# Ensembl/WiggleTools

Measured on AMD Instinct MI355X. Metric: genomic bp/s (whole node) for 'mean' over N BigWig tracks, higher is better.
Workload: dtype f64

## Files before the change

### wiggletools_amd/csrc/build.py

```python
import os
import subprocess
import sys

HERE = os.path.dirname(os.path.abspath(__file__))
SO = os.path.join(HERE, "libwiggletools_amd.so")
KERNEL_SRCS = ["wt_reduce_stream.hip", "wt_reduce_moments.hip", "wt_reduce_order.hip", "wt_patch_kernels.hip", "wt_delta_kernels.hip", "wt_walk.hip"]
SRCS = KERNEL_SRCS + ["wt_engine.hip", "wt_pipe.hip", "wt_compress.hip", "wt_moments.hip", "wt_map.hip", "wt_cover.hip", "wt_region.hip", "wt_synth.hip", "wt_bwdev.hip", "wt_defaults.cpp", "wt_iter_abi.cpp", "wt_bigwig.cpp", "wt_bwwrite.cpp"]
LIBS = ["-lz"]
FLAGS = ["--offload-arch=gfx950", "-O3", "-std=c++17", "-fPIC", "-shared", "-ffp-contract=off",
         "-Wall", "-Wno-unused-function", "-Wno-pass-failed"]


def build_source_variant(srcs, name, extra_flags):
    from concurrent.futures import ThreadPoolExecutor
    srcs = [srcs] if isinstance(srcs, str) else list(srcs)
    hipcc = os.environ.get("HIPCC", "/opt/rocm/bin/hipcc")
    objdir = os.path.join(HERE, ".obj")
    cflags = [f for f in FLAGS if f != "-shared"]

    def compile_one(src):
        obj = os.path.join(objdir, "%s_%s.o" % (src, name))
        subprocess.check_call([hipcc] + cflags + list(extra_flags) + ["-c", os.path.join(HERE, src), "-o", obj])
        return obj

    with ThreadPoolExecutor(len(srcs)) as ex:
        objs = list(ex.map(compile_one, srcs))
    others = [os.path.join(objdir, s + ".o") for s in SRCS if s not in srcs]
    out = os.path.join(HERE, "libwiggletools_amd_%s.so" % name)
    subprocess.check_call([hipcc, "--offload-arch=gfx950", "-shared", "-fPIC"] + objs + others + LIBS + ["-o", out])
    return out


def build(force=False, verbose=False):
    import time
    from concurrent.futures import ThreadPoolExecutor
    srcs = [os.path.join(HERE, s) for s in SRCS]
    hipcc = os.environ.get("HIPCC", "/opt/rocm/bin/hipcc")
    objdir = os.path.join(HERE, ".obj")
    os.makedirs(objdir, exist_ok=True)
    cflags = [f for f in FLAGS if f != "-shared"]

    def newer_than_deps(target, obj):
        try:
            words = open(obj + ".d").read().replace("\\\n", " ").split()
            t = os.path.getmtime(target)
        except OSError:
            return False
        files = [os.path.join(HERE, w) for w in words[1:] if not w.endswith(":")]
        return bool(files) and all(os.path.exists(f) and os.path.getmtime(f) <= t for f in files)

    objs = [os.path.join(objdir, os.path.basename(s) + ".o") for s in srcs]
    if not force and all(newer_than_deps(SO, o) for o in objs):
        if verbose:
            print("wiggletools_amd: libwiggletools_amd.so is newer than the sources / headers of its %d objects: REUSED (force=True recompiles)" % len(objs))
        return SO
    if verbose:
        print("wiggletools_amd: COMPILING %d sources for gfx950 with hipcc" % len(srcs))

    def compile_one(src):
        obj = os.path.join(objdir, os.path.basename(src) + ".o")
        if not force and newer_than_deps(obj, obj):
            if verbose:
                print("wiggletools_amd: %s unchanged: object REUSED" % os.path.basename(src))
            return obj
        cmd = [hipcc] + cflags + ["-MMD", "-MF", os.path.relpath(obj, HERE) + ".d", "-c", os.path.basename(src), "-o", os.path.relpath(obj, HERE)]
        if verbose:
            print(" ".join(cmd))
        t0 = time.time()
        subprocess.check_call(cmd, cwd=HERE)
        if verbose:
            print("wiggletools_amd: %s compiled in %.0f s" % (os.path.basename(src), time.time() - t0))
        return obj

    with ThreadPoolExecutor(len(srcs)) as ex:
        objs = list(ex.map(compile_one, srcs))
    cmd = [hipcc, "--offload-arch=gfx950", "-shared", "-fPIC"] + objs + LIBS + ["-o", SO]
    if verbose:
        print(" ".join(cmd))
    subprocess.check_call(cmd)
    return SO


if __name__ == "__main__":
    print(build(force="--force" in sys.argv, verbose=True))
```

### wiggletools_amd/csrc/wt_core.h

```cpp
#ifndef WT_CORE_H_
#define WT_CORE_H_

#include <stdint.h>
#include <math.h>
#include <type_traits>

#ifdef WT_EMU
#define WT_DEV inline
#define WT_RESTRICT
#else
#include <hip/hip_runtime.h>
#define WT_DEV __device__ __forceinline__
#define WT_RESTRICT __restrict__
#endif

enum {
    WT_OP_SUM = 0, WT_OP_PRODUCT = 1, WT_OP_MEAN = 2, WT_OP_VAR = 3, WT_OP_STDDEV = 4,
    WT_OP_ENTROPY = 5, WT_OP_CV = 6, WT_OP_MIN = 7, WT_OP_MAX = 8, WT_OP_MEDIAN = 9,
    WT_OP_TTEST = 10, WT_OP_MWU = 11,
    WT_OP_MULTIPLEX = 12
};
#define WT_STRICT_SET0 1u
#define WT_STRICT_SET1 2u

// ... 1263 lines not shown
        auto sweep = [&](auto body) {
            int i = 0;
            for (; i + WT_MWU_RB <= N; i += WT_MWU_RB) {
                KeyT k[WT_MWU_RB];
#pragma unroll
                for (int u = 0; u < WT_MWU_RB; u++) k[u] = col[(size_t) (i + u) * colstride];
#pragma unroll
                for (int u = 0; u < WT_MWU_RB; u++) body(k[u]);
            }
            for (; i < N; i++) body(col[(size_t) i * colstride]);
        };
        sweep([&](KeyT key) { all_and &= key; all_or |= key; });
        const KeyT disputed = all_and ^ all_or;
        KeyT Kk = 0;
        for (int b = KB - B; b >= 0; b -= B) {
            const KeyT group = (KeyT) NT << b;
            if (!(disputed & group)) { Kk |= all_and & group; continue; }
            KeyT trial[NT];
            int below[NT];
#pragma unroll
            for (int q = 0; q < NT; q++) { trial[q] = Kk | ((KeyT) (q + 1) << b); below[q] = 0; }
            sweep([&](KeyT key) {
#pragma unroll
                for (int q = 0; q < NT; q++) below[q] += (key < trial[q]);
            });
#pragma unroll
            for (int q = 0; q < NT; q++)
                if (below[q] <= kth) Kk = trial[q];
        }
        const double m = (sizeof(ScrT) == 4) ? (double) wt_unkey32((uint32_t) Kk) : wt_unkey64((uint64_t) Kk);
        res[0] = A.nan[0] ? wt_nan() : m;
        return;
    }
    if (OP == WT_OP_MWU) return;
    if (OP == WT_OP_MULTIPLEX) {
#pragma unroll
        for (int k = 0; k < K; k++) res[k] = A.a[k];
        return;
    }
}

WT_DEV int32_t wt_next_breakpoint(const WtParams &P, const WtCtx &c, int p) {
    const int w = p >> 6;
    const uint64_t here = c.U[w] & ~wt_mask_incl(p & 63);
    const int w2 = here ? w : (int) c.nextw[w];
    if (w2 < 0) return c.sh->next_bp;
    const uint64_t bits = here ? here : c.U[w2];
    return c.sh->w0 + w2 * 64 + wt_ctz64(bits);
}

WT_DEV void wt_phase_emask(const WtParams &P, WtCtx &c, bool two, int tid, int nt) {
    const int nw32 = P.n_words * 2;
    const uint64_t *any0 = (const uint64_t *) c.cover;
    const uint64_t *all0 = (const uint64_t *) (c.cover + nw32);
    const uint64_t *any1 = (const uint64_t *) (c.cover + 2 * nw32);
    const uint64_t *all1 = (const uint64_t *) (c.cover + 3 * nw32);
    for (int w = tid; w < P.n_words; w += nt) {
        uint64_t emit = (P.flags & WT_STRICT_SET0) ? all0[w] : any0[w];
        if (two) emit &= (P.flags & WT_STRICT_SET1) ? all1[w] : any1[w];
        const long long room = (long long) c.sh->emit_hi - ((long long) c.sh->w0 + (long long) w * 64);
        if (room < 64) emit &= (room <= 0) ? 0ull : ((1ull << room) - 1ull);
        c.E[w] = c.U[w] & emit;
    }
    if (tid == nt - 1) {
        int last = -1;
        for (int w = P.n_words - 1; w >= 0; w--) {
            c.nextw[w] = (int16_t) last;
            if (c.U[w]) last = w;
        }
    }
}

WT_DEV void wt_phase_escan(const WtParams &P, WtCtx &c, int tid, int nt) {
    for (int w = tid; w <= P.n_words; w += nt) {
        unsigned s = 0;
        for (int x = 0; x < w; x++) s += (unsigned) wt_popc64(c.E[x]);
        c.epfx[w] = s;
    }
}

template <int K>
WT_DEV unsigned wt_lane_emit_bits(const WtParams &P, const WtCtx &c, int tid) {
    const int p0 = tid * K;
    if (p0 >= P.W) return 0u;
    return (unsigned) ((c.E[p0 >> 6] >> (p0 & 63)) & ((1ull << K) - 1ull));
}

template <int OP, class ValT, class ScrT, int K, int NR>
WT_DEV void wt_phase_eval_chunk(const WtParams &P, WtCtx &c, WtAcc<K, NR> &A, int pass, int t_lo, int t_hi, bool all,
                                int tid, int nt) {
    const int p0 = tid * K;
    if (p0 >= P.W) return;
    const unsigned emit_bits = all ? ((1u << K) - 1u) : wt_lane_emit_bits<K>(P, c, tid);
    if (!emit_bits) return;
    long long run0 = 0;
    if (OP == WT_OP_MULTIPLEX) {
        const int w = p0 >> 6, b0 = p0 & 63;
        const uint64_t below0 = b0 ? wt_mask_incl(b0 - 1) : 0ull;
        run0 = c.sh->goffset + c.epfx[w] + wt_popc64(c.E[w] & below0);
    }
    wt_eval_chunk<OP, ValT, ScrT, K>(P, c, p0, A, pass, t_lo, t_hi, c.scratch, tid, P.W, emit_bits, run0);
}

template <int OP, class ValT, class ScrT, int K, int NR>
WT_DEV void wt_phase_eval_finish(const WtParams &P, WtCtx &c, WtAcc<K, NR> &A, WtLane<K> &L, int tid, int nt) {
    const unsigned emit_bits = wt_lane_emit_bits<K>(P, c, tid);
    if (!emit_bits) return;
    wt_eval_finish<OP, ValT, ScrT, K>(P, A, L.res, c.scratch, c.attr, tid, P.W, emit_bits);
}

template <class ScrT>
WT_DEV void wt_phase_mwu_rank(const WtParams &P, WtCtx &c, int tid, int nt) {
    const int p = tid % P.W, part = tid / P.W, nparts = nt / P.W;
    if (!((c.E[p >> 6] >> (p & 63)) & 1ull)) return;
    wt_mwu_rank<ScrT>(P, c.scratch, c.attr, p, P.W, part, nparts);
}
template <int K, int NR>
WT_DEV void wt_phase_mwu_tail(const WtParams &P, WtCtx &c, const WtAcc<K, NR> &A, WtLane<K> &L, int tid, int nt) {
    if (tid >= P.W || !((c.E[tid >> 6] >> (tid & 63)) & 1ull)) return;
    L.res[0] = A.nan[0] ? wt_nan() : wt_mwu_tail(P, c.attr, tid, P.W);
}

WT_DEV void wt_lookback_finish(const WtParams &P, WtCtx &c, long long k, unsigned long long excl,
                               unsigned long long mine) {
    WtShared *sh = c.sh;
    wt_status_store(&P.status[k], WT_FLAG_PFX | (excl + mine));
    sh->goffset = (long long) excl;
    const int ch = sh->chrom;
    if (k == P.c_first_win[ch]) P.chrom_run_off[ch] = (long long) excl;
    if (k == P.n_windows - 1) {
        P.chrom_run_off[P.n_chrom] = (long long) (excl + mine);
        P.counters[WT_CTR_RUNS] = excl + mine;
    }
    if ((long long) (excl + mine) > P.capacity) wt_glb_or64(&P.counters[WT_CTR_ERROR], WT_ERR_CAPACITY);
}

WT_DEV void wt_phase_lookback(const WtParams &P, WtCtx &c, long long k, unsigned long long mine);
WT_DEV void wt_phase_lookback(const WtParams &P, WtCtx &c, long long k) {
    wt_phase_lookback(P, c, k, (unsigned long long) c.epfx[P.n_words]);
}
WT_DEV void wt_phase_lookback(const WtParams &P, WtCtx &c, long long k, unsigned long long mine) {
    c.sh->n_emit = (int32_t) mine;
    unsigned long long excl = 0;
    if (k > 0) {
        wt_status_store(&P.status[k], WT_FLAG_AGG | mine);
        long long j = k - 1;
        for (;;) {
            unsigned long long v = wt_status_load(&P.status[j]);
            unsigned spins = 0;
            while (v == 0) {
                wt_backoff();
                v = wt_status_load(&P.status[j]);
                if (++spins > (1u << 24)) {
                    wt_glb_or64(&P.counters[WT_CTR_ERROR], WT_ERR_LOOKBACK);
                    v = WT_FLAG_PFX;
                }
            }
            excl += v & WT_VAL_MASK;
            if (v & WT_FLAG_PFX) break;
            j--;
        }
    }
    wt_lookback_finish(P, c, k, excl, mine);
}

#ifndef WT_EMU
WT_DEV void wt_lookback_publish(const WtParams &P, WtCtx &c, long long k, unsigned long long mine) {
    c.sh->n_emit = (int32_t) mine;
    if (k > 0) wt_status_store(&P.status[k], WT_FLAG_AGG | mine);
}
WT_DEV void wt_lookback_publish(const WtParams &P, WtCtx &c, long long k) {
    wt_lookback_publish(P, c, k, (unsigned long long) c.epfx[P.n_words]);
}

WT_DEV void wt_lookback_complete(const WtParams &P, WtCtx &c, long long k, int lane, unsigned long long mine);
WT_DEV void wt_lookback_complete(const WtParams &P, WtCtx &c, long long k, int lane) {
    wt_lookback_complete(P, c, k, lane, (unsigned long long) c.epfx[P.n_words]);
}
#ifndef WT_LOOKBACK_DEPTH
#define WT_LOOKBACK_DEPTH 1
#endif
WT_DEV void wt_lookback_complete(const WtParams &P, WtCtx &c, long long k, int lane, unsigned long long mine) {
    unsigned long long excl = 0;
    long long base = k - 1;
    unsigned long long ahead[WT_LOOKBACK_DEPTH];
    int have = 0;
    while (base >= 0) {
        const long long j = base - lane;
        if (have == 0) {
#pragma unroll
            for (int r = 0; r < WT_LOOKBACK_DEPTH; r++) {
                const long long jr = j - 64ll * r;
                ahead[r] = (jr >= 0) ? wt_status_load(&P.status[jr]) : WT_FLAG_PFX;
            }
            have = WT_LOOKBACK_DEPTH;
        }
        unsigned long long v = ahead[0];
#pragma unroll
        for (int r = 1; r < WT_LOOKBACK_DEPTH; r++) v = (WT_LOOKBACK_DEPTH - have == r) ? ahead[r] : v;
        have--;
        unsigned long long pfx;
        unsigned spins = 0;
        for (;;) {
            const unsigned long long ready = __ballot(v != 0);
            pfx = __ballot((v & WT_FLAG_PFX) != 0);
            const unsigned long long need = pfx ? (((pfx & (0ull - pfx)) << 1) - 1ull) : ~0ull;
            if ((ready & need) == need) break;
            if (++spins > (1u << 22)) {
                if (lane == 0) wt_glb_or64(&P.counters[WT_CTR_ERROR], WT_ERR_LOOKBACK);
                pfx = 1ull;
                break;
            }
            if (v == 0) { wt_backoff(); v = wt_status_load(&P.status[j]); }
        }
        const int p = pfx ? (int) wt_ctz64(pfx) : 63;
        unsigned long long part = (lane <= p) ? (v & WT_VAL_MASK) : 0ull;
        excl += wt_wave_sum_u64(part);
        if (pfx) break;
        base -= 64;
    }
    if (lane == 0) wt_lookback_finish(P, c, k, excl, mine);
}
#endif

template <int OP, class ValT, int K>
WT_DEV void wt_phase_write(const WtParams &P, WtCtx &c, const WtLane<K> &L, int tid, int nt) {
    const int p0 = tid * K;
    unsigned emit_bits = 0;
    if (p0 < P.W) emit_bits = (unsigned) ((c.E[p0 >> 6] >> (p0 & 63)) & ((1ull << K) - 1ull));
    unsigned long long bp = 0;
    if (emit_bits) {
        const long long goff = c.sh->goffset;
        const int32_t w0 = c.sh->w0;
        const int w = p0 >> 6, b0 = p0 & 63;
        const uint64_t below0 = b0 ? wt_mask_incl(b0 - 1) : 0ull;
        long long idx = goff + c.epfx[w] + wt_popc64(c.E[w] & below0);
#pragma unroll
        for (int k = 0; k < K; k++) {
            if (!((emit_bits >> k) & 1u)) continue;
            const long long o = idx++;
            const int p = p0 + k;
            const int32_t fin = wt_next_breakpoint(P, c, p);
            bp += (unsigned long long) (fin - (w0 + p));
            if (o >= P.capacity) continue;
            P.o_start[o] = w0 + p;
            P.o_finish[o] = fin;
            P.o_value[o] = L.res[k];
        }
        wt_lds_add64(&c.sh->bp_sum, bp);
    }
}

WT_DEV void wt_window_stats(const WtParams &P, WtCtx &c) {
    if (c.sh->bp_sum) wt_glb_add64(&P.counters[WT_CTR_BP], c.sh->bp_sum);
    if (c.sh->n_intervals) wt_glb_add64(&P.counters[WT_CTR_INTERVALS], c.sh->n_intervals);
}

WT_DEV long long wt_index_find_segment(const WtParams &P, long long g) {
    long long lo = 0, hi = (long long) P.n_chrom * P.n_tracks;
    while (hi - lo > 1) {
        const long long mid = (lo + hi) >> 1;
        if (P.seg_off[mid] <= g) lo = mid; else hi = mid;
    }
    return lo;
}

struct WtIndexCursor {
    long long seg, s0, s1;
    long long nw, rowbase;
    int32_t cb;
    int i;
};

WT_DEV void wt_index_cursor_set(const WtParams &P, WtIndexCursor &c, long long seg) {
    const int N = P.n_tracks;
    c.seg = seg;
    c.s0 = P.seg_off[seg];
    c.s1 = P.seg_off[seg + 1];
    const int ch = (int) (seg / N);
    c.i = (int) (seg - (long long) ch * N);
    c.cb = P.cbase[ch];
    c.nw = P.c_nwin[ch];
    c.rowbase = P.c_first_win[ch] + ch;
}

WT_DEV void wt_index_apply(const WtParams &P, WtIndexCursor &c, long long g, int32_t f, int32_t pf) {
    while (g >= c.s1) wt_index_cursor_set(P, c, c.seg + 1);
    if (g > c.s0 && g + 1 < c.s1 && pf >= c.cb &&
        ((uint32_t) (pf - c.cb) >> P.logW) == ((uint32_t) (f - c.cb) >> P.logW)) return;
    const long long jr = g - c.s0;
    const int32_t cb = c.cb;
    long long m_lo = 0;
    if (jr > 0 && pf >= cb) m_lo = (long long) ((uint32_t) (pf - cb) >> P.logW) + 1;
    long long m_hi = (f >= cb) ? (long long) ((uint32_t) (f - cb) >> P.logW) : -1;
    const bool last = (g + 1 == c.s1);
    if (m_lo > m_hi && !last) return;
    const int N = P.n_tracks;
    if (m_hi > c.nw) m_hi = c.nw;
    for (long long m = m_lo; m <= m_hi; m++) P.widx[(size_t) (c.rowbase + m) * N + c.i] = (uint32_t) jr;
    if (last)
        for (long long m = m_hi + 1; m <= c.nw; m++) P.widx[(size_t) (c.rowbase + m) * N + c.i] = (uint32_t) (jr + 1);
}

WT_DEV long long wt_lane_lower_bound(const int32_t *fin, long long lo, long long hi, long long g, long long b) {
    if (lo >= hi) return lo;
    if ((long long) fin[g] >= b) {
        hi = g;
        for (long long d = 1;; d <<= 1) {
            const long long q = hi - d;
            if (q < lo) break;
            if ((long long) fin[q] < b) { lo = q + 1; break; }
            hi = q;
        }
    } else {
        lo = g + 1;
        for (long long d = 1;; d <<= 1) {
            const long long q = lo + d - 1;
            if (q >= hi) break;
            if ((long long) fin[q] >= b) { hi = q; break; }
            lo = q + 1;
        }
    }
    while (lo < hi) {
        const long long mid = (lo + hi) >> 1;
        if ((long long) fin[mid] < b) lo = mid + 1; else hi = mid;
    }
    return lo;
}

#include "wt_delta.h"
#include "wt_walk.h"
#include "wt_mwalk.h"

#endif
```

### wiggletools_amd/csrc/wt_devscope.h

```cpp
#ifndef WT_DEVSCOPE_H_
#define WT_DEVSCOPE_H_
#include <hip/hip_runtime.h>

#include <vector>

struct WtDevScope {
    std::vector<void *> ptrs;
    WtDevScope() = default;
    WtDevScope(const WtDevScope &) = delete;
    WtDevScope &operator=(const WtDevScope &) = delete;
    template <class T>
    hipError_t alloc(T **p, size_t bytes) {
        void *q = nullptr;
        const hipError_t e = hipMalloc(&q, bytes ? bytes : 1);
        if (e == hipSuccess) { ptrs.push_back(q); *p = (T *) q; }
        return e;
    }
    ~WtDevScope() {
        for (void *q : ptrs) (void) hipFree(q);
    }
};

#endif
```

### wiggletools_amd/csrc/wt_engine.hip

```cpp
#include <hip/hip_runtime.h>

#include <cstdio>
#include <thread>
#include <atomic>
#include <cstring>
#include <map>
#include <mutex>
#include <string>
#include <vector>

#include "wt_host.h"
#include "wt_trackset.h"
#include "wt_core.h"
#include "wt_plan.h"
#include "wt_kernels.h"
#include "wt_devscope.h"

#ifndef WT_INDEX_UNROLL
#define WT_INDEX_UNROLL 2
#endif
#define WT_INDEX_CHUNK (256 * 4 * WT_INDEX_UNROLL)
__global__ void __launch_bounds__(256) wt_index_kernel(const WtParams P, long long total, long long span) {
    const long long dev_total = P.seg_off[(long long) P.n_chrom * P.n_tracks];
    if (total > dev_total) total = dev_total;
    const long long begin0 = (long long) blockIdx.x * span;
    long long end0 = begin0 + span;
    if (end0 > total) end0 = total;
    if (begin0 >= end0) return;
    WtIndexCursor cur;
    wt_index_cursor_set(P, cur, wt_index_find_segment(P, begin0));
    struct __attribute__((packed, aligned(4))) V4 { int32_t x[4]; };
    V4 f[WT_INDEX_UNROLL], nf[WT_INDEX_UNROLL];
    int32_t pf[WT_INDEX_UNROLL], npf[WT_INDEX_UNROLL];
    const long long n_full = (end0 - begin0) / WT_INDEX_CHUNK;
    auto fetch = [&](long long base, V4 (&v)[WT_INDEX_UNROLL], int32_t (&p)[WT_INDEX_UNROLL]) {
#pragma unroll
        for (int u = 0; u < WT_INDEX_UNROLL; u++) {
            const long long g = base + 4ll * (threadIdx.x + 256 * u);
            v[u] = *(const V4 *) (P.finish + g);
            p[u] = P.finish[g > 0 ? g - 1 : 0];
        }
    };
    if (n_full > 0) {
        const long long last_full = begin0 + (n_full - 1) * WT_INDEX_CHUNK;
        fetch(begin0, f, pf);
        for (long long begin = begin0; begin <= last_full; begin += WT_INDEX_CHUNK) {
            const long long nb = begin + WT_INDEX_CHUNK;
            fetch(nb <= last_full ? nb : last_full, nf, npf);
#pragma unroll
            for (int u = 0; u < WT_INDEX_UNROLL; u++) {
                const long long g = begin + 4ll * (threadIdx.x + 256 * u);
                int32_t prev = pf[u];
#pragma unroll
                for (int q = 0; q < 4; q++) {
                    wt_index_apply(P, cur, g + q, f[u].x[q], prev);
                    prev = f[u].x[q];
                }
            }
#pragma unroll
            for (int u = 0; u < WT_INDEX_UNROLL; u++) { f[u] = nf[u]; pf[u] = npf[u]; }
        }
    }
    const long long begin = begin0 + n_full * WT_INDEX_CHUNK;
    if (begin < end0) {
#pragma unroll
        for (int u = 0; u < WT_INDEX_UNROLL; u++) {
            const long long g = begin + 4ll * (threadIdx.x + 256 * u);
            int32_t prev = (g < end0 && g > 0) ? P.finish[g - 1] : 0;
#pragma unroll
            for (int q = 0; q < 4; q++) {
                if (g + q < end0) {
                    const int32_t fq = P.finish[g + q];
                    wt_index_apply(P, cur, g + q, fq, prev);
                    prev = fq;
                }
            }
        }
    }
}

#define WT_ISEARCH_ROWS 64
#define WT_ISEARCH_TRACKS 16

__device__ __forceinline__ int wt_index_row_chrom(const WtParams &P, long long row) {
    int lo = 0;
    for (int hi = P.n_chrom; hi - lo > 1;) {
        const int mid = (lo + hi) >> 1;
        if (P.c_first_win[mid] + mid <= row) lo = mid; else hi = mid;
    }
    return lo;
}

__global__ void __launch_bounds__(256) wt_index_coarse_kernel(const WtParams P, long long n_strips, uint32_t *coarse) {
    const long long t = (long long) blockIdx.x * 256 + threadIdx.x;
    const int N = P.n_tracks;
    if (t >= n_strips * N) return;
    const long long strip = t / N;
    const int i = (int) (t - strip * N);
    const long long row = strip * WT_ISEARCH_ROWS;
    const int ch = wt_index_row_chrom(P, row);
    const long long m = row - (P.c_first_win[ch] + ch);
    const long long seg = (long long) ch * N + i;
    const long long s0 = P.seg_off[seg], n = P.seg_off[seg + 1] - s0;
    const long long b = (long long) P.cbase[ch] + (m << P.logW);
    coarse[t] = (uint32_t) wt_lane_lower_bound(P.finish + s0, 0, n, n >> 1, b);
}

__global__ void __launch_bounds__(WT_ISEARCH_ROWS * WT_ISEARCH_TRACKS) wt_index_search_kernel(const WtParams P, long long n_rows, long long n_strips,
                                                                                              const uint32_t *coarse) {
    __shared__ uint32_t out[WT_ISEARCH_ROWS][WT_ISEARCH_TRACKS + 1];
    const int tid = threadIdx.x, lane = tid & 63, wave = tid >> 6;
    const int N = P.n_tracks;
    const long long strip = blockIdx.x;
    const long long r0 = strip * WT_ISEARCH_ROWS;
    const int i = (int) blockIdx.y * WT_ISEARCH_TRACKS + wave;
    if (i < N) {
        long long row = r0 + lane;
        if (row > n_rows - 1) row = n_rows - 1;
        const int ch = wt_index_row_chrom(P, row);
        const long long m = row - (P.c_first_win[ch] + ch);
        const long long seg = (long long) ch * N + i;
        const long long s0 = P.seg_off[seg], n = P.seg_off[seg + 1] - s0;
        const long long b = (long long) P.cbase[ch] + (m << P.logW);
        const int32_t *fin = P.finish + s0;
        const int ch_first = __shfl(ch, 0);
        const bool have_next = strip + 1 < n_strips;
        const int ch_next = have_next ? wt_index_row_chrom(P, r0 + WT_ISEARCH_ROWS) : -1;
        const bool real_a = ch == ch_first, real_b = ch == ch_next;
        const long long A = real_a ? (long long) coarse[strip * N + i] : 0;
        const long long B = real_b ? (long long) coarse[(strip + 1) * N + i] : n;
        long long g = (real_a && real_b) ? A + (((B - A) * lane) >> 6) : (A + B) >> 1;
        if (g > B - 1) g = B - 1;
        out[lane][wave] = (uint32_t) wt_lane_lower_bound(fin, A, B, g, b);
    }
    __syncthreads();
    const int orow = tid / WT_ISEARCH_TRACKS, ocol = tid % WT_ISEARCH_TRACKS;
    const long long row = r0 + orow;
    const int track = (int) blockIdx.y * WT_ISEARCH_TRACKS + ocol;
    if (row < n_rows && track < N) P.widx[(size_t) row * N + track] = out[orow][ocol];
}

__global__ void __launch_bounds__(256) wt_index_compare_kernel(const uint32_t *a, const uint32_t *b, long long n, unsigned long long *diff) {
    const long long t = (long long) blockIdx.x * 256 + threadIdx.x;
    if (t < n && a[t] != b[t]) atomicAdd(diff, 1ull);
}

__global__ void __launch_bounds__(256) wt_extents_kernel(const int64_t *seg_off, const int32_t *start,
                                                          const int32_t *finish, long long n_seg,
                                                          int32_t *first_start, int32_t *last_finish) {
    const long long s = (long long) blockIdx.x * blockDim.x + threadIdx.x;
    if (s >= n_seg) return;
    const long long lo = seg_off[s], hi = seg_off[s + 1];
    first_start[s] = hi > lo ? start[lo] : 0;
    last_finish[s] = hi > lo ? finish[hi - 1] : 0;
}

__global__ void __launch_bounds__(256) wt_validate_kernel(const int32_t *start, const int32_t *finish, const int64_t *seg_off,
                                                           long long n_seg, long long total, unsigned long long *out) {
    const long long g = (long long) blockIdx.x * blockDim.x + threadIdx.x;
    if (g >= total) return;
    bool bad = finish[g] <= start[g];
    if (!bad && g > 0 && start[g] < finish[g - 1]) {
        long long lo = 0, hi = n_seg;
        while (hi - lo > 1) {
            const long long mid = (lo + hi) >> 1;
            if (seg_off[mid] <= g) lo = mid; else hi = mid;
        }
        bad = seg_off[lo] != g;
    }
    if (bad) {
        atomicAdd(&out[0], 1ull);
        atomicMin(&out[1], (unsigned long long) g);
    }
}

static thread_local std::string g_last_error;

int wt_fail(int code, const std::string &msg) {
    g_last_error = msg;
    return code;
}

template <class T>
static hipError_t wt_grow(T **p, int64_t *cap, int64_t need) {
    if (*cap >= need && *p) return hipSuccess;
    int64_t c = *cap * 2;
    if (c < need) c = need;
    if (c < 1) c = 1;
    (void) hipFree(*p);
    *p = nullptr; *cap = 0;
    const hipError_t e = hipMalloc((void **) p, sizeof(T) * (size_t) c);
    if (e == hipSuccess) *cap = c;
    return e;
}

static void wt_free_windows(WtWindows &w) {
    (void) hipFree(w.d_tabs);
    (void) hipFree(w.d_widx); (void) hipFree(w.d_cidx); (void) hipFree(w.d_status); (void) hipFree(w.d_bad_list); (void) hipFree(w.d_bad_goff);
    if (w.h_tab) (void) hipHostFree(w.h_tab);
    w = WtWindows();
}

extern "C" {

const char *wtamd_last_error(void) { return g_last_error.c_str(); }
const char *wtamd_version(void) { return "wiggletools_amd 0.1 (gfx950)"; }

int wtamd_device_count(void) {
    int n = 0;
    if (hipGetDeviceCount(&n) != hipSuccess) return 0;
    return n;
}

__global__ void wt_warm_kernel(int *p) { if (p && threadIdx.x == 4096) *p = 0; }

static std::mutex g_warm_mu;
static std::thread *g_warm_thread = nullptr;
static bool g_warm_started = false;

extern "C++" void wt_warmup_join() {
    std::thread *t = nullptr;
    { std::lock_guard<std::mutex> lk(g_warm_mu); t = g_warm_thread; g_warm_thread = nullptr; }
    if (t) { t->join(); delete t; }
}

static std::atomic<int> g_device_chosen{-1};

void wtamd_warmup_async(void) {
    std::lock_guard<std::mutex> lk(g_warm_mu);
    if (g_warm_started || getenv("WTAMD_NO_WARMUP")) return;
    int n = 0, cur = -1;
    if (hipGetDeviceCount(&n) != hipSuccess || n <= 0) { (void) hipGetLastError(); return; }
    int ordinal = g_device_chosen.load();
    if (ordinal < 0 && hipGetDevice(&cur) == hipSuccess && (n == 1 || cur > 0)) ordinal = cur;
    if (ordinal < 0 || ordinal >= n) return;
    g_warm_started = true;
    g_warm_thread = new std::thread([ordinal] {
        if (hipSetDevice(ordinal) != hipSuccess) { (void) hipGetLastError(); return; }
        hipStream_t st[3] = {nullptr, nullptr, nullptr};
        for (auto &s : st)
            if (hipStreamCreateWithFlags(&s, hipStreamNonBlocking) != hipSuccess) s = nullptr;
        for (auto &s : st)
            if (s) hipLaunchKernelGGL(wt_warm_kernel, dim3(1), dim3(64), 0, s, (int *) nullptr);
        for (auto &s : st)
            if (s) { (void) hipStreamSynchronize(s); (void) hipStreamDestroy(s); }
        (void) hipGetLastError();
    });
    atexit(wt_warmup_join);
}

int wtamd_set_device(int ordinal) {
    wt_warmup_join();
    WT_HIP(hipSetDevice(ordinal));
    g_device_chosen.store(ordinal);
    return WTAMD_OK;
}

int wtamd_current_device(void) {
    int d = 0;
    if (hipGetDevice(&d) != hipSuccess) { (void) hipGetLastError(); return -1; }
    return d;
}

extern "C++" int wt_trackset_common(const wtamd_tracks *t, wtamd_trackset *ts) {
    if (!t || t->n_chrom < 0 || t->n_tracks <= 0 || !t->seg_off || !t->defaults)
        return wt_fail(WTAMD_ERR_ARG, "wtamd_trackset_create: bad tracks descriptor");
    if (wtamd_device_count() <= 0) return wt_fail(WTAMD_ERR_NODEVICE, "no HIP device visible");
    ts->n_chrom = t->n_chrom;
    ts->n_tracks = t->n_tracks;
    ts->value_f64 = t->value_is_f64 != 0;
    const int64_t n_seg = (int64_t) t->n_chrom * t->n_tracks;
    ts->seg_off.assign(t->seg_off, t->seg_off + n_seg + 1);
    for (int64_t s = 0; s < n_seg; s++)
        if (ts->seg_off[s + 1] < ts->seg_off[s]) return wt_fail(WTAMD_ERR_ARG, "seg_off not monotone");
    ts->n_intervals = ts->seg_off[n_seg] - ts->seg_off[0];
    if (ts->seg_off[0] != 0) return wt_fail(WTAMD_ERR_ARG, "seg_off[0] must be 0");
    ts->defaults.assign(t->defaults, t->defaults + t->n_tracks);
    if (t->range_lo && t->range_hi) {
        ts->range_lo.assign(t->range_lo, t->range_lo + t->n_chrom);
        ts->range_hi.assign(t->range_hi, t->range_hi + t->n_chrom);
    }
    ts->scratch_f32 = !ts->value_f64 && wt_defaults_fit_f32(ts->defaults.data(), ts->n_tracks);
    WT_HIP(hipGetDevice(&ts->device));
    hipDeviceProp_t prop;
    WT_HIP(hipGetDeviceProperties(&prop, ts->device));
    ts->num_cu = prop.multiProcessorCount;
    WT_HIP(hipMalloc(&ts->d_seg_off, sizeof(int64_t) * (n_seg + 1)));
    WT_HIP(hipMemcpy(ts->d_seg_off, ts->seg_off.data(), sizeof(int64_t) * (n_seg + 1), hipMemcpyHostToDevice));
    WT_HIP(hipMalloc(&ts->d_defaults, sizeof(double) * t->n_tracks));
    WT_HIP(hipMemcpy(ts->d_defaults, ts->defaults.data(), sizeof(double) * t->n_tracks, hipMemcpyHostToDevice));
    WT_HIP(hipMalloc(&ts->d_counters, sizeof(unsigned long long) * WT_CTR_N));
    WT_HIP(hipHostMalloc(&ts->h_counters, sizeof(unsigned long long) * WT_CTR_N));
    WT_HIP(hipHostMalloc(&ts->h_debug, sizeof(unsigned long long) * 16));
    memset(ts->h_debug, 0, sizeof(unsigned long long) * 16);
    WT_HIP(hipMalloc(&ts->d_chrom_run_off, sizeof(int64_t) * (t->n_chrom + 1)));
    WT_HIP(hipEventCreate(&ts->ev_i0));
    WT_HIP(hipEventCreate(&ts->ev_i1));
    WT_HIP(hipEventCreate(&ts->ev_r0));
    WT_HIP(hipEventCreate(&ts->ev_r1));
    return WTAMD_OK;
}

extern "C++" int wt_check_extents(wtamd_trackset *ts) {
    for (size_t q = 0; q < ts->last_finish.size(); q++)
        if (ts->seg_off[q + 1] > ts->seg_off[q] && ts->last_finish[q] > WTAMD_MAX_COORD) {
            const int64_t bad = ts->last_finish[q];
            return wt_fail(WTAMD_ERR_ARG, "run finish " + std::to_string(bad) + " above the supported maximum " +
                           std::to_string((long long) WTAMD_MAX_COORD) + " (2^31 - 65537)");
        }
    return WTAMD_OK;
}

static int wt_refresh_extents_device(wtamd_trackset *ts) {
    const int64_t n_seg = (int64_t) ts->n_chrom * ts->n_tracks;
    ts->first_start.assign(n_seg, 0);
    ts->last_finish.assign(n_seg, 0);
    if (n_seg > 0 && ts->n_intervals > 0) {
        int32_t *d_fs = nullptr, *d_lf = nullptr;
        WtDevScope scope;
        WT_HIP(scope.alloc(&d_fs, sizeof(int32_t) * n_seg));
        WT_HIP(scope.alloc(&d_lf, sizeof(int32_t) * n_seg));
        hipLaunchKernelGGL(wt_extents_kernel, dim3((unsigned) ((n_seg + 255) / 256)), dim3(256), 0, 0,
                           ts->d_seg_off, ts->d_start, ts->d_finish, (long long) n_seg, d_fs, d_lf);
        WT_HIP(hipGetLastError());
        WT_HIP(hipMemcpy(ts->first_start.data(), d_fs, sizeof(int32_t) * n_seg, hipMemcpyDeviceToHost));
        WT_HIP(hipMemcpy(ts->last_finish.data(), d_lf, sizeof(int32_t) * n_seg, hipMemcpyDeviceToHost));
    }
    return WTAMD_OK;
}

static int wt_create_host_impl(const wtamd_tracks *t, wtamd_trackset *ts) {
    int rc = wt_trackset_common(t, ts);
    if (rc != WTAMD_OK) return rc;
    ts->owns = true;
    const int64_t n = ts->n_intervals;
    const size_t vsz = ts->value_f64 ? 8 : 4;
    const int64_t n_alloc = n > 0 ? n : 1;
    WT_HIP(hipMalloc(&ts->d_start, sizeof(int32_t) * n_alloc));
    WT_HIP(hipMalloc(&ts->d_finish, sizeof(int32_t) * n_alloc));
    WT_HIP(hipMalloc(&ts->d_value, vsz * n_alloc));
    if (n > 0) {
        if (!t->start || !t->finish || !t->value) return wt_fail(WTAMD_ERR_ARG, "NULL arrays");
        WT_HIP(hipMemcpy(ts->d_start, t->start, sizeof(int32_t) * n, hipMemcpyHostToDevice));
        WT_HIP(hipMemcpy(ts->d_finish, t->finish, sizeof(int32_t) * n, hipMemcpyHostToDevice));
        WT_HIP(hipMemcpy(ts->d_value, t->value, vsz * n, hipMemcpyHostToDevice));
    }
    const int64_t n_seg = (int64_t) ts->n_chrom * ts->n_tracks;
    ts->first_start.assign(n_seg, 0);
    ts->last_finish.assign(n_seg, 0);
    for (int64_t s = 0; s < n_seg; s++)
        if (ts->seg_off[s + 1] > ts->seg_off[s]) {
            ts->first_start[s] = t->start[ts->seg_off[s]];
            ts->last_finish[s] = t->finish[ts->seg_off[s + 1] - 1];
        }
    return wt_check_extents(ts);
}

int wtamd_trackset_create_host(const wtamd_tracks *t, wtamd_trackset **out) {
    if (!out) return wt_fail(WTAMD_ERR_ARG, "out == NULL");
    wtamd_trackset *ts = new wtamd_trackset();
    const int rc = wt_create_host_impl(t, ts);
    if (rc != WTAMD_OK) { wtamd_trackset_destroy(ts); return rc; }
    *out = ts;
    return WTAMD_OK;
}

static int wt_create_device_impl(const wtamd_tracks *t, wtamd_trackset *ts) {
    int rc = wt_trackset_common(t, ts);
    if (rc != WTAMD_OK) return rc;
    ts->owns = false;
    ts->d_start = const_cast<int32_t *>(t->start);
    ts->d_finish = const_cast<int32_t *>(t->finish);
    ts->d_value = const_cast<void *>(t->value);
    rc = wt_refresh_extents_device(ts);
    if (rc != WTAMD_OK) return rc;
    return wt_check_extents(ts);
}

int wtamd_trackset_create_device(const wtamd_tracks *t, wtamd_trackset **out) {
    if (!out) return wt_fail(WTAMD_ERR_ARG, "out == NULL");
    wtamd_trackset *ts = new wtamd_trackset();
    const int rc = wt_create_device_impl(t, ts);
    if (rc != WTAMD_OK) { wtamd_trackset_destroy(ts); return rc; }
    *out = ts;
    return WTAMD_OK;
}

void wtamd_trackset_destroy(wtamd_trackset *ts) {
    if (!ts) return;
    if (ts->owns) { (void) hipFree(ts->d_start); (void) hipFree(ts->d_finish); (void) hipFree(ts->d_value); }
    (void) hipFree(ts->d_seg_off); (void) hipFree(ts->d_defaults); (void) hipFree(ts->d_counters); (void) hipFree(ts->d_chrom_run_off); (void) hipFree(ts->d_gscratch); (void) hipFree(ts->d_mwu_table);
    for (double *q : ts->mwu_retired) (void) hipFree(q);
    if (ts->h_counters) (void) hipHostFree(ts->h_counters);
    if (ts->h_debug) (void) hipHostFree(ts->h_debug);
    for (auto &kv : ts->windows) wt_free_windows(kv.second);
    if (ts->ev_i0) (void) hipEventDestroy(ts->ev_i0);
    if (ts->ev_i1) (void) hipEventDestroy(ts->ev_i1);
    if (ts->ev_r0) (void) hipEventDestroy(ts->ev_r0);
    if (ts->ev_r1) (void) hipEventDestroy(ts->ev_r1);
    delete ts;
}

static int64_t wt_span(const wtamd_trackset *ts) {
    int64_t span = 0;
    for (int c = 0; c < ts->n_chrom; c++) {
        int64_t lo = INT64_MAX, hi = INT64_MIN;
        for (int i = 0; i < ts->n_tracks; i++) {
            const int64_t s = (int64_t) c * ts->n_tracks + i;
            if (ts->seg_off[s + 1] > ts->seg_off[s]) {
                lo = std::min<int64_t>(lo, ts->first_start[s]);
                hi = std::max<int64_t>(hi, ts->last_finish[s]);
            }
        }
        if (lo <= hi) span += hi - lo;
    }
    return span;
}

int64_t wtamd_trackset_max_runs(const wtamd_trackset *ts) {
    if (!ts) return 0;
    return std::min<int64_t>(2 * ts->n_intervals, wt_span(ts));
}

static int wt_get_windows(wtamd_trackset *ts, int W, WtWindows **out, hipStream_t s = nullptr) {
    WtWindows &w = ts->windows[W];
    *out = &w;
    if (w.tab_valid) return WTAMD_OK;
    wt_make_windows(ts->n_chrom, ts->n_tracks, ts->seg_off.data(), ts->first_start.data(), ts->last_finish.data(), W, w.tab,
                    ts->range_lo.empty() ? nullptr : ts->range_lo.data(),
                    ts->range_hi.empty() ? nullptr : ts->range_hi.data());
    w.indexed = false;
    const int64_t nc = ts->n_chrom > 0 ? ts->n_chrom : 1;
    const int64_t nwin = w.tab.n_windows > 0 ? w.tab.n_windows : 1;
    const int64_t nwidx = (w.tab.n_rows > 0 ? w.tab.n_rows : 1) * (int64_t) ts->n_tracks;
    auto up8 = [](int64_t x) { return (x + 7) & ~(int64_t) 7; };
    if (w.cap_chrom < nc || w.cap_win < nwin || !w.d_tabs) {
        const int64_t cc = w.cap_chrom < nc ? std::max<int64_t>(nc, 2 * w.cap_chrom) : w.cap_chrom;
        const int64_t cw = w.cap_win < nwin ? std::max<int64_t>(nwin, 2 * w.cap_win) : w.cap_win;
        const int64_t o_cnwin = up8(4 * cc), o_chi = o_cnwin + up8(4 * cc), o_cfirst = o_chi + up8(4 * cc), o_win = o_cfirst + 8 * (cc + 1);
        const int64_t total = o_win + up8(4 * cw);
        (void) hipFree(w.d_tabs);
        w.d_tabs = nullptr; w.cap_tabs = 0;
        w.d_cbase = w.d_cnwin = w.d_chi = w.d_win_chrom = nullptr; w.d_cfirst = nullptr;
        if (w.cap_win < cw) { (void) hipFree(w.d_status); w.d_status = nullptr; }
        w.cap_chrom = 0; w.cap_win = 0;
        WT_HIP(hipMalloc((void **) &w.d_tabs, (size_t) total));
        if (!w.d_status) WT_HIP(hipMalloc((void **) &w.d_status, sizeof(unsigned long long) * (size_t) cw));
        w.cap_tabs = total;
        w.d_cbase = (int32_t *) w.d_tabs; w.d_cnwin = (int32_t *) (w.d_tabs + o_cnwin); w.d_chi = (int32_t *) (w.d_tabs + o_chi);
        w.d_cfirst = (int64_t *) (w.d_tabs + o_cfirst); w.d_win_chrom = (int32_t *) (w.d_tabs + o_win);
        w.cap_chrom = cc; w.cap_win = cw;
    }
    WT_HIP(wt_grow(&w.d_widx, &w.cap_widx, nwidx));
    WT_HIP(wt_grow(&w.d_cidx, &w.cap_cidx, ((w.tab.n_rows > 0 ? w.tab.n_rows : 1) + WT_ISEARCH_ROWS - 1) / WT_ISEARCH_ROWS * (int64_t) ts->n_tracks));
    if (ts->n_chrom > 0) {
        if (ts->pipe_mode) {
            if (ts->n_chrom != 1) return wt_fail(WTAMD_ERR_INTERNAL, "pipeline slots hold one chromosome");
            if (!w.h_tab) WT_HIP(hipHostMalloc((void **) &w.h_tab, 64, hipHostMallocDefault));
            int32_t *h32 = (int32_t *) w.h_tab;
            h32[0] = w.tab.cbase[0]; h32[1] = w.tab.c_nwin[0]; h32[2] = w.tab.c_hi[0];
            w.h_tab[2] = w.tab.c_first_win[0]; w.h_tab[3] = w.tab.c_first_win[1];
            WT_HIP(hipMemcpyAsync(w.d_cbase, h32 + 0, sizeof(int32_t), hipMemcpyHostToDevice, s));
            WT_HIP(hipMemcpyAsync(w.d_cnwin, h32 + 1, sizeof(int32_t), hipMemcpyHostToDevice, s));
            WT_HIP(hipMemcpyAsync(w.d_chi, h32 + 2, sizeof(int32_t), hipMemcpyHostToDevice, s));
            WT_HIP(hipMemcpyAsync(w.d_cfirst, w.h_tab + 2, 2 * sizeof(int64_t), hipMemcpyHostToDevice, s));
            WT_HIP(hipMemsetAsync(w.d_win_chrom, 0, sizeof(int32_t) * (size_t) nwin, s));
        } else {
            const int64_t used = ((char *) w.d_win_chrom - w.d_tabs) + (int64_t) sizeof(int32_t) * std::max<int64_t>(w.tab.n_windows, 0);
            std::vector<char> pack((size_t) used, 0);
            memcpy(pack.data() + ((char *) w.d_cbase - w.d_tabs), w.tab.cbase.data(), sizeof(int32_t) * ts->n_chrom);
            memcpy(pack.data() + ((char *) w.d_cnwin - w.d_tabs), w.tab.c_nwin.data(), sizeof(int32_t) * ts->n_chrom);
            memcpy(pack.data() + ((char *) w.d_chi - w.d_tabs), w.tab.c_hi.data(), sizeof(int32_t) * ts->n_chrom);
            memcpy(pack.data() + ((char *) w.d_cfirst - w.d_tabs), w.tab.c_first_win.data(), sizeof(int64_t) * (ts->n_chrom + 1));
            if (w.tab.n_windows > 0) memcpy(pack.data() + ((char *) w.d_win_chrom - w.d_tabs), w.tab.win_chrom.data(), sizeof(int32_t) * w.tab.n_windows);
            WT_HIP(hipMemcpy(w.d_tabs, pack.data(), (size_t) used, hipMemcpyHostToDevice));
        }
    }
    w.tab_valid = true;
    return WTAMD_OK;
}

static void wt_fill_params(const wtamd_trackset *ts, const WtWindows *w, const WtPlan &plan, WtParams &P) {
    memset(&P, 0, sizeof(P));
    P.start = ts->d_start; P.finish = ts->d_finish; P.value = ts->d_value;
    P.seg_off = ts->d_seg_off; P.defaults = ts->d_defaults;
    P.n_chrom = ts->n_chrom; P.n_tracks = ts->n_tracks; P.n_total = ts->n_intervals;
    P.cbase = w->d_cbase; P.c_nwin = w->d_cnwin; P.c_hi = w->d_chi; P.c_first_win = w->d_cfirst;
    P.n_windows = w->tab.n_windows; P.win_chrom = w->d_win_chrom; P.widx = w->d_widx;
    P.status = w->d_status; P.counters = ts->d_counters; P.debug = ts->h_debug;
    wt_plan_to_params(plan, P);
}

static int wt_build_index(wtamd_trackset *ts, WtWindows *w, const WtPlan &plan, hipStream_t s) {
    WtParams P;
    wt_fill_params(ts, w, plan, P);
    WT_HIP(hipEventRecord(ts->ev_i0, s));
    static const int mode = [] {
        const char *e = getenv("WTAMD_INDEX"), *c = getenv("WTAMD_INDEX_CHECK");
        if (c && atoi(c) > 0) return 2;
        return (e && !strcmp(e, "scan")) ? 1 : 0;
    }();
    const size_t n_widx = (size_t) w->tab.n_rows * ts->n_tracks;
    auto scan = [&](uint32_t *dst) -> int {
        WtParams Q = P;
        Q.widx = dst;
        WT_HIP(hipMemsetAsync(dst, 0, sizeof(uint32_t) * n_widx, s));
        if (ts->n_intervals > 0) {
            const long long total = ts->n_intervals;
            long long blocks = (total + WT_INDEX_CHUNK - 1) / WT_INDEX_CHUNK;
            const long long cap = (long long) ts->num_cu * 8;
            if (blocks > cap) blocks = cap;
            long long span = (total + blocks - 1) / blocks;
            span = (span + WT_INDEX_CHUNK - 1) / WT_INDEX_CHUNK * WT_INDEX_CHUNK;
            blocks = (total + span - 1) / span;
            hipLaunchKernelGGL(wt_index_kernel, dim3((unsigned) blocks), dim3(256), 0, s, Q, total, span);
            WT_HIP(hipGetLastError());
        }
        return WTAMD_OK;
    };
    auto search = [&](uint32_t *dst) -> int {
        WtParams Q = P;
        Q.widx = dst;
        const long long n_rows = w->tab.n_rows;
        if (n_rows > 0 && ts->n_tracks > 0) {
            const long long n_strips = (n_rows + WT_ISEARCH_ROWS - 1) / WT_ISEARCH_ROWS;
            if (w->cap_cidx < n_strips * ts->n_tracks) return wt_fail(WTAMD_ERR_INTERNAL, "coarse window index not allocated");
            hipLaunchKernelGGL(wt_index_coarse_kernel, dim3((unsigned) ((n_strips * ts->n_tracks + 255) / 256)), dim3(256), 0, s, Q, n_strips, w->d_cidx);
            WT_HIP(hipGetLastError());
            const dim3 grid((unsigned) n_strips, (unsigned) ((ts->n_tracks + WT_ISEARCH_TRACKS - 1) / WT_ISEARCH_TRACKS));
            hipLaunchKernelGGL(wt_index_search_kernel, grid, dim3(WT_ISEARCH_ROWS * WT_ISEARCH_TRACKS), 0, s, Q, n_rows, n_strips, (const uint32_t *) w->d_cidx);
            WT_HIP(hipGetLastError());
        }
        return WTAMD_OK;
    };
    if (mode == 1) {
        if (int rc = scan(w->d_widx)) return rc;
    } else {
        if (int rc = search(w->d_widx)) return rc;
    }
    if (mode == 2 && n_widx > 0) {
        uint32_t *other = nullptr;
        unsigned long long *d_diff = nullptr, h_diff = 0;
        WT_HIP(hipMalloc(&other, sizeof(uint32_t) * n_widx));
        WT_HIP(hipMalloc(&d_diff, sizeof(unsigned long long)));
        WT_HIP(hipMemsetAsync(d_diff, 0, sizeof(unsigned long long), s));
        if (int rc = scan(other)) return rc;
        hipLaunchKernelGGL(wt_index_compare_kernel, dim3((unsigned) ((n_widx + 255) / 256)), dim3(256), 0, s, w->d_widx, other, (long long) n_widx, d_diff);
        WT_HIP(hipMemcpyAsync(&h_diff, d_diff, sizeof(h_diff), hipMemcpyDeviceToHost, s));
        WT_HIP(hipStreamSynchronize(s));
        (void) hipFree(other); (void) hipFree(d_diff);
        if (h_diff) {
            fprintf(stderr, "wiggletools_amd: WTAMD_INDEX_CHECK: the searched window index differs from the scanned one in %llu of %zu entries\n", h_diff, n_widx);
            return wt_fail(WTAMD_ERR_INTERNAL, "window index check failed");
        }
    }
    WT_HIP(hipEventRecord(ts->ev_i1, s));
    ts->have_index_time = true;
    w->indexed = true;
    return WTAMD_OK;
}

static inline int wt_delta_class(int op) { return op == WT_OP_TTEST ? 1 : ((op == WT_OP_MAX || op == WT_OP_MIN) ? 2 : 0); }
static bool wt_wants_delta(const wtamd_trackset *ts, int op) {
    return !ts->delta_failed_[wt_delta_class(op)] && wt_delta_eligible(op, ts->value_f64, ts->n_tracks, ts->defaults.data());
}

static double wt_events_per_bp(const wtamd_trackset *ts) {
    const int64_t span = wt_span(ts);
    return span > 0 ? 1.25 * (double) ts->n_intervals / (double) span : 0.0;
}

static bool wt_mwu_few_ties(wtamd_trackset *ts, hipStream_t stream) {
    if (ts->mwu_few_ties >= 0) return ts->mwu_few_ties != 0;
    ts->mwu_few_ties = 0;
    if (hipStreamSynchronize(stream) != hipSuccess) { (void) hipGetLastError(); return false; }
    const int64_t n = ts->n_intervals;
    if (n < 1024 || ts->value_f64 || !ts->d_value) return false;
    const int64_t S = std::min<int64_t>(4096, n), stride = n / S;
    std::vector<uint32_t> v((size_t) S);
    if (hipMemcpy2D(v.data(), 4, ts->d_value, (size_t) stride * 4, 4, (size_t) S, hipMemcpyDeviceToHost) != hipSuccess) { (void) hipGetLastError(); return false; }
    std::sort(v.begin(), v.end());
    const int64_t distinct = (int64_t) (std::unique(v.begin(), v.end()) - v.begin());
    ts->mwu_few_ties = distinct * 100 >= S * 97 ? 1 : 0;
    return ts->mwu_few_ties != 0;
}

static bool wt_pick_plan(wtamd_trackset *ts, int op, int n_set0, WtPlan &plan, std::string &err, hipStream_t stream = nullptr) {
    static const int mwalk = getenv("WTAMD_MWALK") ? (atoi(getenv("WTAMD_MWALK")) != 0 ? 1 : 0) : -1;
    const bool walk = !getenv("WTAMD_NO_WALK");
    const bool mwu_walk = op == WT_OP_MWU && mwalk != 0 && !ts->value_f64 && walk && (mwalk == 1 || wt_mwu_few_ties(ts, stream));
    const double events_per_bp = (op == WT_OP_MEDIAN || op == WT_OP_MWU) ? wt_events_per_bp(ts) : 0.0;
    return wt_pick_general_plan(ts->n_tracks, op, ts->value_f64, ts->scratch_f32, n_set0, walk, mwu_walk, events_per_bp, plan, err);
}

static void wt_trackset_forget(wtamd_trackset *ts, bool delta_failed) {
    for (int q = 0; q < 3; q++) { ts->delta_verified_[q] = false; ts->delta_failed_[q] = delta_failed; ts->delta_n_bad_[q] = 0; }
    for (auto &kv : ts->windows) kv.second.indexed = false;
}

extern "C++" int wt_trackset_rebind(wtamd_trackset *ts, int64_t n, const int64_t *seg_off, int32_t range_lo, int32_t range_hi, bool value_f64,
                                    int32_t *d_start, int32_t *d_finish, void *d_value, bool delta_failed) {
    ts->n_intervals = n;
    ts->seg_off.assign(seg_off, seg_off + (int64_t) ts->n_chrom * ts->n_tracks + 1);
    ts->range_lo[0] = range_lo;
    ts->range_hi[0] = range_hi;
    ts->value_f64 = value_f64;
    ts->scratch_f32 = !ts->value_f64 && wt_defaults_fit_f32(ts->defaults.data(), ts->n_tracks);
    ts->d_start = d_start; ts->d_finish = d_finish; ts->d_value = d_value;
    wt_trackset_forget(ts, delta_failed);
    for (auto &kv : ts->windows) kv.second.tab_valid = false;
    return wt_check_extents(ts);
}

int wtamd_trackset_index(wtamd_trackset *ts, int op, void *stream) {
    if (!ts) return wt_fail(WTAMD_ERR_ARG, "ts == NULL");
    wt_trackset_forget(ts, false);
    ts->mwu_few_ties = -1;
    if (!ts->owns && !ts->pipe_mode) {
        int rce = wt_refresh_extents_device(ts);
        if (rce != WTAMD_OK) return rce;
        rce = wt_check_extents(ts);
        if (rce != WTAMD_OK) return rce;
        for (auto &kv : ts->windows) kv.second.tab_valid = false;
    }
    WtPlan plan;
    std::string err;
    if (wt_wants_delta(ts, op)) wt_make_delta_plan_for(plan, ts->n_tracks, op);
    else if (!wt_pick_plan(ts, op, ts->n_tracks / 2, plan, err, (hipStream_t) stream)) return wt_fail(WTAMD_ERR_ARG, err);
    WtWindows *w = nullptr;
    int rc = wt_get_windows(ts, plan.W, &w, (hipStream_t) stream);
    if (rc != WTAMD_OK) return rc;
    return wt_build_index(ts, w, plan, (hipStream_t) stream);
}

extern "C++" int wt_check_desc(const wtamd_trackset *ts, const wtamd_reduce_desc *d) {
    if (!ts || !d) return wt_fail(WTAMD_ERR_ARG, "NULL argument");
    if (d->op < 0 || d->op >= WTAMD_OP_COUNT_) return wt_fail(WTAMD_ERR_ARG, "unknown op");
    if (d->op == WTAMD_OP_TTEST) {
        if (d->n_set0 < 3 || ts->n_tracks - d->n_set0 < 3)
            return wt_fail(WTAMD_ERR_ARG, "The t-test function only works for two sets with enough elements to compute variance");
    } else if (d->op == WTAMD_OP_MWU) {
        if (d->n_set0 < 1 || ts->n_tracks - d->n_set0 < 1)
            return wt_fail(WTAMD_ERR_ARG, "The Mann-Whitney U function only works for two non-empty sets");
    }
    return WTAMD_OK;
}

static int wt_reduce_plan(wtamd_trackset *ts, const WtPlan &plan, int op, uint32_t flags, int n_set0, wtamd_runs *runs,
                          double *d_tile, uint8_t *d_inplay, int64_t *n_runs, hipStream_t s);

extern "C++" int wt_launch_patch(wtamd_trackset *ts, int delta_W, int op, uint32_t flags, int n_set0, wtamd_runs *runs, long long n_bad,
                                 hipStream_t s) {
    WtPlan plan;
    std::string err;
    if (!wt_make_plan(ts->n_tracks, op, ts->scratch_f32, plan, err)) return wt_fail(WTAMD_ERR_INTERNAL, err);
    if (!wt_patch_compatible(plan, delta_W, ts->scratch_f32, ts->value_f64))
        return wt_fail(WTAMD_ERR_INTERNAL, "no general plan compatible with the difference-array windows (general W " + std::to_string(plan.W) + ", difference-array W " +
                       std::to_string(delta_W) + ", slab " + std::to_string((long long) plan.scratch_slab) + ", float staging " + std::to_string((int) ts->scratch_f32) + ", f64 values " +
                       std::to_string((int) ts->value_f64) + ")");
    WtWindows *dw = nullptr, *w = nullptr;
    int rc = wt_get_windows(ts, delta_W, &dw, s);
    if (rc != WTAMD_OK) return rc;
    rc = wt_get_windows(ts, plan.W, &w, s);
    if (rc != WTAMD_OK) return rc;
    WtLaunch L;
    WtParams &P = L.P;
    wt_fill_params(ts, w, plan, P);
    P.op = op; P.flags = flags; P.n_set0 = op == WT_OP_TTEST ? n_set0 : 0;
    P.capacity = runs->capacity;
    P.o_start = runs->start; P.o_finish = runs->finish; P.o_value = runs->value;
    P.chrom_run_off = runs->chrom_run_off ? runs->chrom_run_off : ts->d_chrom_run_off;
    L.T = plan.T; L.lds = plan.lds_bytes; L.stream = s; L.num_cu = ts->num_cu;
    WtPatchArgs Q;
    Q.bad_list = dw->d_bad_list; Q.bad_goff = dw->d_bad_goff;
    Q.n_bad = ts->d_counters + WT_CTR_DELTA_BAD;
    Q.d_win_chrom = dw->d_win_chrom; Q.d_c_first_win = dw->d_cfirst;
    Q.ratio = delta_W / plan.W;
    if (!wt_patch_launch(L, Q, op, plan.ppt, plan.n_chunks > 1, n_bad, !w->indexed))
        return wt_fail(WTAMD_ERR_INTERNAL, "no general plan compatible with the difference-array windows");
    if (L.err != hipSuccess) return wt_fail(WTAMD_ERR_HIP, std::string("patch kernel launch: ") + hipGetErrorString(L.err));
    WT_HIP(hipEventRecord(ts->ev_r1, s));
    ts->stats.patched_windows = (int32_t) n_bad;
    return WTAMD_OK;
}

static int wt_reduce_impl(wtamd_trackset *ts, int op, uint32_t flags, int n_set0, wtamd_runs *runs,
                          double *d_tile, uint8_t *d_inplay, int64_t *n_runs, hipStream_t s) {
    if (!runs || !runs->start || !runs->finish || !runs->value)
        return wt_fail(WTAMD_ERR_ARG, "wtamd_reduce: output arrays missing");
    WtPlan plan;
    std::string err;
    if (!d_tile && wt_wants_delta(ts, op)) {
        wt_make_delta_plan_for(plan, ts->n_tracks, op);
        const int dc = wt_delta_class(op);
        int64_t n_probe = 0;
        const bool probe = !ts->delta_verified_[dc];
        const int rc = wt_reduce_plan(ts, plan, op, flags, n_set0, runs, d_tile, d_inplay,
                                      (probe && !n_runs) ? &n_probe : n_runs, s);
        if (!probe) {
            if (ts->delta_n_bad_[dc] > 0 && (rc == WTAMD_OK || rc == WTAMD_ERR_CAPACITY)) {
                const int rp = wt_launch_patch(ts, plan.W, op, flags, n_set0, runs, ts->delta_n_bad_[dc], s);
                if (rp != WTAMD_OK) return rp;
                if (n_runs) WT_HIP(hipStreamSynchronize(s));
            }
            return rc;
        }
        if (rc != WTAMD_OK && rc != WTAMD_ERR_CAPACITY) return rc;
        const long long n_bad = (long long) ts->h_counters[WT_CTR_DELTA_BAD];
        if (n_bad == 0) { ts->delta_verified_[dc] = true; ts->delta_n_bad_[dc] = 0; return rc; }
        if (wt_few_enough_to_patch(n_bad, ts->stats.n_windows) && !getenv("WTAMD_NO_PATCH")) {
            const int rp = wt_launch_patch(ts, plan.W, op, flags, n_set0, runs, n_bad, s);
            if (rp == WTAMD_OK) {
                WT_HIP(hipStreamSynchronize(s));
                ts->delta_verified_[dc] = true;
                ts->delta_n_bad_[dc] = n_bad;
                return rc;
            }
            if (rp != WTAMD_ERR_INTERNAL) return rp;
        }
        ts->delta_failed_[dc] = true;
    }
    if (!wt_pick_plan(ts, op, n_set0, plan, err, s)) return wt_fail(WTAMD_ERR_ARG, err);
    return wt_reduce_plan(ts, plan, op, flags, n_set0, runs, d_tile, d_inplay, n_runs, s);
}

extern "C++" int wt_reduce_enqueue(wtamd_trackset *ts, const wtamd_reduce_desc &desc, wtamd_runs *runs, double *d_tile, uint8_t *d_inplay,
                                   hipStream_t s, bool *used_delta, int *delta_W) {
    WtPlan plan;
    std::string err;
    *used_delta = !d_tile && wt_wants_delta(ts, desc.op);
    if (*used_delta) {
        wt_make_delta_plan_for(plan, ts->n_tracks, desc.op);
        *delta_W = plan.W;
    } else if (!wt_pick_plan(ts, desc.op, desc.n_set0, plan, err, s)) {
        return wt_fail(WTAMD_ERR_ARG, err);
    }
    return wt_reduce_plan(ts, plan, desc.op, desc.flags, desc.n_set0, runs, d_tile, d_inplay, nullptr, s);
}

static int wt_reduce_plan(wtamd_trackset *ts, const WtPlan &plan, int op, uint32_t flags, int n_set0, wtamd_runs *runs,
                          double *d_tile, uint8_t *d_inplay, int64_t *n_runs, hipStream_t s) {
    if (plan.T > (plan.delta ? ((wt_op_is_var_family(op) || op == WT_OP_TTEST) ? wt_delta_sq_block : wt_delta_block) : wt_reduce_max_block)) return wt_fail(WTAMD_ERR_ARG, "workgroup size above the kernel's launch bound");
    WtWindows *w = nullptr;
    int rc = wt_get_windows(ts, plan.W, &w, s);
    if (rc != WTAMD_OK) return rc;
    if (!w->indexed) {
        rc = wt_build_index(ts, w, plan, s);
        if (rc != WTAMD_OK) return rc;
    }
    WtLaunch L;
    wt_fill_params(ts, w, plan, L.P);
    L.P.op = op; L.P.flags = flags; L.P.n_set0 = n_set0;
    L.P.capacity = runs->capacity;
    L.P.o_start = runs->start; L.P.o_finish = runs->finish; L.P.o_value = runs->value;
    L.P.chrom_run_off = runs->chrom_run_off ? runs->chrom_run_off : ts->d_chrom_run_off;
    L.P.o_tile = d_tile; L.P.o_inplay = d_inplay;
    L.T = plan.T; L.lds = plan.lds_bytes; L.stream = s; L.num_cu = ts->num_cu;
    L.gscratch = &ts->d_gscratch; L.gscratch_bytes = &ts->gscratch_bytes;
    if (op == WT_OP_MWU && !getenv("WTAMD_MWU_DEVICE_ERF")) {
        const int n1 = n_set0, n2 = ts->n_tracks - n_set0;
        if (ts->mwu_n1 != n1 || ts->mwu_n2 != n2) {
            std::vector<double> t;
            const bool have = wt_mwu_make_table(n1, n2, t);
            if (ts->d_mwu_table) { ts->mwu_retired.push_back(ts->d_mwu_table); ts->d_mwu_table = nullptr; }
            if (have) {
                WT_HIP(hipMalloc((void **) &ts->d_mwu_table, sizeof(double) * t.size()));
                WT_HIP(hipMemcpyAsync(ts->d_mwu_table, t.data(), sizeof(double) * t.size(), hipMemcpyHostToDevice, s));
                WT_HIP(hipStreamSynchronize(s));
            }
            ts->mwu_n1 = n1; ts->mwu_n2 = n2; ts->mwu_kmax = have ? (int) t.size() - 1 : 0;
        }
        L.P.mwu_table = ts->d_mwu_table;
        L.P.mwu_kmax = ts->mwu_kmax;
    }
    if (plan.delta) {
        const int64_t nwin = w->tab.n_windows > 0 ? w->tab.n_windows : 1;
        if (w->cap_bad < nwin) {
            int64_t c1 = w->cap_bad, c2 = w->cap_bad;
            WT_HIP(wt_grow(&w->d_bad_list, &c1, nwin));
            WT_HIP(wt_grow(&w->d_bad_goff, &c2, nwin * WT_BAD_SUB));
            w->cap_bad = c1 < c2 / WT_BAD_SUB ? c1 : c2 / WT_BAD_SUB;
        }
        L.P.bad_list = w->d_bad_list;
        L.P.bad_goff = w->d_bad_goff;
        wt_delta_defaults_params(ts->defaults.data(), ts->n_tracks, L.P);
    }

    WT_HIP(hipMemsetAsync(ts->d_counters, 0, sizeof(unsigned long long) * WT_CTR_N, s));
    WT_HIP(hipMemsetAsync(L.P.chrom_run_off, 0, sizeof(int64_t) * (ts->n_chrom + 1), s));
    if (w->tab.n_windows > 0 && ts->n_intervals > 0) {
        WT_HIP(hipMemsetAsync(w->d_status, 0, sizeof(unsigned long long) * w->tab.n_windows, s));
        if (plan.delta) {
            static const int force_u = getenv("WTAMD_DELTA_U") ? atoi(getenv("WTAMD_DELTA_U")) : 0;
            const double tiles_per_wave = (double) ts->n_intervals / (double) w->tab.n_windows / 256.0 / (double) std::max(1, L.T / 64);
            L.small_tiles = force_u == 2 || (force_u != 4 && tiles_per_wave < 8.0);
        }
        WT_HIP(hipEventRecord(ts->ev_r0, s));
        if (plan.delta) {
            wt_delta_launch(L, op);
        } else if (plan.walk_S) {
            L.err = wt_walk_launch(L.P, plan.regcol, L.T, L.lds, L.num_cu, L.gscratch, L.gscratch_bytes, L.stream, &L.grid);
        } else if (!wt_reduce_launch(L, op, ts->value_f64, ts->scratch_f32, plan.ppt, plan.n_chunks > 1 || plan.scratch_slab > 0, plan.regcol)) {
            return wt_fail(WTAMD_ERR_ARG, "op not dispatchable");
        }
        if (L.err != hipSuccess) return wt_fail(WTAMD_ERR_HIP, std::string("kernel launch: ") + hipGetErrorString(L.err));
        WT_HIP(hipEventRecord(ts->ev_r1, s));
        ts->have_reduce_time = true;
    }
    ts->stats.n_windows = w->tab.n_windows;
    ts->stats.window_bp = plan.W;
    ts->stats.lds_bytes = plan.lds_bytes;
    ts->stats.kernel = plan.delta ? 1 : (plan.walk_S ? (plan.walk_mwu ? 3 : 2) : 0);
    ts->stats.patched_windows = 0;
    if (n_runs) {
        WT_HIP(hipMemcpyAsync(ts->h_counters, ts->d_counters, sizeof(unsigned long long) * WT_CTR_N, hipMemcpyDeviceToHost, s));
        const int rcw = wt_bounded_wait([s] { return hipStreamQuery(s); }, "hipStreamQuery", nullptr, 0.002, 200, [ts](double limit_s) {
            char buf[320];
            snprintf(buf, sizeof buf, "kernel did not finish within %.0f s (debug marker %llu, window %lld; per wave %llu %llu %llu %llu %llu %llu %llu %llu)",
                     limit_s, ts->h_debug[0], (long long) ts->h_debug[1], ts->h_debug[2], ts->h_debug[3], ts->h_debug[4],
                     ts->h_debug[5], ts->h_debug[6], ts->h_debug[7], ts->h_debug[8], ts->h_debug[9]);
            return std::string(buf);
        });
        if (rcw != WTAMD_OK) return rcw;
        ts->stats.n_runs = (int64_t) ts->h_counters[WT_CTR_RUNS];
        ts->stats.covered_bp = (int64_t) ts->h_counters[WT_CTR_BP];
        ts->stats.n_intervals = (int64_t) ts->h_counters[WT_CTR_INTERVALS];
        *n_runs = ts->stats.n_runs;
        if (plan.walk_S) {
            static const bool show = getenv("WTAMD_WALK_PROF") != nullptr;
            if (show) {
                static const char *names_w[8] = {"zero+ranges", "count", "offsets", "scatter", "events", "first-median", "moves", "rest"};
                unsigned long long tot = 0;
                for (int q = 0; q < 8; q++) tot += ts->h_counters[WT_CTR_PROF + q];
                fprintf(stderr, "[wt_walk_profile]");
                for (int q = 0; q < 8; q++) fprintf(stderr, " %s %.1f%%", names_w[q], tot ? 100.0 * ts->h_counters[WT_CTR_PROF + q] / tot : 0.0);
                fprintf(stderr, " (total %.3g cycles)\n", (double) tot);
            }
        }
#ifdef WT_PROFILE
        {
            static const char *names_g[8] = {"zero", "load", "count", "emask+escan", "eval", "lookback", "write", "-"};
            static const char *names_d[8] = {"zero", "ranges", "pass1", "pass2", "scan", "escan", "lookback", "write"};
            const char **names = plan.delta ? names_d : names_g;
            unsigned long long tot = 0;
            for (int q = 0; q < 8; q++) tot += ts->h_counters[WT_CTR_PROF + q];
            fprintf(stderr, "[wt_profile] op %d:", op);
            for (int q = 0; q < 8; q++)
                fprintf(stderr, " %s %.1f%%", names[q], tot ? 100.0 * ts->h_counters[WT_CTR_PROF + q] / tot : 0.0);
            fprintf(stderr, " (total %.3g cycles over all workgroups)\n", (double) tot);
            unsigned long long p2[8] = {0};
            if (wt_prof2_take(p2))
                fprintf(stderr, "[wt_profile] register column, cycles summed over waves: gather %.3g  sort/park %.3g  count loop %.3g  erf %.3g  median sort+select %.3g\n",
                        (double) p2[0], (double) p2[1], (double) p2[2], (double) p2[3], (double) p2[4]);
        }
#endif
        if (ts->h_counters[WT_CTR_ERROR] & WT_ERR_LOOKBACK) return wt_fail(WTAMD_ERR_INTERNAL, "look-back timed out");
        if (ts->h_counters[WT_CTR_ERROR] & WT_ERR_CAPACITY) return wt_fail(WTAMD_ERR_CAPACITY, "output capacity too small");
    }
    return WTAMD_OK;
}

int wtamd_reduce(wtamd_trackset *ts, const wtamd_reduce_desc *desc, wtamd_runs *runs, int64_t *n_runs, void *stream) {
    int rc = wt_check_desc(ts, desc);
    if (rc != WTAMD_OK) return rc;
    return wt_reduce_impl(ts, desc->op, desc->flags, desc->n_set0, runs, nullptr, nullptr, n_runs, (hipStream_t) stream);
}

static int wt_reduce_host_impl(wtamd_trackset *ts, int op, uint32_t flags, int n_set0, wtamd_runs *runs,
                               double *h_tile, uint8_t *h_inplay, int64_t *n_runs) {
    if (!runs) return wt_fail(WTAMD_ERR_ARG, "runs == NULL");
    int64_t cap = wtamd_trackset_max_runs(ts);
    if (cap > runs->capacity) cap = runs->capacity;
    const int64_t alloc = cap > 0 ? cap : 1;
    const int N = ts->n_tracks;
    WtDevScope scope;
    wtamd_runs d{};
    d.capacity = cap;
    double *d_tile = nullptr;
    uint8_t *d_inplay = nullptr;
    WT_HIP(scope.alloc(&d.start, sizeof(int32_t) * alloc));
    WT_HIP(scope.alloc(&d.finish, sizeof(int32_t) * alloc));
    WT_HIP(scope.alloc(&d.value, sizeof(double) * alloc));
    WT_HIP(scope.alloc(&d.chrom_run_off, sizeof(int64_t) * (ts->n_chrom + 1)));
    if (op == WT_OP_MULTIPLEX) {
        WT_HIP(scope.alloc(&d_tile, sizeof(double) * alloc * N));
        WT_HIP(scope.alloc(&d_inplay, sizeof(uint8_t) * alloc * N));
    }
    int64_t n = 0;
    int rc = wt_reduce_impl(ts, op, flags, n_set0, &d, d_tile, d_inplay, &n, nullptr);
    if (rc == WTAMD_OK) {
        if (n > 0) {
            WT_HIP(hipMemcpy(runs->start, d.start, sizeof(int32_t) * n, hipMemcpyDeviceToHost));
            WT_HIP(hipMemcpy(runs->finish, d.finish, sizeof(int32_t) * n, hipMemcpyDeviceToHost));
            if (runs->value) WT_HIP(hipMemcpy(runs->value, d.value, sizeof(double) * n, hipMemcpyDeviceToHost));
            if (h_tile) WT_HIP(hipMemcpy(h_tile, d_tile, sizeof(double) * n * N, hipMemcpyDeviceToHost));
            if (h_inplay) WT_HIP(hipMemcpy(h_inplay, d_inplay, sizeof(uint8_t) * n * N, hipMemcpyDeviceToHost));
        }
        if (runs->chrom_run_off)
            WT_HIP(hipMemcpy(runs->chrom_run_off, d.chrom_run_off, sizeof(int64_t) * (ts->n_chrom + 1), hipMemcpyDeviceToHost));
        if (n_runs) *n_runs = n;
    }
    return rc;
}

int wtamd_reduce_host(wtamd_trackset *ts, const wtamd_reduce_desc *desc, wtamd_runs *runs, int64_t *n_runs) {
    int rc = wt_check_desc(ts, desc);
    if (rc != WTAMD_OK) return rc;
    return wt_reduce_host_impl(ts, desc->op, desc->flags, desc->n_set0, runs, nullptr, nullptr, n_runs);
}

int wtamd_multiplex_host(wtamd_trackset *ts, uint32_t flags, wtamd_runs *runs, double *values, uint8_t *inplay,
                         int64_t *n_runs) {
    if (!ts || !values || !inplay) return wt_fail(WTAMD_ERR_ARG, "NULL argument");
    return wt_reduce_host_impl(ts, WT_OP_MULTIPLEX, flags, 0, runs, values, inplay, n_runs);
}

static int wt_runs_auc_span(const wtamd_runs *runs, int64_t n_runs, double *auc, double *span, void *stream) {
    hipStream_t s = (hipStream_t) stream;
    const int blocks = 512;
    double *d_partial = nullptr, h[2] = {0, 0};
    WtDevScope scope;
    WT_HIP(scope.alloc(&d_partial, wt_auc_partial_bytes(blocks) + sizeof(double) * 2));
    const int rc = wt_auc_async(runs->start, runs->finish, runs->value, (long long) n_runs, nullptr, blocks, d_partial, d_partial + 2 * blocks, span != nullptr, s);
    if (rc != WTAMD_OK) return rc;
    WT_HIP(hipMemcpyAsync(h, d_partial + 2 * blocks, sizeof(double) * (span ? 2 : 1), hipMemcpyDeviceToHost, s));
    WT_HIP(hipStreamSynchronize(s));
    *auc = h[0];
    if (span) *span = h[1];
    return WTAMD_OK;
}

int wtamd_runs_auc(const wtamd_runs *runs, int64_t n_runs, double *auc, void *stream) {
    if (!runs || !auc) return wt_fail(WTAMD_ERR_ARG, "NULL argument");
    return wt_runs_auc_span(runs, n_runs, auc, nullptr, stream);
}

int wtamd_runs_mean(const wtamd_runs *runs, int64_t n_runs, double *mean, void *stream) {
    if (!runs || !mean) return wt_fail(WTAMD_ERR_ARG, "NULL argument");
    double sum = 0, span = 0;
    const int rc = wt_runs_auc_span(runs, n_runs, &sum, &span, stream);
    if (rc != WTAMD_OK) return rc;
    *mean = span > 0 ? sum / span : __builtin_nan("");
    return WTAMD_OK;
}

static int wt_pearson_impl(wtamd_trackset *ts, double *result7) {
    if (ts->n_tracks != 2) return wt_fail(WTAMD_ERR_ARG, "wtamd_pearson: the track set must hold exactly two tracks");
    int64_t cap = wtamd_trackset_max_runs(ts);
    const int64_t alloc = cap > 0 ? cap : 1;
    wtamd_runs d{};
    d.capacity = cap;
    double *d_tile = nullptr;
    uint8_t *d_inplay = nullptr;
    char *d_partial = nullptr;
    double *d_out = nullptr;
    const int blocks = 256;
    WtDevScope scope;
    WT_HIP(scope.alloc(&d.start, sizeof(int32_t) * alloc));
    WT_HIP(scope.alloc(&d.finish, sizeof(int32_t) * alloc));
    WT_HIP(scope.alloc(&d.value, sizeof(double) * alloc));
    WT_HIP(scope.alloc(&d.chrom_run_off, sizeof(int64_t) * (ts->n_chrom + 1)));
    WT_HIP(scope.alloc(&d_tile, sizeof(double) * alloc * 2));
    WT_HIP(scope.alloc(&d_inplay, sizeof(uint8_t) * alloc * 2));
    WT_HIP(scope.alloc(&d_partial, wt_pearson_partial_bytes(blocks)));
    WT_HIP(scope.alloc(&d_out, sizeof(double) * 7));
    int64_t n = 0;
    int rc = wt_reduce_impl(ts, WT_OP_MULTIPLEX, 0, 0, &d, d_tile, d_inplay, &n, nullptr);
    if (rc == WTAMD_OK) {
        rc = wt_pearson_async(d.start, d.finish, d_tile, d_inplay, ts->defaults[0], ts->defaults[1], (long long) n, nullptr, blocks, d_partial, d_out, nullptr);
        if (rc != WTAMD_OK || hipMemcpy(result7, d_out, sizeof(double) * 7, hipMemcpyDeviceToHost) != hipSuccess)
            rc = wt_fail(WTAMD_ERR_HIP, "wtamd_pearson: kernel launch / copy failed");
    }
    return rc;
}

int wtamd_pearson(wtamd_trackset *ts, double *result) {
    if (!ts || !result) return wt_fail(WTAMD_ERR_ARG, "NULL argument");
    double r[7];
    const int rc = wt_pearson_impl(ts, r);
    if (rc == WTAMD_OK) *result = r[0];
    return rc;
}

int wtamd_pearson_moments(wtamd_trackset *ts, double *moments) {
    if (!ts || !moments) return wt_fail(WTAMD_ERR_ARG, "NULL argument");
    double r[7];
    const int rc = wt_pearson_impl(ts, r);
    if (rc == WTAMD_OK) memcpy(moments, r + 1, sizeof(double) * 6);
    return rc;
}


int wtamd_trackset_validate(wtamd_trackset *ts, int64_t *n_bad, int64_t *first_bad) {
    if (!ts || !n_bad) return wt_fail(WTAMD_ERR_ARG, "NULL argument");
    *n_bad = 0;
    if (first_bad) *first_bad = -1;
    if (ts->n_intervals <= 0) return WTAMD_OK;
    unsigned long long h[2] = {0ull, ~0ull}, *d = nullptr;
    WtDevScope scope;
    WT_HIP(scope.alloc(&d, sizeof h));
    WT_HIP(hipMemcpy(d, h, sizeof h, hipMemcpyHostToDevice));
    const long long total = ts->n_intervals;
    hipLaunchKernelGGL(wt_validate_kernel, dim3((unsigned) ((total + 255) / 256)), dim3(256), 0, nullptr, ts->d_start,
                       ts->d_finish, ts->d_seg_off, (long long) ts->n_chrom * ts->n_tracks, total, d);
    const hipError_t e = hipMemcpy(h, d, sizeof h, hipMemcpyDeviceToHost);
    if (e != hipSuccess) return wt_fail(WTAMD_ERR_HIP, "wtamd_trackset_validate: kernel / copy failed");
    *n_bad = (int64_t) h[0];
    if (first_bad && h[0]) *first_bad = (int64_t) h[1];
    return WTAMD_OK;
}

int wtamd_get_stats(const wtamd_trackset *ts_c, wtamd_stats *out) {
    if (!ts_c || !out) return wt_fail(WTAMD_ERR_ARG, "NULL argument");
    wtamd_trackset *ts = const_cast<wtamd_trackset *>(ts_c);
    if (ts->have_index_time && hipEventSynchronize(ts->ev_i1) == hipSuccess)
        (void) hipEventElapsedTime(&ts->stats.index_ms, ts->ev_i0, ts->ev_i1);
    if (ts->have_reduce_time && hipEventSynchronize(ts->ev_r1) == hipSuccess)
        (void) hipEventElapsedTime(&ts->stats.reduce_ms, ts->ev_r0, ts->ev_r1);
    *out = ts->stats;
    return WTAMD_OK;
}

}
```

### wiggletools_amd/csrc/wt_host.h

```cpp
#ifndef WT_HOST_H_
#define WT_HOST_H_

#include <hip/hip_runtime.h>

#include <chrono>
#include <cstdint>
#include <cstdio>
#include <cstdlib>
#include <string>
#include <thread>
#include <unistd.h>

#include "../../include/wiggletools_amd.h"

int wt_fail(int code, const std::string &msg);

#define WT_HIP(expr)                                                                           \
    do {                                                                                       \
        hipError_t e_ = (expr);                                                                \
        if (e_ != hipSuccess)                                                                  \
            return wt_fail(WTAMD_ERR_HIP, std::string(#expr) + ": " + hipGetErrorString(e_));  \
    } while (0)

template <class Query, class Fatal>
static inline int wt_bounded_wait(Query query, const char *call, const char *what, double nap_after_s, int nap_us, Fatal fatal) {
    const double limit_s = getenv("WTAMD_TIMEOUT_S") ? atof(getenv("WTAMD_TIMEOUT_S")) : 120.0;
    const auto t0 = std::chrono::steady_clock::now();
    for (;;) {
        const hipError_t q = query();
        if (q == hipSuccess) return WTAMD_OK;
        if (q != hipErrorNotReady) return wt_fail(WTAMD_ERR_HIP, std::string(call) + (what ? std::string(" (") + what + ")" : std::string()) + ": " + hipGetErrorString(q));
        const double el = std::chrono::duration<double>(std::chrono::steady_clock::now() - t0).count();
        if (el > limit_s) {
            fprintf(stderr, "wiggletools_amd: FATAL: %s\n", fatal(limit_s).c_str());
            fflush(stderr);
            _exit(70);
        }
        if (el > nap_after_s) std::this_thread::sleep_for(std::chrono::microseconds(nap_us));
    }
}

long long wt_map_scratch_words(long long capacity);
int wt_map_upload_chains(const wtamd_map_chain *chains, int n_tracks, void **d_out, bool *drops, bool *f32_exact);
int wt_map_chain_async(const void *d_chains, int n_tracks, bool drops, const int64_t *d_seg_in, long long n, const int32_t *start,
                       const int32_t *finish, const void *value, bool value_is_f64, unsigned long long *scratch,
                       int32_t *o_start, int32_t *o_finish, double *o_value, int64_t *d_seg_out, hipStream_t stream, bool out_f32);
long long wt_bw_scratch_bytes(long long n_sec, long long plain_stride);
long long wt_bw_fill_sections(int num_cu);
int wt_bw_decode_async(const void *h_bytes, void *d_bytes, long long n_bytes, const void *d_comp, const void *d_secs, const void *d_tracks, int n_tracks,
                       long long n_sec, long long plain_stride, void *scratch, long long capacity, int32_t *o_start, int32_t *o_finish,
                       float *o_value, int64_t *d_seg_off, unsigned long long *h_status, int copy_blocks, hipStream_t s_copy,
                       hipEvent_t e_copied, hipStream_t s_dec);
long long wt_compress_scratch_words(long long capacity);
int wt_compress_async(const int32_t *start, const int32_t *finish, const double *value, const unsigned long long *d_n,
                      long long capacity, unsigned long long *scratch, int32_t *o_start, int32_t *o_finish, double *o_value,
                      unsigned long long *d_n_out, hipStream_t s);
size_t wt_moments_partial_bytes(int blocks);
int wt_moments_async(const int32_t *start, const int32_t *finish, const double *value, long long cap, const unsigned long long *n_dev,
                     int blocks, void *d_partial, double *d_out6, hipStream_t st);
size_t wt_auc_partial_bytes(int blocks);
int wt_auc_async(const int32_t *start, const int32_t *finish, const double *value, long long n, const unsigned long long *n_dev,
                 int blocks, void *d_partial, double *d_out, bool with_span, hipStream_t st);
size_t wt_pearson_partial_bytes(int blocks);
int wt_pearson_async(const int32_t *start, const int32_t *finish, const double *tile, const uint8_t *inplay, double dx, double dy, long long n,
                     const unsigned long long *n_dev, int blocks, void *d_partial, double *d_out7, hipStream_t st);

#endif
```

### wiggletools_amd/csrc/wt_pipe.hip

```cpp
#include <hip/hip_runtime.h>

#include <algorithm>
#include <chrono>
#include <cstring>
#include <string>
#include <vector>

#include "wt_host.h"
#include "wt_trackset.h"
#include "wt_core.h"
#include "wt_plan.h"
#include "wt_bwdev_core.h"
#include "wt_pipe.h"
#include "wt_pool.h"

__global__ void __launch_bounds__(256) wt_gather_kernel(const WtGatherSeg *segs, int n_segs, long long n_chunks,
                                                         int32_t *d_start, int32_t *d_finish, float *d_value) {
    __shared__ WtGatherSeg tab[WT_GATHER_MAX_SEGS];
    {
        const long long *src = (const long long *) segs;
        long long *dst = (long long *) tab;
        const int words = n_segs * (int) (sizeof(WtGatherSeg) / 8);
        for (int i = threadIdx.x; i < words; i += 256) dst[i] = __builtin_nontemporal_load(src + i);
    }
// ... 604 lines not shown
        p->d_bw_scratches[s.bw_dec] = p->d_bw_scratch; p->bw_scratch_caps[s.bw_dec] = c;
    }
    if (!b.redo) memcpy(s.h_bw, b.bw_tracks, sizeof(wtamd_bw_track) * (size_t) N);
    s.h_bw_status[0] = ~0ull; s.h_bw_status[1] = 0;
    WT_HIP(hipEventRecord(s.e_bw0, p->s_dec));
    const int rc = wt_bw_decode_async(s.h_bw, s.d_bw, total, s.d_bw + s.bw_off_bytes, s.d_bw + s.bw_off_sec, s.d_bw, N, b.bw_secs, b.bw_stride, p->d_bw_scratch,
                                      (long long) s.dcap, s.d_start, s.d_finish, (float *) s.d_value, b.compacted ? s.d_mseg : s.ts->d_seg_off,
                                      s.h_bw_status, p->gather_blocks, p->s_copy, s.e_bwc, p->s_dec);
    if (rc != WTAMD_OK) return rc;
    WT_HIP(hipEventRecord(s.e_bw1, p->s_dec));
    s.bw_secs = b.bw_secs; s.bw_bytes = b.bw_bytes; s.bw_stride = b.bw_stride; s.bw_bound = b.n;
    s.bw_res_bytes = s.bw_res_secs = -1;
    return WTAMD_OK;
}

static int wt_pipe_upload_gather(wtamd_pipe *p, WtSlot &s, const WtBatch &b) {
    const int64_t max_segs = 2 * (int64_t) s.direct.size() + 1;
    if (s.seg_cap < max_segs) {
        if (s.h_segs) wt_host_free(s.h_segs);
        s.h_segs = nullptr; s.seg_cap = 0;
        const int64_t c = 2 * max_segs;
        WT_HIP(wt_host_alloc((void **) &s.h_segs, sizeof(WtGatherSeg) * c));
        s.seg_cap = c;
    }
    int ns = 0;
    long long chunks = 0;
    auto add = [&](const int32_t *ps, const int32_t *pf, const float *pv, int64_t dst, int64_t count) {
        if (count <= 0) return;
        s.h_segs[ns++] = WtGatherSeg{ps, pf, pv, dst, count, chunks};
        chunks += (count + WT_GATHER_CHUNK - 1) / WT_GATHER_CHUNK;
    };
    int64_t pos = 0;
    for (const auto &d : s.direct) {
        add(s.h_start + pos, s.h_finish + pos, s.h_v32 + pos, pos, d.at - pos);
        add(d.start, d.finish, d.value, d.at, d.count);
        pos = d.at + d.count;
    }
    add(s.h_start + pos, s.h_finish + pos, s.h_v32 + pos, pos, b.n - pos);
    long long grid = p->gather_blocks;
    if (grid > chunks) grid = chunks;
    if (grid < 1) grid = 1;
    hipLaunchKernelGGL(wt_gather_kernel, dim3((unsigned) grid), dim3(256), 0, p->s_copy, s.h_segs, ns, chunks,
                       s.d_start, s.d_finish, (float *) s.d_value);
    WT_HIP(hipGetLastError());
    return WTAMD_OK;
}

static int wt_pipe_upload_copies(wtamd_pipe *p, WtSlot &s, const WtBatch &b) {
    auto staged = [&](int64_t a, int64_t e) -> int {
        if (e <= a) return WTAMD_OK;
        WT_HIP(hipMemcpyAsync(s.d_start + a, s.h_start + a, sizeof(int32_t) * (e - a), hipMemcpyHostToDevice, p->s_copy));
        WT_HIP(hipMemcpyAsync(s.d_finish + a, s.h_finish + a, sizeof(int32_t) * (e - a), hipMemcpyHostToDevice, p->s_copy));
        if (b.f64) WT_HIP(hipMemcpyAsync((double *) s.d_value + a, s.h_v64 + a, sizeof(double) * (e - a), hipMemcpyHostToDevice, p->s_copy));
        else WT_HIP(hipMemcpyAsync((float *) s.d_value + a, s.h_v32 + a, sizeof(float) * (e - a), hipMemcpyHostToDevice, p->s_copy));
        return WTAMD_OK;
    };
    int64_t pos = 0;
    for (const auto &d : s.direct) {
        const int rc = staged(pos, d.at);
        if (rc != WTAMD_OK) return rc;
        WT_HIP(hipMemcpyAsync(s.d_start + d.at, d.start, sizeof(int32_t) * d.count, hipMemcpyHostToDevice, p->s_copy));
        WT_HIP(hipMemcpyAsync(s.d_finish + d.at, d.finish, sizeof(int32_t) * d.count, hipMemcpyHostToDevice, p->s_copy));
        WT_HIP(hipMemcpyAsync((float *) s.d_value + d.at, d.value, sizeof(float) * d.count, hipMemcpyHostToDevice, p->s_copy));
        pos = d.at + d.count;
    }
    return staged(pos, b.n);
}

static int wt_pipe_upload(wtamd_pipe *p, WtSlot &s, const WtBatch &b) {
    const int N = p->cfg.n_tracks;
    int rc = WTAMD_OK;
    WT_HIP(hipEventRecord(s.e_h0, p->s_copy));
    s.bw = b.bw;
    if (b.bw) {
        rc = wt_pipe_upload_bw(p, s, b);
    } else {
        WT_HIP(hipMemcpyAsync(b.compacted ? s.d_mseg : s.ts->d_seg_off, s.h_seg, sizeof(int64_t) * ((size_t) N + 1), hipMemcpyHostToDevice, p->s_copy));
        if (b.n > 0 && p->gather && !b.f64 && !s.direct.empty() && s.direct_pinned && 2 * (int64_t) s.direct.size() + 1 <= WT_GATHER_MAX_SEGS)
            rc = wt_pipe_upload_gather(p, s, b);
        else if (b.n > 0)
            rc = wt_pipe_upload_copies(p, s, b);
    }
    if (rc != WTAMD_OK) return rc;
    s.direct.clear();
    WT_HIP(hipEventRecord(s.e_h1, b.bw ? p->s_dec : p->s_copy));
    p->st.h2d_bytes += b.bw ? s.bw_off_bytes + b.bw_bytes : (int64_t) sizeof(int64_t) * (N + 1) + b.n * (b.f64 ? 16 : 12);
    return WTAMD_OK;
}

static int wt_pipe_compute(wtamd_pipe *p, WtSlot &s, const WtBatch &b) {
    wtamd_trackset *ts = s.ts;
    WT_HIP(hipStreamWaitEvent(p->s_comp, s.e_h1, 0));
    WT_HIP(hipEventRecord(s.e_k0, p->s_comp));
    if (b.mapped) {
        const int rc = wt_map_chain_async(p->d_chains, p->cfg.n_tracks, p->map_drops, b.compacted ? s.d_mseg : ts->d_seg_off, (long long) b.n, s.d_start, s.d_finish,
                                          s.d_value, b.f64, s.d_mscratch, s.d_mstart, s.d_mfinish, s.d_mvalue, ts->d_seg_off, p->s_comp, b.map_f32);
        if (rc != WTAMD_OK) return wt_fail(rc, "operator chain launch failed");
    }
    wtamd_runs runs = wt_slot_runs(s);
    s.patched = false;
    const int rc = wt_reduce_enqueue(ts, p->cfg.desc, &runs, p->tile ? s.d_tile : nullptr, p->tile ? s.d_ip : nullptr, p->s_comp, &s.used_delta, &s.delta_W);
    if (rc != WTAMD_OK) return rc;
    s.integrated = p->integrate != 0;
    s.compressed = p->compress && !s.integrated;
    return s.compressed ? wt_pipe_compress(p, s) : WTAMD_OK;
}

static int wt_pipe_submit_impl(wtamd_pipe *p, int value_is_f64, int32_t range_lo, int32_t range_hi,
                               const wtamd_bw_track *bw_tracks, int64_t bw_bytes, int64_t bw_secs, WtSlot *redo) {
    if (!p || (!redo && p->acquired < 0)) return wt_fail(WTAMD_ERR_ARG, "wtamd_pipe_submit: no acquired slot");
    WtSlot &s = redo ? *redo : p->slots[(size_t) p->acquired];
    const bool bw = bw_tracks != nullptr, f64 = value_is_f64 != 0, mapped = p->d_chains != nullptr;
    WtBatch b = {bw, f64, redo != nullptr, 0, range_lo, range_hi, bw_tracks, bw_bytes, bw_secs, redo ? s.bw_stride : 0,
                 mapped, mapped && p->map_f32 && !f64, mapped && p->map_drops};
    static const bool sdma_out = !(getenv("WTAMD_BW_EXPORT") && !strcmp(getenv("WTAMD_BW_EXPORT"), "kernel"));
    int rc = wt_pipe_check(p, s, b);
    if (rc == WTAMD_OK) rc = wt_pipe_reserve(p, s, b);
    if (rc == WTAMD_OK) rc = wt_pipe_rebind(p, s, b);
    if (rc == WTAMD_OK) rc = wt_pipe_upload(p, s, b);
    if (rc == WTAMD_OK) rc = wt_pipe_compute(p, s, b);
    if (rc != WTAMD_OK) return rc;
    s.export_pending = bw && sdma_out && !p->tile && !s.integrated;
    rc = wt_pipe_ship(p, s, s.e_cnt, p->integrate, true);
    if (rc != WTAMD_OK) return rc;

    s.n_int = b.n; s.f64 = f64; s.err = WTAMD_OK;
    if (redo) return WTAMD_OK;
    s.state = 2;
    p->acquired = -1;
    p->head = (p->head + 1) % (int) p->slots.size();
    p->in_flight++;
    p->st.batches++;
    if (!bw) p->st.intervals += b.n;
    if (s.used_delta) p->st.delta_batches++;
    return WTAMD_OK;
}

static int wt_pipe_wait_slot(wtamd_pipe *p, WtSlot &s) {
    int rc = WTAMD_OK;
    if (s.integrated) {
        rc = wt_wait_event(s.e_cnt, "batch kernels");
        if (rc == WTAMD_OK) s.ts->h_counters[WT_CTR_EXPORTED] = s.ts->h_counters[WT_CTR_RUNS];
    } else if (s.export_pending) {
        s.export_pending = false;
        rc = wt_wait_event(s.e_cnt, "batch kernels");
        if (rc == WTAMD_OK) {
            unsigned long long *hc = s.ts->h_counters;
            if (!s.compressed) hc[WT_CTR_EXPORTED] = hc[WT_CTR_RUNS];
            if ((int64_t) hc[WT_CTR_EXPORTED] > s.ocap) hc[WT_CTR_EXPORTED] = (unsigned long long) s.ocap;
            const size_t nr = (size_t) hc[WT_CTR_EXPORTED];
            const bool cz = s.compressed;
            hipError_t e = hipEventRecord(s.e_d0, p->s_out);
            if (e == hipSuccess && nr > 0) {
                e = hipMemcpyAsync(s.h_os, cz ? s.d_cs : s.d_os, sizeof(int32_t) * nr, hipMemcpyDeviceToHost, p->s_out);
                if (e == hipSuccess) e = hipMemcpyAsync(s.h_of, cz ? s.d_cf : s.d_of, sizeof(int32_t) * nr, hipMemcpyDeviceToHost, p->s_out);
                if (e == hipSuccess) e = hipMemcpyAsync(s.h_ov, cz ? s.d_cv : s.d_ov, sizeof(double) * nr, hipMemcpyDeviceToHost, p->s_out);
            }
            if (e == hipSuccess) e = hipEventRecord(s.e_d1, p->s_out);
            if (e != hipSuccess) rc = wt_fail(WTAMD_ERR_HIP, std::string("copy-engine export: ") + hipGetErrorString(e));
        }
    }
    if (rc == WTAMD_OK && !s.integrated) rc = wt_wait_event(s.e_d1, "batch");
    return rc;
}

int wtamd_pipe_collect(wtamd_pipe *p, wtamd_pipe_result *out) {
    WtDevGuard dev_guard_(p ? p->device : -1);
    if (!p || !out) return wt_fail(WTAMD_ERR_ARG, "NULL argument");
    if (p->in_flight <= 0) return wt_fail(WTAMD_ERR_ARG, "wtamd_pipe_collect: nothing in flight");
    if (p->held) return wt_fail(WTAMD_ERR_ARG, "wtamd_pipe_collect: the previous result was not released");
    WtSlot &s = p->slots[(size_t) p->tail];
    if (s.state != 2) return wt_fail(WTAMD_ERR_INTERNAL, "wtamd_pipe_collect: slot order corrupted");
    const auto t_wait0 = std::chrono::steady_clock::now();
    int rc = wt_pipe_wait_slot(p, s);
    if (rc == WTAMD_OK && s.bw && s.h_bw_status[0] == WT_BW_ERR_CAPACITY && s.dcap < s.bw_bound) {
        p->bw_density = 2.0;
        p->bw_redone++;
        rc = wt_pipe_submit_impl(p, 0, s.ts->range_lo[0], s.ts->range_hi[0], (const wtamd_bw_track *) s.h_bw, s.bw_bytes, s.bw_secs, &s);
        if (rc == WTAMD_OK) rc = wt_pipe_wait_slot(p, s);
    }
    s.state = 3;
    p->in_flight--;
    p->held = 1;
    if (rc != WTAMD_OK) return rc;
    p->last_bw_err = 0;
    if (s.bw) {
        const unsigned long long e = s.h_bw_status[0];
        if (e) {
            p->last_bw_err = e == ~0ull ? ~0u : (unsigned) e;
            std::string why = "BigWig sections could not be decoded on the device:";
            if (e == ~0ull) why += " decode kernels did not report";
            else {
                if (e & WT_BW_ERR_INFLATE) why += " corrupt zlib stream;";
                if (e & WT_BW_ERR_SECTION) why += " malformed section;";
                if (e & WT_BW_ERR_EXTENT) why += " items outside their index leaf / out of order (WTAMD_BW_DEVICE=0 selects the host decoder);";
                if (e & WT_BW_ERR_COORD) why += " coordinate above the supported maximum;";
                if (e & WT_BW_ERR_CAPACITY) why += " more intervals than the host's bound;";
            }
            return wt_fail(WTAMD_ERR_INTERNAL, why);
        }
        s.n_int = (int64_t) s.h_bw_status[1];
        if (s.bw_bound > 0 && p->bw_density < 1.0) {
            const double d = (double) s.n_int / (double) s.bw_bound;
            if (d > p->bw_density) p->bw_density = d;
        }
        p->st.intervals += s.n_int;
        p->st.bw_sections += s.bw_secs;
        float msb = 0;
        if (hipEventElapsedTime(&msb, s.e_bw0, s.e_bw1) == hipSuccess) p->st.bw_decode_ms += msb;
    }
    rc = wt_pipe_finish(p, s);
    if (rc != WTAMD_OK) return rc;
    p->st.host_wait_ms += std::chrono::duration<double, std::milli>(std::chrono::steady_clock::now() - t_wait0).count();
    float ms = 0;
    if (hipEventElapsedTime(&ms, s.e_h0, s.e_h1) == hipSuccess) p->st.h2d_ms += ms;
    if (hipEventElapsedTime(&ms, s.e_k0, s.e_cnt) == hipSuccess) p->st.kernel_ms += ms;
    if (!s.integrated && hipEventElapsedTime(&ms, s.e_d0, s.e_d1) == hipSuccess) p->st.d2h_ms += ms;
    p->st.runs += s.n_runs;
    p->st.covered_bp += s.covered;
    p->st.d2h_bytes += s.integrated ? (int64_t) (sizeof(unsigned long long) * WT_CTR_N + 48) : s.n_runs * (16 + (p->tile ? 9 * (int64_t) p->cfg.n_tracks : 0));
    out->n_runs = s.n_runs;
    out->integ_valid = s.integrated ? 1 : 0;
    out->reserved = 0;
    for (int k = 0; k < 6; k++) out->integ[k] = s.integrated ? s.h_integ[k] : 0.0;
    if (s.integrated && !p->tile && s.integ_mode != 2) { out->integ[2] = out->integ[3] = out->integ[4] = out->integ[5] = 0.0; }
    out->start = s.integrated ? nullptr : s.h_os; out->finish = s.integrated ? nullptr : s.h_of; out->value = s.integrated ? nullptr : s.h_ov;
    out->tile = (p->tile && !s.integrated) ? s.h_tile : nullptr;
    out->inplay = (p->tile && !s.integrated) ? s.h_ip : nullptr;
    out->covered_bp = s.covered;
    out->n_intervals = s.n_int;
    return WTAMD_OK;
}

int wtamd_pipe_release(wtamd_pipe *p) {
    if (!p || !p->held) return wt_fail(WTAMD_ERR_ARG, "wtamd_pipe_release: nothing to release");
    p->slots[(size_t) p->tail].state = 0;
    p->held = 0;
    p->tail = (p->tail + 1) % (int) p->slots.size();
    return WTAMD_OK;
}

int wtamd_pipe_in_flight(const wtamd_pipe *p) { return p ? p->in_flight : 0; }

int wtamd_pipe_set_compress(wtamd_pipe *p, int on) {
    if (!p) return wt_fail(WTAMD_ERR_ARG, "NULL argument");
    if (on && p->tile) return wt_fail(WTAMD_ERR_ARG, "wtamd_pipe_set_compress: the Multiplexer tile cannot be compressed");
    p->compress = on != 0;
    return WTAMD_OK;
}

int wtamd_pipe_set_integrate(wtamd_pipe *p, int on) {
    if (!p) return wt_fail(WTAMD_ERR_ARG, "NULL argument");
    if (on && p->tile && p->cfg.n_tracks != 2) return wt_fail(WTAMD_ERR_ARG, "the fused Pearson integrator needs a Multiplexer of exactly two tracks");
    if (on == 2 && p->tile) return wt_fail(WTAMD_ERR_ARG, "wtamd_pipe_set_integrate: mode 2 (run moments) needs a reducer, not a Multiplexer tile");
    p->integrate = on == 2 ? 2 : on != 0;
    return WTAMD_OK;
}

int wtamd_pipe_integrate_modes(const wtamd_pipe *p) {
    if (!p) return 0;
    return p->tile ? 1 : 2;
}

int wtamd_pipe_integrate_held(wtamd_pipe *p, double *integ) {
    WtDevGuard dev_guard_(p ? p->device : -1);
    if (!p || !integ) return wt_fail(WTAMD_ERR_ARG, "NULL argument");
    if (!p->held) return wt_fail(WTAMD_ERR_ARG, "wtamd_pipe_integrate_held: no collected batch");
    WtSlot &s = p->slots[(size_t) p->tail];
    for (int k = 0; k < 6; k++) integ[k] = 0.0;
    const int mode = p->integrate == 2 ? 2 : 1;
    if (!s.integrated || s.integ_mode != mode) {
        int rc = wt_pipe_enqueue_integ(p, s, p->s_comp, mode);
        if (rc != WTAMD_OK) return rc;
        WT_HIP(hipEventRecord(s.e_patch, p->s_comp));
        rc = wt_wait_event(s.e_patch, "integrals of the held batch");
        if (rc != WTAMD_OK) return rc;
    }
    for (int k = 0; k < (p->tile || mode == 2 ? 6 : 2); k++) integ[k] = s.h_integ[k];
    return WTAMD_OK;
}

int wtamd_pipe_set_map(wtamd_pipe *p, const wtamd_map_chain *chains) {
    WtDevGuard dev_guard_(p ? p->device : -1);
    if (!p) return wt_fail(WTAMD_ERR_ARG, "NULL argument");
    if (p->in_flight > 0 || p->acquired >= 0) return wt_fail(WTAMD_ERR_ARG, "wtamd_pipe_set_map: batches in flight");
    if (p->d_chains) { (void) wt_dev_free(p->d_chains); p->d_chains = nullptr; p->map_drops = false; p->map_f32 = false; }
    if (!chains) return WTAMD_OK;
    bool any = false;
    for (int t = 0; t < p->cfg.n_tracks; t++) any = any || chains[t].n_ops != 0;
    if (!any) return WTAMD_OK;
    return wt_map_upload_chains(chains, p->cfg.n_tracks, &p->d_chains, &p->map_drops, &p->map_f32);
}

void *wtamd_host_alloc(size_t bytes) {
    void *q = nullptr;
    if (wt_host_alloc(&q, bytes ? bytes : 1) != hipSuccess) return nullptr;
    return q;
}

void wtamd_host_free(void *q) {
    if (q) wt_host_free(q);
}

void wtamd_pool_trim(void) {
    std::vector<void *> host, dev;
    {
        std::lock_guard<std::mutex> lk(g_pinned_pool.mu);
        for (auto &kv : g_pinned_pool.free_list) { host.push_back(kv.second); g_pinned_pool.size_of.erase(kv.second); }
        g_pinned_pool.free_list.clear();
        g_pinned_pool.pooled = 0;
    }
    {
        std::lock_guard<std::mutex> lk(g_dev_pool.mu);
        for (auto &kv : g_dev_pool.free_list) { dev.push_back(kv.second); g_dev_pool.size_of.erase(kv.second); }
        g_dev_pool.free_list.clear();
        g_dev_pool.pooled = 0;
    }
    for (void *x : host) wt_pin_raw_free(x);
    for (void *x : dev) (void) hipFree(x);
}

void wtamd_pool_stats(int64_t out[6]) {
    if (!out) return;
    {
        std::lock_guard<std::mutex> lk(g_pinned_pool.mu);
        out[0] = (int64_t) g_pinned_pool.misses; out[1] = (int64_t) g_pinned_pool.miss_bytes; out[2] = (int64_t) g_pinned_pool.pooled;
    }
    std::lock_guard<std::mutex> lk(g_dev_pool.mu);
    out[3] = (int64_t) g_dev_pool.misses; out[4] = (int64_t) g_dev_pool.miss_bytes; out[5] = (int64_t) g_dev_pool.pooled;
}

int wtamd_pipe_get_stats(const wtamd_pipe *p, wtamd_pipe_stats *out) {
    if (!p || !out) return wt_fail(WTAMD_ERR_ARG, "NULL argument");
    *out = p->st;
    return WTAMD_OK;
}

}
```

### wiggletools_amd/csrc/wt_plan.h

```cpp
#ifndef WT_PLAN_H_
#define WT_PLAN_H_

#include <algorithm>
#include <cmath>
#include <cstdint>
#include <cstdlib>
#include <cstring>
#include <string>
#include <vector>

#include "wt_core.h"

struct WtPlan {
    int W = 0;
    int T = 0;
    int n_words = 0;
    int spitch = 0, cpitch = 0, count_segs = 8;
    int chunk_tracks = 0, n_chunks = 1;
    int lanes_per_pos = 1;
    int off_acc = 0, off_ev = 0, off_ltv = 0, off_ltc = 0, off_gtv = 0, off_gtc = 0, off_tbase = 0, off_tpfx = 0, off_tfirst = 0, off_dsh = 0, off_tdef = 0;
    int off_qa = 0, off_ltq = 0, off_gtq = 0, delta_q = 0;
    int delta_ns = 1;
    bool delta = false;
    int off_S = 0, off_cnt = 0, off_segtot = 0, off_U = 0, off_cover = 0, off_E = 0, off_epfx = 0, off_nextw = 0, off_gbase = 0, off_scratch = 0, off_shared = 0;
// ... 52 lines not shown
    p.lds_bytes = o;
}

static inline bool wt_op_is_var_family(int op) {
    return op == WT_OP_VAR || op == WT_OP_STDDEV || op == WT_OP_ENTROPY || op == WT_OP_CV;
}

static inline void wt_make_delta_plan(WtPlan &p, int n_tracks, bool squares = false, bool two_sets = false) {
    if (two_sets) squares = true;
    const char *eT = getenv("WTAMD_DELTA_T");
    const int T0 = squares ? WT_DELTA_SQ_T0 : 1024;
    int T = eT ? atoi(eT) : T0;
    (void) n_tracks;
    const int Tmax = squares ? WT_DELTA_SQ_T0 : WT_MAX_DELTA_T;
    if (T < 64 || T > Tmax || ((T & (T - 1)) && !(squares && T > 512 && T % 64 == 0))) T = T0;
    if (squares && !eT) {
        const char *eS = getenv("WTAMD_DELTA_SQ_T");
        if (eS && atoi(eS) >= 512 && atoi(eS) <= Tmax && atoi(eS) % 64 == 0) T = atoi(eS);
    }
    int TS = squares && T > 512 ? 512 : T;
    const int ns = two_sets ? 2 : 1;
    if (two_sets) {
        const char *e2 = getenv("WTAMD_DELTA_TT_W");
        TS = (e2 && atoi(e2) == 1024) ? 128 : 256;
        if (T < 2 * TS) T = 2 * TS;
    }
    p = WtPlan();
    p.delta = true;
    p.delta_ns = ns;
    p.T = T; p.ppt = WT_DELTA_K; p.W = WT_DELTA_K * TS; p.n_words = p.W / 64;
    p.chunk_tracks = 0; p.n_chunks = 1;
    int o = 0;
    p.off_acc = o;    o = wt_align16(o + (ns * p.W + p.W / 32) * 8);
    p.off_ev = o;     o = wt_align16(o + (ns * p.W + p.W / 32) * 4);
    p.off_U = o;      o = wt_align16(o + p.n_words * 8);
    p.off_E = o;      o = wt_align16(o + p.n_words * 8);
    p.off_epfx = o;   o = wt_align16(o + std::max(p.n_words + 1, 48) * 4);
    p.off_nextw = o;  o = wt_align16(o + p.n_words * 2);
    p.off_ltv = o;    o = wt_align16(o + ns * TS * 8);
    p.off_ltc = o;    o = wt_align16(o + std::max(T, ns * TS) * 4);
    p.off_gtv = o;    o = wt_align16(o + ns * (TS / WT_DELTA_GROUP) * 8);
    p.off_gtc = o;    o = wt_align16(o + (std::max(T, ns * TS) / WT_DELTA_GROUP) * 4);
    p.off_tbase = o;  o = wt_align16(o + T * 8);
    p.off_tpfx = o;   o = wt_align16(o + (T + 1) * 4);
    p.off_tfirst = o; o = wt_align16(o + WT_DELTA_TF * 2);
    p.off_tdef = o;   o = wt_align16(o + (squares ? 0 : T * 4));
    p.off_dsh = o;    o = wt_align16(o + (int) sizeof(WtDeltaShared));
    p.delta_q = squares ? 1 : 0;
    if (squares) {
        p.off_qa = o;  o = wt_align16(o + 2 * ns * p.W * 8);
        p.off_ltq = o; o = wt_align16(o + 2 * ns * TS * 8);
        p.off_gtq = o; o = wt_align16(o + 2 * ns * (TS / WT_DELTA_GROUP) * 8);
    }
    p.off_shared = o; o = wt_align16(o + (int) sizeof(WtShared));
    p.lds_bytes = o;
}

static inline bool wt_defaults_fit_f32(const double *d, int n);

static inline void wt_make_delta_plan_for(WtPlan &p, int n_tracks, int op) {
    wt_make_delta_plan(p, n_tracks, wt_op_is_var_family(op), op == WT_OP_TTEST);
}

static inline bool wt_delta_eligible(int op, bool value_f64, int n_tracks, const double *defaults) {
    if (getenv("WTAMD_NO_DELTA")) return false;
    const bool sq = wt_op_is_var_family(op);
    if (op == WT_OP_TTEST) {
        return !getenv("WTAMD_NO_DELTA_TTEST") && !value_f64 && n_tracks >= 8 && n_tracks <= 32767 && wt_defaults_fit_f32(defaults, n_tracks);
    }
    const bool mm = op == WT_OP_MAX || op == WT_OP_MIN;
    if (mm && getenv("WTAMD_NO_DELTA_MINMAX")) return false;
    if (op != WT_OP_SUM && op != WT_OP_MEAN && !sq && !mm) return false;
    if (sq && (n_tracks < 8 || getenv("WTAMD_NO_DELTA_VAR"))) return false;
    const char *eM = getenv("WTAMD_DELTA_MIN_TRACKS");
    const int min_tracks = eM ? atoi(eM) : 4;
    if (value_f64 || n_tracks < min_tracks || n_tracks > 32767) return false;
    for (int i = 0; i < n_tracks; i++) {
        if (defaults[i] == 0.0) continue;
        if (sq || mm || getenv("WTAMD_NO_DELTA_DEFAULTS")) return false;
        const float f = (float) defaults[i];
        if (!((double) f == defaults[i]) || !(f - f == 0.0f)) return false;
    }
    return true;
}

static inline void wt_delta_defaults_params(const double *defaults, int n_tracks, WtParams &P) {
    P.delta_df = 0; P.def_emin = 255; P.def_emax = 0;
    if (P.op == WT_OP_TTEST) return;
    for (int i = 0; i < n_tracks; i++) {
        if (defaults[i] == 0.0) continue;
        const float f = (float) defaults[i];
        uint32_t bits;
        memcpy(&bits, &f, 4);
        int e = (int) ((bits >> 23) & 0xffu);
        if (e == 0) e = 1;
        P.delta_df = 1;
        if (e < P.def_emin) P.def_emin = e;
        if (e > P.def_emax) P.def_emax = e;
    }
}

static inline bool wt_make_walk_plan(WtPlan &p, int n_tracks, int nr, double events_per_bp, int hard_limit = 160 * 1024, int mwu_n_set0 = -1) {
    const char *eT = getenv("WTAMD_WALK_T"), *eS = getenv("WTAMD_WALK_S"), *eP = getenv("WTAMD_WALK_PAIR");
    const bool mwu = mwu_n_set0 >= 0;
    const int n_big = mwu ? std::max(mwu_n_set0, n_tracks - mwu_n_set0) : 0;
    if (mwu && (mwu_n_set0 < 1 || n_tracks - mwu_n_set0 < 1 || n_big > 64)) return false;
    const int pair = mwu ? 1 : (eP ? (atoi(eP) != 0 ? 1 : 0) : WT_WALK_PAIR_DEFAULT);
    const int wantT = eT ? atoi(eT) : 256, wantS = eS ? atoi(eS) : (pair ? 16 : 32);
    struct Cand { int T, S; bool half_cu; };
    for (const Cand cd : {Cand{wantT, wantS, pair != 0}, Cand{128, 16, pair != 0}, Cand{64, 32, pair != 0},
                          Cand{wantT, wantS, false}, Cand{wantT, 16, false}, Cand{256, 16, false}, Cand{128, 16, false}, Cand{64, 16, false}}) {
        const int T = cd.T, S = cd.S;
        if (cd.half_cu && (eT || eS) && (T != wantT || S != wantS)) continue;
        if (T != 64 && T != 128 && T != 256 && !(pair && T == 512)) continue;
        if (S != 4 && S != 8 && S != 16 && S != 32) continue;
        if (n_tracks > T) continue;
        WtPlan q;
        q.T = T; q.W = (T >> pair) * S; q.n_words = q.W / 64; q.ppt = S; q.walk_S = S; q.regcol = nr; q.walk_pair = pair; q.walk_mwu = mwu ? 1 : 0;
        if (q.W < 64) continue;
        q.chunk_tracks = n_tracks; q.n_chunks = 1;
        int o = 0;
        q.off_wcol = o;   o = wt_align16(o + (((mwu ? n_big : (pair ? (n_tracks + 1) / 2 : n_tracks)) + 7) & ~7) * T * 4);
        q.off_wcnt = o;   o = wt_align16(o + q.W * 4);
        q.off_woff = 0;
        q.off_wtot = o;   o = wt_align16(o + T * 4);
        q.off_wbase = o;  o = wt_align16(o + (T + 1) * 4);
        q.off_wgt = o;    o = wt_align16(o + (T / 64 + 1) * 4);
        q.off_wncov = o;  o = wt_align16(o + T * 4);
        q.off_wfe = o;    o = wt_align16(o + T * 4);
        q.off_wdk = o;    o = wt_align16(o + n_tracks * 4);
        q.off_wguess = o; o = wt_align16(o + 8);
        q.off_tbase = o;  o = wt_align16(o + T * 8);
        q.off_ltc = o;    o = wt_align16(o + T * 4);
        q.off_gtc = o;    o = wt_align16(o + (T / WT_DELTA_GROUP + 1) * 4);
        q.off_tpfx = o;   o = wt_align16(o + (T + 1) * 4);
        q.off_tfirst = o; o = wt_align16(o + WT_WALK_TF * 2);
        q.off_shared = o; o = wt_align16(o + (int) sizeof(WtShared));
        q.lds_bytes = o;
        if (q.lds_bytes > hard_limit - 1024) continue;
        if (cd.half_cu && q.lds_bytes > hard_limit / 2 - 512) continue;
        int capp = 16;
        if (events_per_bp > 0) {
            capp = 8;
            while (capp < 64 && capp < 2.5 * events_per_bp) capp <<= 1;
        }
        if (const char *eC = getenv("WTAMD_WALK_CAPP")) { const int c = atoi(eC); if (c >= 1 && c <= 64 && !(c & (c - 1))) capp = c; }
        long long ov = 2048;
        if (const char *eO = getenv("WTAMD_WALK_OV")) { const long long c = atoll(eO); if (c >= 0) ov = c; }
        q.walk_capp = capp;
        q.walk_ov = (int) ov;
        long long bytes = (long long) q.W * capp * 8 + (ov > 8 ? ov : 8) * 12;
        const long long lane_max = 2ll * n_tracks * S * 8;
        if (bytes < lane_max) bytes = lane_max;
        bytes = (bytes + 255) & ~255ll;
        q.walk_off_at = (int) bytes;
        q.scratch_slab = (bytes + (long long) (q.W + 1) * 4 + 255) & ~255ll;
        p = q;
        return true;
    }
    return false;
}

static inline int wt_regcol_slots(int n_tracks, int op, bool scratch_f32, int n_set0) {
    if (!scratch_f32 || getenv("WTAMD_NO_REGCOL")) return 0;
    if (getenv("WTAMD_CHUNK") || getenv("WTAMD_GLOBAL_SCRATCH") || getenv("WTAMD_PPT") || getenv("WTAMD_T") || getenv("WTAMD_MWU_LPP1"))
        return 0;
    int need = 0;
    if (op == WT_OP_MEDIAN) need = n_tracks;
    else if (op == WT_OP_MWU) need = 2 * std::max(n_set0, n_tracks - n_set0);
    else return 0;
    if (op == WT_OP_MWU && (n_set0 < 1 || n_set0 >= n_tracks)) return 0;
    for (int nr : {32, 64, 128})
        if (need <= nr) return nr;
    return 0;
}

static inline bool wt_make_plan(int n_tracks, int op, bool scratch_f32, WtPlan &out, std::string &err,
                                int soft_limit = 80 * 1024, int hard_limit = 160 * 1024, int n_set0 = 0) {
    const char *eP = getenv("WTAMD_PPT");
    if (const int nr = wt_regcol_slots(n_tracks, op, scratch_f32, n_set0)) {
        WtPlan p;
        const int kk = 2;
        wt_carve(n_tracks, op, 256 * kk, 256, 4, p, 0, false, nr, n_set0);
        p.ppt = kk;
        p.lanes_per_pos = 1;
        if (p.n_chunks == 1 && p.lds_bytes <= hard_limit / 2 - 512) { out = p; return true; }
    }
    const char *eT = getenv("WTAMD_T");
    const bool scr = wt_op_needs_scratch(op);
    const int scratch_elem = scr ? (scratch_f32 ? 4 : 8) : 0;
    struct Cand { int ppt, T, lpp; };
    std::vector<Cand> cands;
    if (eP || eT) {
        const int ppt = scr ? 1 : (eP ? atoi(eP) : 4);
        const int T = eT ? atoi(eT) : 256;
        if ((ppt == 1 || ppt == 4) && T >= 64 && T <= 512 && !(T & (T - 1))) cands.push_back({ppt, T, 1});
    }
    if (cands.empty()) {
        if (op == WT_OP_MWU && !getenv("WTAMD_MWU_LPP1")) cands = {{1, 512, 2}, {1, 256, 2}, {1, 128, 2}, {1, 64, 1}};
        else if (scr) cands = {{1, 256, 1}, {1, 128, 1}, {1, 64, 1}};
        else cands = {{4, 512, 1}, {4, 256, 1}, {1, 512, 1}, {1, 256, 1}, {1, 128, 1}, {1, 64, 1}};
    }
    const int limit = hard_limit - 1024;
    const int half = hard_limit / 2 - 512;
    (void) soft_limit;
    const char *eC = getenv("WTAMD_CHUNK");
    auto try_plan = [&](const Cand &cd, int chunk, int lim, bool glob = false) -> bool {
        WtPlan p;
        wt_carve(n_tracks, scr ? op : WT_OP_SUM, cd.ppt * cd.T / cd.lpp, cd.T, scratch_elem, p, chunk, glob);
        p.ppt = cd.ppt;
        p.lanes_per_pos = cd.lpp;
        if (p.lds_bytes > lim) return false;
        out = p;
        return true;
    };
    auto max_chunk = [&](const Cand &cd, int lim, bool glob = false) -> int {
        int lo = 0, hi = n_tracks;
        while (lo < hi) {
            const int mid = (lo + hi + 1) / 2;
            WtPlan p;
            wt_carve(n_tracks, scr ? op : WT_OP_SUM, cd.ppt * cd.T / cd.lpp, cd.T, scratch_elem, p, mid, glob);
            if (p.lds_bytes <= lim) lo = mid; else hi = mid - 1;
        }
        return lo;
    };
    const bool eG = scr && getenv("WTAMD_GLOBAL_SCRATCH");
    if (eC || eG) {
        for (const Cand &cd : cands)
            if (try_plan(cd, eC ? atoi(eC) : 0, limit, eG)) return true;
    } else if (!scr) {
        const Cand &cd = cands[0];
        if (try_plan(cd, 0, half)) return true;
        const int best = max_chunk(cd, half);
        if (best >= 16) {
            const int n_chunks = (n_tracks + best - 1) / best;
            if (try_plan(cd, (n_tracks + n_chunks - 1) / n_chunks, half)) return true;
        }
        for (const Cand &c2 : cands)
            if (try_plan(c2, 0, limit)) return true;
    } else {
        if (op == WT_OP_MWU && cands.size() > 1 && try_plan({1, 256, 1}, 0, half)) return true;
        for (const Cand &cd : cands)
            if (try_plan(cd, 0, limit)) return true;
        for (const Cand &cd : cands) {
            const int best = max_chunk(cd, half, true);
            if (best < 1) continue;
            const int n_chunks = (n_tracks + best - 1) / best;
            if (try_plan(cd, (n_tracks + n_chunks - 1) / n_chunks, half, true)) return true;
        }
    }
    err = "no LDS plan fits " + std::to_string(n_tracks) + " tracks (op " + std::to_string(op) + ")";
    return false;
}

static inline int wt_mwu_wrap_mul(int a, int b) { return (int) ((unsigned) a * (unsigned) b); }
static inline bool wt_mwu_make_table(int n1, int n2, std::vector<double> &t) {
    const double mu = (double) (wt_mwu_wrap_mul(n1, n2) / 2);
    const double sigma = sqrt((double) (wt_mwu_wrap_mul(wt_mwu_wrap_mul(n1, n2), (int) ((unsigned) n1 + (unsigned) n2 + 1u)) / 12));
    t.clear();
    if (sigma != sigma) { t.push_back(sigma); return true; }
    const int cap = 1 << 20;
    for (int k = 0; k < cap; k++) {
        const double U1 = mu + 0.5 * (double) k;
        const double v = k == 0 ? 2 * erf((U1 - mu) / sigma) : 2 * erf((mu - U1) / sigma);
        t.push_back(v);
        if (v == -2.0) return true;
    }
    t.clear();
    return false;
}

static inline void wt_plan_to_params(const WtPlan &p, WtParams &P) {
    P.W = p.W; P.n_words = p.n_words; P.spitch = p.spitch; P.cpitch = p.cpitch; P.count_segs = p.count_segs;
    P.chunk_tracks = p.chunk_tracks; P.n_chunks = p.n_chunks;
    P.g_scratch = nullptr; P.g_scratch_slab = p.scratch_slab; P.g_attr_slab = p.attr_slab;
    P.logW = 0;
    while ((1 << P.logW) < p.W) P.logW++;
    P.off_S = p.off_S; P.off_cnt = p.off_cnt; P.off_segtot = p.off_segtot; P.off_U = p.off_U; P.off_cover = p.off_cover; P.off_E = p.off_E;
    P.off_epfx = p.off_epfx; P.off_nextw = p.off_nextw; P.off_gbase = p.off_gbase; P.off_scratch = p.off_scratch;
    P.off_dflt32 = p.off_dflt32;
    P.off_acc = p.off_acc; P.off_ev = p.off_ev; P.off_ltv = p.off_ltv; P.off_ltc = p.off_ltc;
    P.off_gtv = p.off_gtv; P.off_gtc = p.off_gtc; P.off_tbase = p.off_tbase; P.off_tpfx = p.off_tpfx; P.off_tfirst = p.off_tfirst; P.off_dsh = p.off_dsh; P.off_tdef = p.off_tdef;
    P.delta_df = 0; P.def_emin = 255; P.def_emax = 0;
    P.off_qa = p.off_qa; P.off_ltq = p.off_ltq; P.off_gtq = p.off_gtq; P.delta_q = p.delta_q; P.delta_ns = p.delta_ns;
    P.off_wcol = p.off_wcol; P.off_wcnt = p.off_wcnt; P.off_woff = p.off_woff; P.off_wtot = p.off_wtot; P.off_wbase = p.off_wbase;
    P.off_wgt = p.off_wgt; P.off_wncov = p.off_wncov; P.off_wfe = p.off_wfe; P.off_wdk = p.off_wdk; P.walk_S = p.walk_S;
    P.off_wguess = p.off_wguess; P.walk_capp = p.walk_capp; P.walk_ov = p.walk_ov; P.walk_off_at = p.walk_off_at; P.walk_pair = p.walk_pair;
    P.walk_mwu = p.walk_mwu;
    P.off_shared = p.off_shared; P.lds_bytes = p.lds_bytes;
}

struct WtWindowTables {
    std::vector<int32_t> cbase, c_nwin, c_hi, win_chrom;
    std::vector<int64_t> c_first_win;
    std::vector<int> empty_chrom;
    int64_t n_windows = 0;
    int64_t n_rows = 0;
    int64_t span_bp = 0;
};

static inline void wt_make_windows(int n_chrom, int n_tracks, const int64_t *seg_off,
                                   const int32_t *first_start, const int32_t *last_finish, int W,
                                   WtWindowTables &t, const int32_t *range_lo = nullptr,
                                   const int32_t *range_hi = nullptr) {
    t.cbase.assign(n_chrom, 0);
    t.c_nwin.assign(n_chrom, 1);
    t.c_hi.assign(n_chrom, INT32_MAX);
    t.c_first_win.assign(n_chrom + 1, 0);
    t.win_chrom.clear();
    t.empty_chrom.clear();
    t.span_bp = 0;
    for (int c = 0; c < n_chrom; c++) {
        int64_t lo = INT64_MAX, hi = INT64_MIN;
        for (int i = 0; i < n_tracks; i++) {
            const int64_t s = (int64_t) c * n_tracks + i;
            if (seg_off[s + 1] > seg_off[s]) {
                lo = std::min<int64_t>(lo, first_start[s]);
                hi = std::max<int64_t>(hi, last_finish[s]);
            }
        }
        int64_t nw = 1;
        if (lo <= hi) {
            const int64_t data_hi = hi;
            if (range_lo && range_lo[c] > lo) lo = range_lo[c];
            if (range_hi && range_hi[c] != INT32_MAX && range_hi[c] < hi) hi = range_hi[c];
            if (lo < hi) {
                t.cbase[c] = (int32_t) lo;
                nw = std::max<int64_t>(1, (hi - lo + W - 1) / W);
                t.span_bp += hi - lo;
            } else {
                t.cbase[c] = (int32_t) std::min<int64_t>(data_hi, INT32_MAX - 65536);
                t.empty_chrom.push_back(c);
            }
        }
        t.c_nwin[c] = (int32_t) nw;
        if (range_hi) t.c_hi[c] = range_hi[c];
        t.c_first_win[c + 1] = t.c_first_win[c] + nw;
        for (int64_t m = 0; m < nw; m++) t.win_chrom.push_back(c);
    }
    t.n_windows = t.c_first_win[n_chrom];
    t.n_rows = t.n_windows + n_chrom;
}

template <int OP, int K, class F>
static inline void wt_dispatch_types2(bool value_f64, bool scratch_f32, bool multi, F &f) {
    if (multi) {
        if (value_f64) f.template run<OP, double, double, K, true>();
        else if (!scratch_f32) f.template run<OP, float, double, K, true>();
        else f.template run<OP, float, float, K, true>();
    } else {
        if (value_f64) f.template run<OP, double, double, K, false>();
        else if (!scratch_f32) f.template run<OP, float, double, K, false>();
        else f.template run<OP, float, float, K, false>();
    }
}

template <int OP, class F>
static inline void wt_dispatch_op(bool value_f64, bool scratch_f32, int ppt, bool multi, F &f, int regcol = 0) {
    if constexpr (OP == WT_OP_MEDIAN || OP == WT_OP_MWU) {
        if (regcol && !value_f64 && scratch_f32 && !multi) {
            if (regcol == 32) f.template run<OP, float, float, 2, false, 32>();
            else if (regcol == 64) f.template run<OP, float, float, 2, false, 64>();
            else f.template run<OP, float, float, 2, false, 128>();
            return;
        }
    }
    if (wt_op_needs_scratch(OP) || ppt == 1) wt_dispatch_types2<OP, 1>(value_f64, scratch_f32, multi, f);
    else wt_dispatch_types2<OP, 4>(value_f64, scratch_f32, multi, f);
}

template <int... OPS, class F>
static inline bool wt_dispatch_ops(int op, bool value_f64, bool scratch_f32, int ppt, bool multi, F &f, int regcol = 0) {
    if (op == WT_OP_ENTROPY) op = WT_OP_STDDEV;
    return ((op == OPS ? (wt_dispatch_op<OPS>(value_f64, scratch_f32, ppt, multi, f, regcol), true) : false) || ...);
}

template <class F>
static inline bool wt_dispatch(int op, bool value_f64, bool scratch_f32, int ppt, bool multi, F &f, int regcol = 0) {
    return wt_dispatch_ops<WT_OP_SUM, WT_OP_PRODUCT, WT_OP_MEAN, WT_OP_VAR, WT_OP_STDDEV, WT_OP_CV, WT_OP_MIN, WT_OP_MAX, WT_OP_MEDIAN, WT_OP_TTEST, WT_OP_MWU,
                           WT_OP_MULTIPLEX>(op, value_f64, scratch_f32, ppt, multi, f, regcol);
}

static inline bool wt_defaults_fit_f32(const double *d, int n) {
    for (int i = 0; i < n; i++) {
        if (d[i] != d[i]) continue;
        if ((double) (float) d[i] != d[i]) return false;
    }
    return true;
}

static inline bool wt_pick_general_plan(int n_tracks, int op, bool value_f64, bool scratch_f32, int n_set0, bool median_walk, bool mwu_walk,
                                        double events_per_bp, WtPlan &plan, std::string &err) {
    if (op == WT_OP_MEDIAN && !value_f64 && median_walk)
        if (const int nr = wt_regcol_slots(n_tracks, op, scratch_f32, n_set0))
            if (wt_make_walk_plan(plan, n_tracks, nr, events_per_bp)) return true;
    if (op == WT_OP_MWU && !value_f64 && mwu_walk)
        if (const int nr = wt_regcol_slots(n_tracks, op, scratch_f32, n_set0))
            if (wt_make_walk_plan(plan, n_tracks, nr, events_per_bp, 160 * 1024, n_set0)) return true;
    return wt_make_plan(n_tracks, op, scratch_f32, plan, err, 80 * 1024, 160 * 1024, n_set0);
}

static inline bool wt_patch_compatible(const WtPlan &general, int delta_W, bool scratch_f32, bool value_f64) {
    return !(general.scratch_slab > 0 || general.W > delta_W || delta_W % general.W != 0 || delta_W / general.W > WT_BAD_SUB || !scratch_f32 || value_f64);
}

static inline bool wt_few_enough_to_patch(long long n_bad, long long n_windows) { return n_bad * 4 <= n_windows; }

#endif
```

### wiggletools_amd/csrc/wt_pool.h

```cpp
#ifndef WT_POOL_H_
#define WT_POOL_H_

#include <sys/mman.h>

#include <atomic>
#include <cstring>
#include <map>
#include <mutex>
#include <vector>

#include "wt_host.h"

static bool wt_is_registered(const void *q);
static bool wt_is_pinned(const void *q) {
    if (wt_is_registered(q)) return true;
    hipPointerAttribute_t a;
    if (hipPointerGetAttributes(&a, q) != hipSuccess) { (void) hipGetLastError(); return false; }
    return a.type == hipMemoryTypeHost;
}

struct WtPinnedPool {
    std::mutex mu;
    std::multimap<size_t, void *> free_list;
    std::map<void *, size_t> size_of;
    size_t pooled = 0;
    size_t misses = 0, miss_bytes = 0;
    size_t limit() const {
        const char *e = getenv("WTAMD_PINNED_POOL_MB");
        return (size_t) (e ? atoll(e) : 8192) << 20;
    }
};
static WtPinnedPool g_pinned_pool;

static size_t wt_pool_round(size_t bytes) {
    if (bytes < (1u << 20)) return bytes;
    int lg = 63;
    while (!((bytes >> lg) & 1u)) lg--;
    const size_t step = (size_t) 1 << (lg - 3);
    return (bytes + step - 1) / step * step;
}

struct WtRegistered { void *base; size_t map_len; size_t len; };
static std::mutex g_reg_mu;
static std::map<void *, WtRegistered> g_registered;
static std::atomic<int> g_reg_state{0};
static std::atomic<int> g_reg_failures{0};

static bool wt_is_registered(const void *q) {
    std::lock_guard<std::mutex> lk(g_reg_mu);
    auto it = g_registered.upper_bound((void *) q);
    if (it == g_registered.begin()) return false;
    --it;
    return (const char *) q < (const char *) it->first + it->second.len;
}

static int wt_pin_threads() {
    static const int n = [] {
        int c = (int) std::thread::hardware_concurrency();
        if (FILE *fp = fopen("/sys/fs/cgroup/cpu.max", "r")) {
            char q[64]; long long period = 0;
            if (fscanf(fp, "%63s %lld", q, &period) == 2 && period > 0 && strcmp(q, "max") != 0) {
                const long long k = atoll(q) / period;
                if (k >= 1 && k < c) c = (int) k;
            }
            fclose(fp);
        }
        return c < 1 ? 1 : (c > 16 ? 16 : c);
    }();
    return n;
}

static bool wt_pin_by_register(void **out, size_t bytes) {
    static const bool off = getenv("WTAMD_PIN") && !strcmp(getenv("WTAMD_PIN"), "malloc");
    if (off || g_reg_state.load() < 0 || bytes < ((size_t) 2 << 20)) return false;
    const size_t huge = (size_t) 2 << 20;
    const size_t len = (bytes + huge - 1) / huge * huge;
    void *base = mmap(nullptr, len + huge, PROT_READ | PROT_WRITE, MAP_PRIVATE | MAP_ANONYMOUS, -1, 0);
    if (base == MAP_FAILED) return false;
    char *p = (char *) (((uintptr_t) base + huge - 1) & ~(uintptr_t) (huge - 1));
#ifdef MADV_HUGEPAGE
    (void) madvise(p, len, MADV_HUGEPAGE);
#endif
    int T = wt_pin_threads();
    const size_t per_thread_min = (size_t) 32 << 20;
    if ((size_t) T > len / per_thread_min) T = (int) (len / per_thread_min);
    if (T < 1) T = 1;
    const size_t slice = (len / (size_t) T + huge - 1) / huge * huge;
    auto touch = [p, len, slice](int t) {
        const size_t a = slice * (size_t) t, b = a + slice < len ? a + slice : len;
        for (size_t q = a; q < b; q += 4096) ((volatile char *) p)[q] = 0;
    };
    std::vector<std::thread> th;
    for (int t = 1; t < T; t++) th.emplace_back(touch, t);
    touch(0);
    for (auto &t : th) t.join();
    void *dp = nullptr;
    const bool registered = hipHostRegister(p, len, hipHostRegisterDefault) == hipSuccess;
    if (!registered || hipHostGetDevicePointer(&dp, p, 0) != hipSuccess || dp != (void *) p) {
        (void) hipGetLastError();
        const bool never = registered;
        if (registered) (void) hipHostUnregister(p);
        munmap(base, len + huge);
        if (never || g_reg_failures.fetch_add(1) + 1 >= 3) g_reg_state.store(-1);
        return false;
    }
    g_reg_state.store(1);
    g_reg_failures.store(0);
    { std::lock_guard<std::mutex> lk(g_reg_mu); g_registered[p] = WtRegistered{base, len + huge, len}; }
    *out = p;
    return true;
}

static hipError_t wt_pin_raw_alloc(void **out, size_t bytes) {
    if (wt_pin_by_register(out, bytes)) return hipSuccess;
    return hipHostMalloc(out, bytes, hipHostMallocDefault);
}

static void wt_pin_raw_free(void *q) {
    WtRegistered r{nullptr, 0};
    {
        std::lock_guard<std::mutex> lk(g_reg_mu);
        auto it = g_registered.find(q);
        if (it != g_registered.end()) { r = it->second; g_registered.erase(it); }
    }
    if (r.base) { (void) hipHostUnregister(q); munmap(r.base, r.map_len); }
    else (void) hipHostFree(q);
}

static hipError_t wt_host_alloc(void **out, size_t bytes) {
    if (bytes < 1) bytes = 1;
    bytes = wt_pool_round(bytes);
    if (bytes >= (1u << 20)) {
        std::lock_guard<std::mutex> lk(g_pinned_pool.mu);
        auto it = g_pinned_pool.free_list.lower_bound(bytes);
        if (it != g_pinned_pool.free_list.end() && it->first <= bytes + bytes / 4) {
            *out = it->second;
            g_pinned_pool.pooled -= it->first;
            g_pinned_pool.free_list.erase(it);
            return hipSuccess;
        }
    }
    const auto t_alloc0 = std::chrono::steady_clock::now();
    hipError_t e = wt_pin_raw_alloc(out, bytes);
    if (e != hipSuccess) {
        std::vector<void *> idle;
        {
            std::lock_guard<std::mutex> lk(g_pinned_pool.mu);
            for (auto &kv : g_pinned_pool.free_list) { idle.push_back(kv.second); g_pinned_pool.size_of.erase(kv.second); }
            g_pinned_pool.free_list.clear();
            g_pinned_pool.pooled = 0;
        }
        if (!idle.empty()) {
            (void) hipGetLastError();
            for (void *x : idle) wt_pin_raw_free(x);
            e = wt_pin_raw_alloc(out, bytes);
        }
    }
    if (e == hipSuccess && bytes >= (1u << 20)) {
        std::lock_guard<std::mutex> lk(g_pinned_pool.mu);
        g_pinned_pool.size_of[*out] = bytes;
        g_pinned_pool.misses++;
        g_pinned_pool.miss_bytes += bytes;
        static const bool trace = getenv("WTAMD_TRACE_POOL") != nullptr;
        bool by_register = false;
        if (trace) { std::lock_guard<std::mutex> lk2(g_reg_mu); by_register = g_registered.count(*out) != 0; }
        if (trace) fprintf(stderr, "[pool] page-locked %.1f MB (%s) in %.1f ms\n", bytes / 1048576.0, by_register ? "mmap + hipHostRegister" : "hipHostMalloc",
                           std::chrono::duration<double, std::milli>(std::chrono::steady_clock::now() - t_alloc0).count());
    }
    return e;
}

static void wt_host_free(void *q) {
    if (!q) return;
    {
        std::lock_guard<std::mutex> lk(g_pinned_pool.mu);
        auto it = g_pinned_pool.size_of.find(q);
        if (it != g_pinned_pool.size_of.end()) {
            if (g_pinned_pool.pooled + it->second <= g_pinned_pool.limit()) {
                g_pinned_pool.free_list.emplace(it->second, q);
                g_pinned_pool.pooled += it->second;
                return;
            }
            g_pinned_pool.size_of.erase(it);
        }
    }
    wt_pin_raw_free(q);
}

struct WtDevPool {
    std::mutex mu;
    std::multimap<std::pair<int, size_t>, void *> free_list;
    std::map<void *, std::pair<int, size_t>> size_of;
    size_t pooled = 0, misses = 0, miss_bytes = 0;
    size_t limit() const {
        const char *e = getenv("WTAMD_DEVICE_POOL_MB");
        return (size_t) (e ? atoll(e) : 65536) << 20;
    }
};
static WtDevPool g_dev_pool;

template <class T>
static hipError_t wt_dev_alloc(T **out, size_t bytes, int line = __builtin_LINE()) {
    if (bytes < 1) bytes = 1;
    bytes = wt_pool_round(bytes);
    int dev = 0;
    (void) hipGetDevice(&dev);
    {
        std::lock_guard<std::mutex> lk(g_dev_pool.mu);
        auto it = g_dev_pool.free_list.lower_bound({dev, bytes});
        if (it != g_dev_pool.free_list.end() && it->first.first == dev && it->first.second <= bytes + bytes / 4) {
            *out = (T *) it->second;
            g_dev_pool.pooled -= it->first.second;
            g_dev_pool.free_list.erase(it);
            return hipSuccess;
        }
    }
    void *q = nullptr;
    const auto t_alloc0 = std::chrono::steady_clock::now();
    hipError_t e = hipMalloc(&q, bytes);
    if (e != hipSuccess) {
        std::vector<void *> idle;
        {
            std::lock_guard<std::mutex> lk(g_dev_pool.mu);
            for (auto &kv : g_dev_pool.free_list) { idle.push_back(kv.second); g_dev_pool.size_of.erase(kv.second); }
            g_dev_pool.free_list.clear();
            g_dev_pool.pooled = 0;
        }
        if (!idle.empty()) {
            (void) hipGetLastError();
            for (void *x : idle) (void) hipFree(x);
            e = hipMalloc(&q, bytes);
        }
    }
    *out = (T *) q;
    if (e == hipSuccess) {
        std::lock_guard<std::mutex> lk(g_dev_pool.mu);
        g_dev_pool.size_of[q] = {dev, bytes};
        g_dev_pool.misses++;
        g_dev_pool.miss_bytes += bytes;
        static const bool trace = getenv("WTAMD_TRACE_POOL") != nullptr;
        if (trace && bytes >= (1u << 20)) fprintf(stderr, "[pool] hipMalloc %.1f MB in %.1f ms (device %d, wt_pipe.hip:%d)\n", bytes / 1048576.0,
                                                  std::chrono::duration<double, std::milli>(std::chrono::steady_clock::now() - t_alloc0).count(), dev, line);
    }
    return e;
}

static hipError_t wt_dev_free(void *q) {
    if (!q) return hipSuccess;
    {
        std::lock_guard<std::mutex> lk(g_dev_pool.mu);
        auto it = g_dev_pool.size_of.find(q);
        if (it != g_dev_pool.size_of.end()) {
            if (g_dev_pool.pooled + it->second.second <= g_dev_pool.limit()) {
                g_dev_pool.free_list.emplace(it->second, q);
                g_dev_pool.pooled += it->second.second;
                return hipSuccess;
            }
            g_dev_pool.size_of.erase(it);
        }
    }
    return hipFree(q);
}

#endif
```

### wiggletools_amd/csrc/wt_trackset.h

```cpp
#ifndef WT_TRACKSET_H_
#define WT_TRACKSET_H_

#include <map>
#include <vector>

#include "wt_host.h"
#include "wt_plan.h"

struct WtWindows {
    WtPlan plan_geom;
    WtWindowTables tab;
    int32_t *d_cbase = nullptr, *d_cnwin = nullptr, *d_chi = nullptr, *d_win_chrom = nullptr;
    int64_t *d_cfirst = nullptr;
    uint32_t *d_widx = nullptr;
    uint32_t *d_cidx = nullptr;
    unsigned long long *d_status = nullptr;
    int32_t *d_bad_list = nullptr;
    long long *d_bad_goff = nullptr;
    bool indexed = false;
    int64_t cap_chrom = 0, cap_win = 0, cap_widx = 0, cap_bad = 0, cap_cidx = 0;
    bool tab_valid = false;
    int64_t *h_tab = nullptr;
    char *d_tabs = nullptr;
    int64_t cap_tabs = 0;
};

struct wtamd_trackset {
    int n_chrom = 0, n_tracks = 0;
    bool value_f64 = false;
    bool owns = false;
    int64_t n_intervals = 0;
    std::vector<int64_t> seg_off;
    std::vector<double> defaults;
    std::vector<int32_t> first_start, last_finish;
    std::vector<int32_t> range_lo, range_hi;
    int32_t *d_start = nullptr, *d_finish = nullptr;
    void *d_value = nullptr;
    int64_t *d_seg_off = nullptr;
    double *d_defaults = nullptr;
    unsigned long long *d_counters = nullptr;
    unsigned long long *h_counters = nullptr;
    unsigned long long *h_debug = nullptr;
    int64_t *d_chrom_run_off = nullptr;
    char *d_gscratch = nullptr;
    size_t gscratch_bytes = 0;
    double *d_mwu_table = nullptr;
    int mwu_n1 = -1, mwu_n2 = -1, mwu_kmax = 0;
    int mwu_few_ties = -1;
    std::vector<double *> mwu_retired;
    std::map<int, WtWindows> windows;
    hipEvent_t ev_i0 = nullptr, ev_i1 = nullptr, ev_r0 = nullptr, ev_r1 = nullptr;
    bool have_index_time = false, have_reduce_time = false;
    wtamd_stats stats{};
    int device = 0;
    int num_cu = 256;
    bool scratch_f32 = false;
    bool delta_failed_[3] = {false, false, false};
    bool delta_verified_[3] = {false, false, false};
    long long delta_n_bad_[3] = {0, 0, 0};
    bool pipe_mode = false;
};

void wt_warmup_join();
int wt_trackset_common(const wtamd_tracks *t, wtamd_trackset *ts);
int wt_check_extents(wtamd_trackset *ts);
int wt_check_desc(const wtamd_trackset *ts, const wtamd_reduce_desc *d);

int wt_trackset_rebind(wtamd_trackset *ts, int64_t n, const int64_t *seg_off, int32_t range_lo, int32_t range_hi, bool value_f64,
                       int32_t *d_start, int32_t *d_finish, void *d_value, bool delta_failed);

int wt_reduce_enqueue(wtamd_trackset *ts, const wtamd_reduce_desc &desc, wtamd_runs *runs, double *d_tile, uint8_t *d_inplay,
                      hipStream_t s, bool *used_delta, int *delta_W);

int wt_launch_patch(wtamd_trackset *ts, int delta_W, int op, uint32_t flags, int n_set0, wtamd_runs *runs, long long n_bad,
                    hipStream_t s);

#endif
```

Baseline: 44.68 billion.

## Add pooled device/pinned allocators, interpolation index search, async extents and window tables

Introduces a shared pool module for device and page-locked host allocations. Scoped and trackset allocations, previously raw hipMalloc/hipFree, now go through it and synchronize via a device quiesce before reuse. The index search kernels switch to an interpolation-guided lower bound with a fast path for single-chromosome sets. Extents are now computed on a stream into persistent buffers, and window tables gain async upload events and new clear and win-chrom kernels. The goal is to cut allocation and synchronization overhead and search cost per call, at the price of global device synchronizations on free and more complex buffer lifetimes.

After: 49.00 billion (median of 6 runs). +9.7%, better.

```diff
diff --git a/wiggletools_amd/csrc/build.py b/wiggletools_amd/csrc/build.py
--- a/wiggletools_amd/csrc/build.py
+++ b/wiggletools_amd/csrc/build.py
@@ -5,7 +5,7 @@
 HERE = os.path.dirname(os.path.abspath(__file__))
 SO = os.path.join(HERE, "libwiggletools_amd.so")
 KERNEL_SRCS = ["wt_reduce_stream.hip", "wt_reduce_moments.hip", "wt_reduce_order.hip", "wt_patch_kernels.hip", "wt_delta_kernels.hip", "wt_walk.hip"]
-SRCS = KERNEL_SRCS + ["wt_engine.hip", "wt_pipe.hip", "wt_compress.hip", "wt_moments.hip", "wt_map.hip", "wt_cover.hip", "wt_region.hip", "wt_synth.hip", "wt_bwdev.hip", "wt_defaults.cpp", "wt_iter_abi.cpp", "wt_bigwig.cpp", "wt_bwwrite.cpp"]
+SRCS = KERNEL_SRCS + ["wt_engine.hip", "wt_pool.hip", "wt_pipe.hip", "wt_compress.hip", "wt_moments.hip", "wt_map.hip", "wt_cover.hip", "wt_region.hip", "wt_synth.hip", "wt_bwdev.hip", "wt_defaults.cpp", "wt_iter_abi.cpp", "wt_bigwig.cpp", "wt_bwwrite.cpp"]
 LIBS = ["-lz"]
 FLAGS = ["--offload-arch=gfx950", "-O3", "-std=c++17", "-fPIC", "-shared", "-ffp-contract=off",
          "-Wall", "-Wno-unused-function", "-Wno-pass-failed"]
diff --git a/wiggletools_amd/csrc/wt_core.h b/wiggletools_amd/csrc/wt_core.h
--- a/wiggletools_amd/csrc/wt_core.h
+++ b/wiggletools_amd/csrc/wt_core.h
@@ -1589,31 +1589,7 @@
         for (long long m = m_hi + 1; m <= c.nw; m++) P.widx[(size_t) (c.rowbase + m) * N + c.i] = (uint32_t) (jr + 1);
 }
 
-WT_DEV long long wt_lane_lower_bound(const int32_t *fin, long long lo, long long hi, long long g, long long b) {
-    if (lo >= hi) return lo;
-    if ((long long) fin[g] >= b) {
-        hi = g;
-        for (long long d = 1;; d <<= 1) {
-            const long long q = hi - d;
-            if (q < lo) break;
-            if ((long long) fin[q] < b) { lo = q + 1; break; }
-            hi = q;
-        }
-    } else {
-        lo = g + 1;
-        for (long long d = 1;; d <<= 1) {
-            const long long q = lo + d - 1;
-            if (q >= hi) break;
-            if ((long long) fin[q] >= b) { hi = q; break; }
-            lo = q + 1;
-        }
-    }
-    while (lo < hi) {
-        const long long mid = (lo + hi) >> 1;
-        if ((long long) fin[mid] < b) lo = mid + 1; else hi = mid;
-    }
-    return lo;
-}
+#include "wt_isearch.h"
 
 #include "wt_delta.h"
 #include "wt_walk.h"
diff --git a/wiggletools_amd/csrc/wt_devscope.h b/wiggletools_amd/csrc/wt_devscope.h
--- a/wiggletools_amd/csrc/wt_devscope.h
+++ b/wiggletools_amd/csrc/wt_devscope.h
@@ -3,6 +3,8 @@
 #include <hip/hip_runtime.h>
 
 #include <vector>
+
+#include "wt_pool.h"
 
 struct WtDevScope {
     std::vector<void *> ptrs;
@@ -10,14 +12,16 @@
     WtDevScope(const WtDevScope &) = delete;
     WtDevScope &operator=(const WtDevScope &) = delete;
     template <class T>
-    hipError_t alloc(T **p, size_t bytes) {
+    hipError_t alloc(T **p, size_t bytes, const char *file = __builtin_FILE(), int line = __builtin_LINE()) {
         void *q = nullptr;
-        const hipError_t e = hipMalloc(&q, bytes ? bytes : 1);
+        const hipError_t e = wt_dev_alloc_bytes(&q, bytes ? bytes : 1, file, line);
         if (e == hipSuccess) { ptrs.push_back(q); *p = (T *) q; }
         return e;
     }
     ~WtDevScope() {
-        for (void *q : ptrs) (void) hipFree(q);
+        if (ptrs.empty()) return;
+        (void) wt_pool_quiesce();
+        for (void *q : ptrs) (void) wt_dev_free(q);
     }
 };
 
diff --git a/wiggletools_amd/csrc/wt_engine.hip b/wiggletools_amd/csrc/wt_engine.hip
--- a/wiggletools_amd/csrc/wt_engine.hip
+++ b/wiggletools_amd/csrc/wt_engine.hip
@@ -15,6 +15,7 @@
 #include "wt_plan.h"
 #include "wt_kernels.h"
 #include "wt_devscope.h"
+#include "wt_pool.h"
 
 #ifndef WT_INDEX_UNROLL
 #define WT_INDEX_UNROLL 2
@@ -91,25 +92,45 @@
     return lo;
 }
 
+struct WtIndexRow { int ch; long long b, s0, n; };
+__device__ __forceinline__ WtIndexRow wt_index_row(const WtParams &P, long long row, int i) {
+    WtIndexRow r;
+    r.ch = P.n_chrom == 1 ? 0 : wt_index_row_chrom(P, row);
+    const long long m = row - (P.c_first_win[r.ch] + r.ch);
+    const long long seg = (long long) r.ch * P.n_tracks + i;
+    r.s0 = P.seg_off[seg];
+    r.n = P.seg_off[seg + 1] - r.s0;
+    r.b = (long long) P.cbase[r.ch] + (m << P.logW);
+    return r;
+}
+
 __global__ void __launch_bounds__(256) wt_index_coarse_kernel(const WtParams P, long long n_strips, uint32_t *coarse) {
     const long long t = (long long) blockIdx.x * 256 + threadIdx.x;
     const int N = P.n_tracks;
     if (t >= n_strips * N) return;
     const long long strip = t / N;
     const int i = (int) (t - strip * N);
-    const long long row = strip * WT_ISEARCH_ROWS;
-    const int ch = wt_index_row_chrom(P, row);
-    const long long m = row - (P.c_first_win[ch] + ch);
-    const long long seg = (long long) ch * N + i;
-    const long long s0 = P.seg_off[seg], n = P.seg_off[seg + 1] - s0;
-    const long long b = (long long) P.cbase[ch] + (m << P.logW);
-    coarse[t] = (uint32_t) wt_lane_lower_bound(P.finish + s0, 0, n, n >> 1, b);
+    const WtIndexRow r = wt_index_row(P, strip * WT_ISEARCH_ROWS, i);
+    const int32_t *fin = P.finish + r.s0;
+    long long g = r.n >> 1;
+    float density = 0.0f;
+    if (r.n > 1) {
+        const long long f0 = fin[0], f1 = fin[r.n - 1];
+        if (f1 > f0) {
+            density = (float) (r.n - 1) / (float) (f1 - f0);
+            const float guess = fminf(fmaxf((float) (r.b - f0) * density, 0.0f), (float) (r.n - 1));
+            g = (long long) guess;
+            if (g > r.n - 1) g = r.n - 1;
+        }
+    }
+    coarse[t] = (uint32_t) wt_interp_lower_bound(WtFinArray{fin}, 0, r.n, g, r.b, density);
 }
 
 __global__ void __launch_bounds__(WT_ISEARCH_ROWS * WT_ISEARCH_TRACKS) wt_index_search_kernel(const WtParams P, long long n_rows, long long n_strips,
                                                                                               const uint32_t *coarse) {
     __shared__ uint32_t out[WT_ISEARCH_ROWS][WT_ISEARCH_TRACKS + 1];
-    const int tid = threadIdx.x, lane = tid & 63, wave = tid >> 6;
+    const int tid = threadIdx.x, lane = tid & 63;
+    const int wave = __builtin_amdgcn_readfirstlane(tid >> 6);
     const int N = P.n_tracks;
     const long long strip = blockIdx.x;
     const long long r0 = strip * WT_ISEARCH_ROWS;
@@ -117,21 +138,23 @@
     if (i < N) {
         long long row = r0 + lane;
         if (row > n_rows - 1) row = n_rows - 1;
-        const int ch = wt_index_row_chrom(P, row);
-        const long long m = row - (P.c_first_win[ch] + ch);
-        const long long seg = (long long) ch * N + i;
-        const long long s0 = P.seg_off[seg], n = P.seg_off[seg + 1] - s0;
-        const long long b = (long long) P.cbase[ch] + (m << P.logW);
-        const int32_t *fin = P.finish + s0;
-        const int ch_first = __shfl(ch, 0);
+        const WtIndexRow r = wt_index_row(P, row, i);
+        const int32_t *fin = P.finish + r.s0;
         const bool have_next = strip + 1 < n_strips;
-        const int ch_next = have_next ? wt_index_row_chrom(P, r0 + WT_ISEARCH_ROWS) : -1;
-        const bool real_a = ch == ch_first, real_b = ch == ch_next;
-        const long long A = real_a ? (long long) coarse[strip * N + i] : 0;
-        const long long B = real_b ? (long long) coarse[(strip + 1) * N + i] : n;
+        const long long cA = (long long) coarse[strip * N + i];
+        const long long cB = have_next ? (long long) coarse[(strip + 1) * N + i] : 0;
+        bool real_a = true, real_b = have_next;
+        if (P.n_chrom != 1) {
+            const int ch_first = __shfl(r.ch, 0);
+            const int ch_next = have_next ? wt_index_row_chrom(P, r0 + WT_ISEARCH_ROWS) : -1;
+            real_a = r.ch == ch_first; real_b = r.ch == ch_next;
+        }
+        const long long A = real_a ? cA : 0;
+        const long long B = real_b ? cB : r.n;
         long long g = (real_a && real_b) ? A + (((B - A) * lane) >> 6) : (A + B) >> 1;
         if (g > B - 1) g = B - 1;
-        out[lane][wave] = (uint32_t) wt_lane_lower_bound(fin, A, B, g, b);
+        const float density = (real_a && real_b) ? (float) (B - A) / (float) ((long long) WT_ISEARCH_ROWS << P.logW) : 0.0f;
+        out[lane][wave] = (uint32_t) wt_interp_lower_bound(WtFinArray{fin}, A, B, g, r.b, density);
     }
     __syncthreads();
     const int orow = tid / WT_ISEARCH_TRACKS, ocol = tid % WT_ISEARCH_TRACKS;
@@ -153,6 +176,25 @@
     const long long lo = seg_off[s], hi = seg_off[s + 1];
     first_start[s] = hi > lo ? start[lo] : 0;
     last_finish[s] = hi > lo ? finish[hi - 1] : 0;
+}
+
+__global__ void __launch_bounds__(256) wt_win_chrom_kernel(const int64_t *c_first_win, int n_chrom, long long n_windows, int32_t *win_chrom) {
+    const long long k = (long long) blockIdx.x * 256 + threadIdx.x;
+    if (k >= n_windows) return;
+    int lo = 0;
+    for (int hi = n_chrom; hi - lo > 1;) {
+        const int mid = (lo + hi) >> 1;
+        if (c_first_win[mid] <= k) lo = mid; else hi = mid;
+    }
+    win_chrom[k] = lo;
+}
+
+__global__ void __launch_bounds__(256) wt_clear_kernel(unsigned long long *counters, int n_counters, int64_t *chrom_run_off, int n_cro,
+                                                        unsigned long long *status, long long n_status) {
+    const long long t = (long long) blockIdx.x * 256 + threadIdx.x, stride = (long long) gridDim.x * 256;
+    for (long long q = t; q < n_status; q += stride) status[q] = 0ull;
+    for (long long q = t; q < n_counters; q += stride) counters[q] = 0ull;
+    for (long long q = t; q < n_cro; q += stride) chrom_run_off[q] = 0;
 }
 
 __global__ void __launch_bounds__(256) wt_validate_kernel(const int32_t *start, const int32_t *finish, const int64_t *seg_off,
@@ -182,22 +224,30 @@
 }
 
 template <class T>
-static hipError_t wt_grow(T **p, int64_t *cap, int64_t need) {
+static hipError_t wt_grow(T **p, int64_t *cap, int64_t need, bool *quiet) {
     if (*cap >= need && *p) return hipSuccess;
     int64_t c = *cap * 2;
     if (c < need) c = need;
     if (c < 1) c = 1;
-    (void) hipFree(*p);
+    if (*p) {
+        if (!*quiet) {
+            const hipError_t eq = wt_pool_quiesce();
+            if (eq != hipSuccess) return eq;
+            *quiet = true;
+        }
+        (void) wt_dev_free(*p);
+    }
     *p = nullptr; *cap = 0;
-    const hipError_t e = hipMalloc((void **) p, sizeof(T) * (size_t) c);
+    const hipError_t e = wt_dev_alloc(p, sizeof(T) * (size_t) c);
     if (e == hipSuccess) *cap = c;
     return e;
 }
 
 static void wt_free_windows(WtWindows &w) {
-    (void) hipFree(w.d_tabs);
-    (void) hipFree(w.d_widx); (void) hipFree(w.d_cidx); (void) hipFree(w.d_status); (void) hipFree(w.d_bad_list); (void) hipFree(w.d_bad_goff);
-    if (w.h_tab) (void) hipHostFree(w.h_tab);
+    (void) wt_dev_free(w.d_tabs);
+    (void) wt_dev_free(w.d_widx); (void) wt_dev_free(w.d_cidx); (void) wt_dev_free(w.d_status); (void) wt_dev_free(w.d_bad_list); (void) wt_dev_free(w.d_bad_goff);
+    if (w.h_tab) wt_host_free(w.h_tab);
+    if (w.ev_tab) (void) hipEventDestroy(w.ev_tab);
     w = WtWindows();
 }
 
@@ -285,15 +335,15 @@
     hipDeviceProp_t prop;
     WT_HIP(hipGetDeviceProperties(&prop, ts->device));
     ts->num_cu = prop.multiProcessorCount;
-    WT_HIP(hipMalloc(&ts->d_seg_off, sizeof(int64_t) * (n_seg + 1)));
+    WT_HIP(wt_dev_alloc(&ts->d_seg_off, sizeof(int64_t) * (n_seg + 1)));
     WT_HIP(hipMemcpy(ts->d_seg_off, ts->seg_off.data(), sizeof(int64_t) * (n_seg + 1), hipMemcpyHostToDevice));
-    WT_HIP(hipMalloc(&ts->d_defaults, sizeof(double) * t->n_tracks));
+    WT_HIP(wt_dev_alloc(&ts->d_defaults, sizeof(double) * t->n_tracks));
     WT_HIP(hipMemcpy(ts->d_defaults, ts->defaults.data(), sizeof(double) * t->n_tracks, hipMemcpyHostToDevice));
-    WT_HIP(hipMalloc(&ts->d_counters, sizeof(unsigned long long) * WT_CTR_N));
-    WT_HIP(hipHostMalloc(&ts->h_counters, sizeof(unsigned long long) * WT_CTR_N));
-    WT_HIP(hipHostMalloc(&ts->h_debug, sizeof(unsigned long long) * 16));
+    WT_HIP(wt_dev_alloc(&ts->d_counters, sizeof(unsigned long long) * WT_CTR_N));
+    WT_HIP(wt_host_alloc((void **) &ts->h_counters, sizeof(unsigned long long) * WT_CTR_N));
+    WT_HIP(wt_host_alloc((void **) &ts->h_debug, sizeof(unsigned long long) * 16));
     memset(ts->h_debug, 0, sizeof(unsigned long long) * 16);
-    WT_HIP(hipMalloc(&ts->d_chrom_run_off, sizeof(int64_t) * (t->n_chrom + 1)));
+    WT_HIP(wt_dev_alloc(&ts->d_chrom_run_off, sizeof(int64_t) * (t->n_chrom + 1)));
     WT_HIP(hipEventCreate(&ts->ev_i0));
     WT_HIP(hipEventCreate(&ts->ev_i1));
     WT_HIP(hipEventCreate(&ts->ev_r0));
@@ -311,20 +361,21 @@
     return WTAMD_OK;
 }
 
-static int wt_refresh_extents_device(wtamd_trackset *ts) {
+static int wt_refresh_extents_device(wtamd_trackset *ts, hipStream_t s) {
     const int64_t n_seg = (int64_t) ts->n_chrom * ts->n_tracks;
     ts->first_start.assign(n_seg, 0);
     ts->last_finish.assign(n_seg, 0);
     if (n_seg > 0 && ts->n_intervals > 0) {
-        int32_t *d_fs = nullptr, *d_lf = nullptr;
-        WtDevScope scope;
-        WT_HIP(scope.alloc(&d_fs, sizeof(int32_t) * n_seg));
-        WT_HIP(scope.alloc(&d_lf, sizeof(int32_t) * n_seg));
-        hipLaunchKernelGGL(wt_extents_kernel, dim3((unsigned) ((n_seg + 255) / 256)), dim3(256), 0, 0,
-                           ts->d_seg_off, ts->d_start, ts->d_finish, (long long) n_seg, d_fs, d_lf);
+        const size_t bytes = sizeof(int32_t) * 2 * (size_t) n_seg;
+        if (!ts->d_extents) WT_HIP(wt_dev_alloc(&ts->d_extents, bytes));
+        if (!ts->h_extents) WT_HIP(wt_host_alloc((void **) &ts->h_extents, bytes));
+        hipLaunchKernelGGL(wt_extents_kernel, dim3((unsigned) ((n_seg + 255) / 256)), dim3(256), 0, s,
+                           ts->d_seg_off, ts->d_start, ts->d_finish, (long long) n_seg, ts->d_extents, ts->d_extents + n_seg);
         WT_HIP(hipGetLastError());
-        WT_HIP(hipMemcpy(ts->first_start.data(), d_fs, sizeof(int32_t) * n_seg, hipMemcpyDeviceToHost));
-        WT_HIP(hipMemcpy(ts->last_finish.data(), d_lf, sizeof(int32_t) * n_seg, hipMemcpyDeviceToHost));
+        WT_HIP(hipMemcpyAsync(ts->h_extents, ts->d_extents, bytes, hipMemcpyDeviceToHost, s));
+        WT_HIP(hipStreamSynchronize(s));
+        ts->first_start.assign(ts->h_extents, ts->h_extents + n_seg);
+        ts->last_finish.assign(ts->h_extents + n_seg, ts->h_extents + 2 * n_seg);
     }
     return WTAMD_OK;
 }
@@ -372,7 +423,7 @@
     ts->d_start = const_cast<int32_t *>(t->start);
     ts->d_finish = const_cast<int32_t *>(t->finish);
     ts->d_value = const_cast<void *>(t->value);
-    rc = wt_refresh_extents_device(ts);
+    rc = wt_refresh_extents_device(ts, nullptr);
     if (rc != WTAMD_OK) return rc;
     return wt_check_extents(ts);
 }
@@ -388,11 +439,15 @@
 
 void wtamd_trackset_destroy(wtamd_trackset *ts) {
     if (!ts) return;
+    (void) wt_pool_quiesce();
     if (ts->owns) { (void) hipFree(ts->d_start); (void) hipFree(ts->d_finish); (void) hipFree(ts->d_value); }
-    (void) hipFree(ts->d_seg_off); (void) hipFree(ts->d_defaults); (void) hipFree(ts->d_counters); (void) hipFree(ts->d_chrom_run_off); (void) hipFree(ts->d_gscratch); (void) hipFree(ts->d_mwu_table);
+    (void) wt_dev_free(ts->d_seg_off); (void) wt_dev_free(ts->d_defaults); (void) wt_dev_free(ts->d_counters); (void) wt_dev_free(ts->d_chrom_run_off);
+    (void) wt_dev_free(ts->d_extents);
+    (void) hipFree(ts->d_gscratch); (void) hipFree(ts->d_mwu_table);
     for (double *q : ts->mwu_retired) (void) hipFree(q);
-    if (ts->h_counters) (void) hipHostFree(ts->h_counters);
-    if (ts->h_debug) (void) hipHostFree(ts->h_debug);
+    if (ts->h_counters) wt_host_free(ts->h_counters);
+    if (ts->h_debug) wt_host_free(ts->h_debug);
+    if (ts->h_extents) wt_host_free(ts->h_extents);
     for (auto &kv : ts->windows) wt_free_windows(kv.second);
     if (ts->ev_i0) (void) hipEventDestroy(ts->ev_i0);
     if (ts->ev_i1) (void) hipEventDestroy(ts->ev_i1);
@@ -428,52 +483,62 @@
     if (w.tab_valid) return WTAMD_OK;
     wt_make_windows(ts->n_chrom, ts->n_tracks, ts->seg_off.data(), ts->first_start.data(), ts->last_finish.data(), W, w.tab,
                     ts->range_lo.empty() ? nullptr : ts->range_lo.data(),
-                    ts->range_hi.empty() ? nullptr : ts->range_hi.data());
+                    ts->range_hi.empty() ? nullptr : ts->range_hi.data(), false);
     w.indexed = false;
     const int64_t nc = ts->n_chrom > 0 ? ts->n_chrom : 1;
     const int64_t nwin = w.tab.n_windows > 0 ? w.tab.n_windows : 1;
     const int64_t nwidx = (w.tab.n_rows > 0 ? w.tab.n_rows : 1) * (int64_t) ts->n_tracks;
     auto up8 = [](int64_t x) { return (x + 7) & ~(int64_t) 7; };
+    bool quiet = false;
     if (w.cap_chrom < nc || w.cap_win < nwin || !w.d_tabs) {
         const int64_t cc = w.cap_chrom < nc ? std::max<int64_t>(nc, 2 * w.cap_chrom) : w.cap_chrom;
         const int64_t cw = w.cap_win < nwin ? std::max<int64_t>(nwin, 2 * w.cap_win) : w.cap_win;
         const int64_t o_cnwin = up8(4 * cc), o_chi = o_cnwin + up8(4 * cc), o_cfirst = o_chi + up8(4 * cc), o_win = o_cfirst + 8 * (cc + 1);
         const int64_t total = o_win + up8(4 * cw);
-        (void) hipFree(w.d_tabs);
+        if (w.d_tabs || w.d_status) { WT_HIP(wt_pool_quiesce()); quiet = true; }
+        (void) wt_dev_free(w.d_tabs);
         w.d_tabs = nullptr; w.cap_tabs = 0;
         w.d_cbase = w.d_cnwin = w.d_chi = w.d_win_chrom = nullptr; w.d_cfirst = nullptr;
-        if (w.cap_win < cw) { (void) hipFree(w.d_status); w.d_status = nullptr; }
+        if (w.cap_win < cw) { (void) wt_dev_free(w.d_status); w.d_status = nullptr; }
         w.cap_chrom = 0; w.cap_win = 0;
-        WT_HIP(hipMalloc((void **) &w.d_tabs, (size_t) total));
-        if (!w.d_status) WT_HIP(hipMalloc((void **) &w.d_status, sizeof(unsigned long long) * (size_t) cw));
+        WT_HIP(wt_dev_alloc(&w.d_tabs, (size_t) total));
+        if (!w.d_status) WT_HIP(wt_dev_alloc(&w.d_status, sizeof(unsigned long long) * (size_t) cw));
         w.cap_tabs = total;
         w.d_cbase = (int32_t *) w.d_tabs; w.d_cnwin = (int32_t *) (w.d_tabs + o_cnwin); w.d_chi = (int32_t *) (w.d_tabs + o_chi);
         w.d_cfirst = (int64_t *) (w.d_tabs + o_cfirst); w.d_win_chrom = (int32_t *) (w.d_tabs + o_win);
         w.cap_chrom = cc; w.cap_win = cw;
     }
-    WT_HIP(wt_grow(&w.d_widx, &w.cap_widx, nwidx));
-    WT_HIP(wt_grow(&w.d_cidx, &w.cap_cidx, ((w.tab.n_rows > 0 ? w.tab.n_rows : 1) + WT_ISEARCH_ROWS - 1) / WT_ISEARCH_ROWS * (int64_t) ts->n_tracks));
+    WT_HIP(wt_grow(&w.d_widx, &w.cap_widx, nwidx, &quiet));
+    WT_HIP(wt_grow(&w.d_cidx, &w.cap_cidx, ((w.tab.n_rows > 0 ? w.tab.n_rows : 1) + WT_ISEARCH_ROWS - 1) / WT_ISEARCH_ROWS * (int64_t) ts->n_tracks, &quiet));
     if (ts->n_chrom > 0) {
-        if (ts->pipe_mode) {
-            if (ts->n_chrom != 1) return wt_fail(WTAMD_ERR_INTERNAL, "pipeline slots hold one chromosome");
-            if (!w.h_tab) WT_HIP(hipHostMalloc((void **) &w.h_tab, 64, hipHostMallocDefault));
-            int32_t *h32 = (int32_t *) w.h_tab;
-            h32[0] = w.tab.cbase[0]; h32[1] = w.tab.c_nwin[0]; h32[2] = w.tab.c_hi[0];
-            w.h_tab[2] = w.tab.c_first_win[0]; w.h_tab[3] = w.tab.c_first_win[1];
-            WT_HIP(hipMemcpyAsync(w.d_cbase, h32 + 0, sizeof(int32_t), hipMemcpyHostToDevice, s));
-            WT_HIP(hipMemcpyAsync(w.d_cnwin, h32 + 1, sizeof(int32_t), hipMemcpyHostToDevice, s));
-            WT_HIP(hipMemcpyAsync(w.d_chi, h32 + 2, sizeof(int32_t), hipMemcpyHostToDevice, s));
-            WT_HIP(hipMemcpyAsync(w.d_cfirst, w.h_tab + 2, 2 * sizeof(int64_t), hipMemcpyHostToDevice, s));
-            WT_HIP(hipMemsetAsync(w.d_win_chrom, 0, sizeof(int32_t) * (size_t) nwin, s));
-        } else {
-            const int64_t used = ((char *) w.d_win_chrom - w.d_tabs) + (int64_t) sizeof(int32_t) * std::max<int64_t>(w.tab.n_windows, 0);
-            std::vector<char> pack((size_t) used, 0);
-            memcpy(pack.data() + ((char *) w.d_cbase - w.d_tabs), w.tab.cbase.data(), sizeof(int32_t) * ts->n_chrom);
-            memcpy(pack.data() + ((char *) w.d_cnwin - w.d_tabs), w.tab.c_nwin.data(), sizeof(int32_t) * ts->n_chrom);
-            memcpy(pack.data() + ((char *) w.d_chi - w.d_tabs), w.tab.c_hi.data(), sizeof(int32_t) * ts->n_chrom);
-            memcpy(pack.data() + ((char *) w.d_cfirst - w.d_tabs), w.tab.c_first_win.data(), sizeof(int64_t) * (ts->n_chrom + 1));
-            if (w.tab.n_windows > 0) memcpy(pack.data() + ((char *) w.d_win_chrom - w.d_tabs), w.tab.win_chrom.data(), sizeof(int32_t) * w.tab.n_windows);
-            WT_HIP(hipMemcpy(w.d_tabs, pack.data(), (size_t) used, hipMemcpyHostToDevice));
+        if (ts->pipe_mode && ts->n_chrom != 1) return wt_fail(WTAMD_ERR_INTERNAL, "pipeline slots hold one chromosome");
+        if (!w.ev_tab) WT_HIP(hipEventCreateWithFlags(&w.ev_tab, hipEventDisableTiming));
+        if (w.tab_in_flight) { WT_HIP(hipEventSynchronize(w.ev_tab)); w.tab_in_flight = false; }
+        const int64_t head = (char *) w.d_win_chrom - w.d_tabs;
+        if (w.h_tab_bytes < head) {
+            if (w.h_tab) wt_host_free(w.h_tab);
+            w.h_tab = nullptr; w.h_tab_bytes = 0;
+            WT_HIP(wt_host_alloc((void **) &w.h_tab, (size_t) head));
+            w.h_tab_bytes = head;
+        }
+        const int64_t o_cfirst = (char *) w.d_cfirst - w.d_tabs;
+        const int64_t used = o_cfirst + (int64_t) sizeof(int64_t) * (ts->n_chrom + 1);
+        memset(w.h_tab, 0, (size_t) used);
+        memcpy(w.h_tab + ((char *) w.d_cbase - w.d_tabs), w.tab.cbase.data(), sizeof(int32_t) * ts->n_chrom);
+        memcpy(w.h_tab + ((char *) w.d_cnwin - w.d_tabs), w.tab.c_nwin.data(), sizeof(int32_t) * ts->n_chrom);
+        memcpy(w.h_tab + ((char *) w.d_chi - w.d_tabs), w.tab.c_hi.data(), sizeof(int32_t) * ts->n_chrom);
+        memcpy(w.h_tab + o_cfirst, w.tab.c_first_win.data(), sizeof(int64_t) * (ts->n_chrom + 1));
+        WT_HIP(hipMemcpyAsync(w.d_tabs, w.h_tab, (size_t) used, hipMemcpyHostToDevice, s));
+        WT_HIP(hipEventRecord(w.ev_tab, s));
+        w.tab_in_flight = true;
+        if (w.tab.n_windows > 0) {
+            if (ts->n_chrom == 1) {
+                WT_HIP(hipMemsetAsync(w.d_win_chrom, 0, sizeof(int32_t) * (size_t) w.tab.n_windows, s));
+            } else {
+                hipLaunchKernelGGL(wt_win_chrom_kernel, dim3((unsigned) ((w.tab.n_windows + 255) / 256)), dim3(256), 0, s,
+                                   (const int64_t *) w.d_cfirst, ts->n_chrom, (long long) w.tab.n_windows, w.d_win_chrom);
+                WT_HIP(hipGetLastError());
+            }
         }
     }
     w.tab_valid = true;
@@ -617,7 +682,7 @@
     wt_trackset_forget(ts, false);
     ts->mwu_few_ties = -1;
     if (!ts->owns && !ts->pipe_mode) {
-        int rce = wt_refresh_extents_device(ts);
+        int rce = wt_refresh_extents_device(ts, (hipStream_t) stream);
         if (rce != WTAMD_OK) return rce;
         rce = wt_check_extents(ts);
         if (rce != WTAMD_OK) return rce;
@@ -777,8 +842,9 @@
         const int64_t nwin = w->tab.n_windows > 0 ? w->tab.n_windows : 1;
         if (w->cap_bad < nwin) {
             int64_t c1 = w->cap_bad, c2 = w->cap_bad;
-            WT_HIP(wt_grow(&w->d_bad_list, &c1, nwin));
-            WT_HIP(wt_grow(&w->d_bad_goff, &c2, nwin * WT_BAD_SUB));
+            bool quiet = false;
+            WT_HIP(wt_grow(&w->d_bad_list, &c1, nwin, &quiet));
+            WT_HIP(wt_grow(&w->d_bad_goff, &c2, nwin * WT_BAD_SUB, &quiet));
             w->cap_bad = c1 < c2 / WT_BAD_SUB ? c1 : c2 / WT_BAD_SUB;
         }
         L.P.bad_list = w->d_bad_list;
@@ -786,10 +852,16 @@
         wt_delta_defaults_params(ts->defaults.data(), ts->n_tracks, L.P);
     }
 
-    WT_HIP(hipMemsetAsync(ts->d_counters, 0, sizeof(unsigned long long) * WT_CTR_N, s));
-    WT_HIP(hipMemsetAsync(L.P.chrom_run_off, 0, sizeof(int64_t) * (ts->n_chrom + 1), s));
-    if (w->tab.n_windows > 0 && ts->n_intervals > 0) {
-        WT_HIP(hipMemsetAsync(w->d_status, 0, sizeof(unsigned long long) * w->tab.n_windows, s));
+    const bool launches = w->tab.n_windows > 0 && ts->n_intervals > 0;
+    {
+        const long long n_status = launches ? (long long) w->tab.n_windows : 0;
+        const long long most = std::max<long long>(std::max<long long>(n_status, WT_CTR_N), ts->n_chrom + 1);
+        const unsigned blocks = (unsigned) std::min<long long>((most + 255) / 256, 1024);
+        hipLaunchKernelGGL(wt_clear_kernel, dim3(blocks), dim3(256), 0, s, ts->d_counters, (int) WT_CTR_N, L.P.chrom_run_off, ts->n_chrom + 1,
+                           w->d_status, n_status);
+        WT_HIP(hipGetLastError());
+    }
+    if (launches) {
         if (plan.delta) {
             static const int force_u = getenv("WTAMD_DELTA_U") ? atoi(getenv("WTAMD_DELTA_U")) : 0;
             const double tiles_per_wave = (double) ts->n_intervals / (double) w->tab.n_windows / 256.0 / (double) std::max(1, L.T / 64);
diff --git a/wiggletools_amd/csrc/wt_host.h b/wiggletools_amd/csrc/wt_host.h
--- a/wiggletools_amd/csrc/wt_host.h
+++ b/wiggletools_amd/csrc/wt_host.h
@@ -36,7 +36,10 @@
             fflush(stderr);
             _exit(70);
         }
-        if (el > nap_after_s) std::this_thread::sleep_for(std::chrono::microseconds(nap_us));
+        if (el > nap_after_s) {
+            const double nap = el * (1e6 / 64.0);
+            std::this_thread::sleep_for(std::chrono::nanoseconds((long long) (1e3 * (nap < (double) nap_us ? nap : (double) nap_us))));
+        }
     }
 }
 
diff --git a/wiggletools_amd/csrc/wt_isearch.h b/wiggletools_amd/csrc/wt_isearch.h
--- /dev/null
+++ b/wiggletools_amd/csrc/wt_isearch.h
@@ -0,0 +1,70 @@
+#ifndef WT_ISEARCH_H_
+#define WT_ISEARCH_H_
+
+#include <math.h>
+#include <stdint.h>
+
+#ifndef WT_DEV
+#if defined(__HIPCC__) && !defined(WT_EMU)
+#define WT_DEV __device__ __forceinline__
+#else
+#define WT_DEV inline
+#endif
+#endif
+
+struct WtFinArray {
+    const int32_t *p;
+    WT_DEV long long operator()(long long x) const { return (long long) p[x]; }
+};
+
+template <class Fin>
+WT_DEV long long wt_gallop_lower_bound(Fin fin, long long lo, long long hi, long long g, long long b) {
+    if (lo >= hi) return lo;
+    if (fin(g) >= b) {
+        hi = g;
+        for (long long d = 1;; d <<= 1) {
+            const long long q = hi - d;
+            if (q < lo) break;
+            if (fin(q) < b) { lo = q + 1; break; }
+            hi = q;
+        }
+    } else {
+        lo = g + 1;
+        for (long long d = 1;; d <<= 1) {
+            const long long q = lo + d - 1;
+            if (q >= hi) break;
+            if (fin(q) >= b) { hi = q; break; }
+            lo = q + 1;
+        }
+    }
+    while (lo < hi) {
+        const long long mid = (lo + hi) >> 1;
+        if (fin(mid) < b) lo = mid + 1; else hi = mid;
+    }
+    return lo;
+}
+
+#define WT_ISEARCH_STEPS 2
+template <class Fin>
+WT_DEV long long wt_interp_lower_bound(Fin fin, long long lo, long long hi, long long g, long long b, float density) {
+    if (lo >= hi) return lo;
+    if (density > 0.0f) {
+        for (int step = 0; step < WT_ISEARCH_STEPS; step++) {
+            const long long f = fin(g);
+            if (f >= b) hi = g; else lo = g + 1;
+            if (lo >= hi) return lo;
+            const float span = (float) (hi - lo);
+            const float move = fminf(fmaxf((float) (b - f) * density, -span), span);
+            g += (long long) move;
+            if (g < lo) g = lo;
+            if (g > hi - 1) g = hi - 1;
+        }
+    }
+    return wt_gallop_lower_bound(fin, lo, hi, g, b);
+}
+
+WT_DEV long long wt_lane_lower_bound(const int32_t *fin, long long lo, long long hi, long long g, long long b) {
+    return wt_gallop_lower_bound(WtFinArray{fin}, lo, hi, g, b);
+}
+
+#endif
diff --git a/wiggletools_amd/csrc/wt_pipe.hip b/wiggletools_amd/csrc/wt_pipe.hip
--- a/wiggletools_amd/csrc/wt_pipe.hip
+++ b/wiggletools_amd/csrc/wt_pipe.hip
@@ -930,33 +930,6 @@
     if (q) wt_host_free(q);
 }
 
-void wtamd_pool_trim(void) {
-    std::vector<void *> host, dev;
-    {
-        std::lock_guard<std::mutex> lk(g_pinned_pool.mu);
-        for (auto &kv : g_pinned_pool.free_list) { host.push_back(kv.second); g_pinned_pool.size_of.erase(kv.second); }
-        g_pinned_pool.free_list.clear();
-        g_pinned_pool.pooled = 0;
-    }
-    {
-        std::lock_guard<std::mutex> lk(g_dev_pool.mu);
-        for (auto &kv : g_dev_pool.free_list) { dev.push_back(kv.second); g_dev_pool.size_of.erase(kv.second); }
-        g_dev_pool.free_list.clear();
-        g_dev_pool.pooled = 0;
-    }
-    for (void *x : host) wt_pin_raw_free(x);
-    for (void *x : dev) (void) hipFree(x);
-}
-
-void wtamd_pool_stats(int64_t out[6]) {
-    if (!out) return;
-    {
-        std::lock_guard<std::mutex> lk(g_pinned_pool.mu);
-        out[0] = (int64_t) g_pinned_pool.misses; out[1] = (int64_t) g_pinned_pool.miss_bytes; out[2] = (int64_t) g_pinned_pool.pooled;
-    }
-    std::lock_guard<std::mutex> lk(g_dev_pool.mu);
-    out[3] = (int64_t) g_dev_pool.misses; out[4] = (int64_t) g_dev_pool.miss_bytes; out[5] = (int64_t) g_dev_pool.pooled;
-}
 
 int wtamd_pipe_get_stats(const wtamd_pipe *p, wtamd_pipe_stats *out) {
     if (!p || !out) return wt_fail(WTAMD_ERR_ARG, "NULL argument");
diff --git a/wiggletools_amd/csrc/wt_plan.h b/wiggletools_amd/csrc/wt_plan.h
--- a/wiggletools_amd/csrc/wt_plan.h
+++ b/wiggletools_amd/csrc/wt_plan.h
@@ -378,7 +378,7 @@
 static inline void wt_make_windows(int n_chrom, int n_tracks, const int64_t *seg_off,
                                    const int32_t *first_start, const int32_t *last_finish, int W,
                                    WtWindowTables &t, const int32_t *range_lo = nullptr,
-                                   const int32_t *range_hi = nullptr) {
+                                   const int32_t *range_hi = nullptr, bool with_win_chrom = true) {
     t.cbase.assign(n_chrom, 0);
     t.c_nwin.assign(n_chrom, 1);
     t.c_hi.assign(n_chrom, INT32_MAX);
@@ -412,7 +412,7 @@
         t.c_nwin[c] = (int32_t) nw;
         if (range_hi) t.c_hi[c] = range_hi[c];
         t.c_first_win[c + 1] = t.c_first_win[c] + nw;
-        for (int64_t m = 0; m < nw; m++) t.win_chrom.push_back(c);
+        if (with_win_chrom) t.win_chrom.insert(t.win_chrom.end(), (size_t) nw, c);
     }
     t.n_windows = t.c_first_win[n_chrom];
     t.n_rows = t.n_windows + n_chrom;
diff --git a/wiggletools_amd/csrc/wt_pool.h b/wiggletools_amd/csrc/wt_pool.h
--- a/wiggletools_amd/csrc/wt_pool.h
+++ b/wiggletools_amd/csrc/wt_pool.h
@@ -1,265 +1,25 @@
 #ifndef WT_POOL_H_
 #define WT_POOL_H_
 
-#include <sys/mman.h>
-
-#include <atomic>
-#include <cstring>
-#include <map>
-#include <mutex>
-#include <vector>
-
 #include "wt_host.h"
 
-static bool wt_is_registered(const void *q);
-static bool wt_is_pinned(const void *q) {
-    if (wt_is_registered(q)) return true;
-    hipPointerAttribute_t a;
-    if (hipPointerGetAttributes(&a, q) != hipSuccess) { (void) hipGetLastError(); return false; }
-    return a.type == hipMemoryTypeHost;
-}
+bool wt_is_pinned(const void *q);
 
-struct WtPinnedPool {
-    std::mutex mu;
-    std::multimap<size_t, void *> free_list;
-    std::map<void *, size_t> size_of;
-    size_t pooled = 0;
-    size_t misses = 0, miss_bytes = 0;
-    size_t limit() const {
-        const char *e = getenv("WTAMD_PINNED_POOL_MB");
-        return (size_t) (e ? atoll(e) : 8192) << 20;
-    }
-};
-static WtPinnedPool g_pinned_pool;
+size_t wt_pool_round(size_t bytes);
 
-static size_t wt_pool_round(size_t bytes) {
-    if (bytes < (1u << 20)) return bytes;
-    int lg = 63;
-    while (!((bytes >> lg) & 1u)) lg--;
-    const size_t step = (size_t) 1 << (lg - 3);
-    return (bytes + step - 1) / step * step;
-}
+hipError_t wt_host_alloc(void **out, size_t bytes);
+void wt_host_free(void *q);
 
-struct WtRegistered { void *base; size_t map_len; size_t len; };
-static std::mutex g_reg_mu;
-static std::map<void *, WtRegistered> g_registered;
-static std::atomic<int> g_reg_state{0};
-static std::atomic<int> g_reg_failures{0};
-
-static bool wt_is_registered(const void *q) {
-    std::lock_guard<std::mutex> lk(g_reg_mu);
-    auto it = g_registered.upper_bound((void *) q);
-    if (it == g_registered.begin()) return false;
-    --it;
-    return (const char *) q < (const char *) it->first + it->second.len;
-}
-
-static int wt_pin_threads() {
-    static const int n = [] {
-        int c = (int) std::thread::hardware_concurrency();
-        if (FILE *fp = fopen("/sys/fs/cgroup/cpu.max", "r")) {
-            char q[64]; long long period = 0;
-            if (fscanf(fp, "%63s %lld", q, &period) == 2 && period > 0 && strcmp(q, "max") != 0) {
-                const long long k = atoll(q) / period;
-                if (k >= 1 && k < c) c = (int) k;
-            }
-            fclose(fp);
-        }
-        return c < 1 ? 1 : (c > 16 ? 16 : c);
-    }();
-    return n;
-}
-
-static bool wt_pin_by_register(void **out, size_t bytes) {
-    static const bool off = getenv("WTAMD_PIN") && !strcmp(getenv("WTAMD_PIN"), "malloc");
-    if (off || g_reg_state.load() < 0 || bytes < ((size_t) 2 << 20)) return false;
-    const size_t huge = (size_t) 2 << 20;
-    const size_t len = (bytes + huge - 1) / huge * huge;
-    void *base = mmap(nullptr, len + huge, PROT_READ | PROT_WRITE, MAP_PRIVATE | MAP_ANONYMOUS, -1, 0);
-    if (base == MAP_FAILED) return false;
-    char *p = (char *) (((uintptr_t) base + huge - 1) & ~(uintptr_t) (huge - 1));
-#ifdef MADV_HUGEPAGE
-    (void) madvise(p, len, MADV_HUGEPAGE);
-#endif
-    int T = wt_pin_threads();
-    const size_t per_thread_min = (size_t) 32 << 20;
-    if ((size_t) T > len / per_thread_min) T = (int) (len / per_thread_min);
-    if (T < 1) T = 1;
-    const size_t slice = (len / (size_t) T + huge - 1) / huge * huge;
-    auto touch = [p, len, slice](int t) {
-        const size_t a = slice * (size_t) t, b = a + slice < len ? a + slice : len;
-        for (size_t q = a; q < b; q += 4096) ((volatile char *) p)[q] = 0;
-    };
-    std::vector<std::thread> th;
-    for (int t = 1; t < T; t++) th.emplace_back(touch, t);
-    touch(0);
-    for (auto &t : th) t.join();
-    void *dp = nullptr;
-    const bool registered = hipHostRegister(p, len, hipHostRegisterDefault) == hipSuccess;
-    if (!registered || hipHostGetDevicePointer(&dp, p, 0) != hipSuccess || dp != (void *) p) {
-        (void) hipGetLastError();
-        const bool never = registered;
-        if (registered) (void) hipHostUnregister(p);
-        munmap(base, len + huge);
-        if (never || g_reg_failures.fetch_add(1) + 1 >= 3) g_reg_state.store(-1);
-        return false;
-    }
-    g_reg_state.store(1);
-    g_reg_failures.store(0);
-    { std::lock_guard<std::mutex> lk(g_reg_mu); g_registered[p] = WtRegistered{base, len + huge, len}; }
-    *out = p;
-    return true;
-}
-
-static hipError_t wt_pin_raw_alloc(void **out, size_t bytes) {
-    if (wt_pin_by_register(out, bytes)) return hipSuccess;
-    return hipHostMalloc(out, bytes, hipHostMallocDefault);
-}
-
-static void wt_pin_raw_free(void *q) {
-    WtRegistered r{nullptr, 0};
-    {
-        std::lock_guard<std::mutex> lk(g_reg_mu);
-        auto it = g_registered.find(q);
-        if (it != g_registered.end()) { r = it->second; g_registered.erase(it); }
-    }
-    if (r.base) { (void) hipHostUnregister(q); munmap(r.base, r.map_len); }
-    else (void) hipHostFree(q);
-}
-
-static hipError_t wt_host_alloc(void **out, size_t bytes) {
-    if (bytes < 1) bytes = 1;
-    bytes = wt_pool_round(bytes);
-    if (bytes >= (1u << 20)) {
-        std::lock_guard<std::mutex> lk(g_pinned_pool.mu);
-        auto it = g_pinned_pool.free_list.lower_bound(bytes);
-        if (it != g_pinned_pool.free_list.end() && it->first <= bytes + bytes / 4) {
-            *out = it->second;
-            g_pinned_pool.pooled -= it->first;
-            g_pinned_pool.free_list.erase(it);
-            return hipSuccess;
-        }
-    }
-    const auto t_alloc0 = std::chrono::steady_clock::now();
-    hipError_t e = wt_pin_raw_alloc(out, bytes);
-    if (e != hipSuccess) {
-        std::vector<void *> idle;
-        {
-            std::lock_guard<std::mutex> lk(g_pinned_pool.mu);
-            for (auto &kv : g_pinned_pool.free_list) { idle.push_back(kv.second); g_pinned_pool.size_of.erase(kv.second); }
-            g_pinned_pool.free_list.clear();
-            g_pinned_pool.pooled = 0;
-        }
-        if (!idle.empty()) {
-            (void) hipGetLastError();
-            for (void *x : idle) wt_pin_raw_free(x);
-            e = wt_pin_raw_alloc(out, bytes);
-        }
-    }
-    if (e == hipSuccess && bytes >= (1u << 20)) {
-        std::lock_guard<std::mutex> lk(g_pinned_pool.mu);
-        g_pinned_pool.size_of[*out] = bytes;
-        g_pinned_pool.misses++;
-        g_pinned_pool.miss_bytes += bytes;
-        static const bool trace = getenv("WTAMD_TRACE_POOL") != nullptr;
-        bool by_register = false;
-        if (trace) { std::lock_guard<std::mutex> lk2(g_reg_mu); by_register = g_registered.count(*out) != 0; }
-        if (trace) fprintf(stderr, "[pool] page-locked %.1f MB (%s) in %.1f ms\n", bytes / 1048576.0, by_register ? "mmap + hipHostRegister" : "hipHostMalloc",
-                           std::chrono::duration<double, std::milli>(std::chrono::steady_clock::now() - t_alloc0).count());
-    }
+hipError_t wt_dev_alloc_bytes(void **out, size_t bytes, const char *file, int line);
+template <class T>
+static inline hipError_t wt_dev_alloc(T **out, size_t bytes, const char *file = __builtin_FILE(), int line = __builtin_LINE()) {
+    void *q = nullptr;
+    const hipError_t e = wt_dev_alloc_bytes(&q, bytes, file, line);
+    *out = (T *) q;
     return e;
 }
+hipError_t wt_dev_free(void *q);
 
-static void wt_host_free(void *q) {
-    if (!q) return;
-    {
-        std::lock_guard<std::mutex> lk(g_pinned_pool.mu);
-        auto it = g_pinned_pool.size_of.find(q);
-        if (it != g_pinned_pool.size_of.end()) {
-            if (g_pinned_pool.pooled + it->second <= g_pinned_pool.limit()) {
-                g_pinned_pool.free_list.emplace(it->second, q);
-                g_pinned_pool.pooled += it->second;
-                return;
-            }
-            g_pinned_pool.size_of.erase(it);
-        }
-    }
-    wt_pin_raw_free(q);
-}
-
-struct WtDevPool {
-    std::mutex mu;
-    std::multimap<std::pair<int, size_t>, void *> free_list;
-    std::map<void *, std::pair<int, size_t>> size_of;
-    size_t pooled = 0, misses = 0, miss_bytes = 0;
-    size_t limit() const {
-        const char *e = getenv("WTAMD_DEVICE_POOL_MB");
-        return (size_t) (e ? atoll(e) : 65536) << 20;
-    }
-};
-static WtDevPool g_dev_pool;
-
-template <class T>
-static hipError_t wt_dev_alloc(T **out, size_t bytes, int line = __builtin_LINE()) {
-    if (bytes < 1) bytes = 1;
-    bytes = wt_pool_round(bytes);
-    int dev = 0;
-    (void) hipGetDevice(&dev);
-    {
-        std::lock_guard<std::mutex> lk(g_dev_pool.mu);
-        auto it = g_dev_pool.free_list.lower_bound({dev, bytes});
-        if (it != g_dev_pool.free_list.end() && it->first.first == dev && it->first.second <= bytes + bytes / 4) {
-            *out = (T *) it->second;
-            g_dev_pool.pooled -= it->first.second;
-            g_dev_pool.free_list.erase(it);
-            return hipSuccess;
-        }
-    }
-    void *q = nullptr;
-    const auto t_alloc0 = std::chrono::steady_clock::now();
-    hipError_t e = hipMalloc(&q, bytes);
-    if (e != hipSuccess) {
-        std::vector<void *> idle;
-        {
-            std::lock_guard<std::mutex> lk(g_dev_pool.mu);
-            for (auto &kv : g_dev_pool.free_list) { idle.push_back(kv.second); g_dev_pool.size_of.erase(kv.second); }
-            g_dev_pool.free_list.clear();
-            g_dev_pool.pooled = 0;
-        }
-        if (!idle.empty()) {
-            (void) hipGetLastError();
-            for (void *x : idle) (void) hipFree(x);
-            e = hipMalloc(&q, bytes);
-        }
-    }
-    *out = (T *) q;
-    if (e == hipSuccess) {
-        std::lock_guard<std::mutex> lk(g_dev_pool.mu);
-        g_dev_pool.size_of[q] = {dev, bytes};
-        g_dev_pool.misses++;
-        g_dev_pool.miss_bytes += bytes;
-        static const bool trace = getenv("WTAMD_TRACE_POOL") != nullptr;
-        if (trace && bytes >= (1u << 20)) fprintf(stderr, "[pool] hipMalloc %.1f MB in %.1f ms (device %d, wt_pipe.hip:%d)\n", bytes / 1048576.0,
-                                                  std::chrono::duration<double, std::milli>(std::chrono::steady_clock::now() - t_alloc0).count(), dev, line);
-    }
-    return e;
-}
-
-static hipError_t wt_dev_free(void *q) {
-    if (!q) return hipSuccess;
-    {
-        std::lock_guard<std::mutex> lk(g_dev_pool.mu);
-        auto it = g_dev_pool.size_of.find(q);
-        if (it != g_dev_pool.size_of.end()) {
-            if (g_dev_pool.pooled + it->second.second <= g_dev_pool.limit()) {
-                g_dev_pool.free_list.emplace(it->second, q);
-                g_dev_pool.pooled += it->second.second;
-                return hipSuccess;
-            }
-            g_dev_pool.size_of.erase(it);
-        }
-    }
-    return hipFree(q);
-}
+hipError_t wt_pool_quiesce();
 
 #endif
diff --git a/wiggletools_amd/csrc/wt_pool.hip b/wiggletools_amd/csrc/wt_pool.hip
--- /dev/null
+++ b/wiggletools_amd/csrc/wt_pool.hip
@@ -0,0 +1,297 @@
+#include <sys/mman.h>
+
+#include <atomic>
+#include <cstring>
+#include <map>
+#include <mutex>
+#include <vector>
+
+#include "wt_pool.h"
+
+static bool wt_is_registered(const void *q);
+bool wt_is_pinned(const void *q) {
+    if (wt_is_registered(q)) return true;
+    hipPointerAttribute_t a;
+    if (hipPointerGetAttributes(&a, q) != hipSuccess) { (void) hipGetLastError(); return false; }
+    return a.type == hipMemoryTypeHost;
+}
+
+struct WtPinnedPool {
+    std::mutex mu;
+    std::multimap<size_t, void *> free_list;
+    std::map<void *, size_t> size_of;
+    size_t pooled = 0;
+    size_t misses = 0, miss_bytes = 0;
+    size_t limit() const {
+        const char *e = getenv("WTAMD_PINNED_POOL_MB");
+        return (size_t) (e ? atoll(e) : 8192) << 20;
+    }
+};
+static WtPinnedPool g_pinned_pool;
+
+size_t wt_pool_round(size_t bytes) {
+    if (bytes < (1u << 20)) return (bytes + 255) / 256 * 256;
+    int lg = 63;
+    while (!((bytes >> lg) & 1u)) lg--;
+    const size_t step = (size_t) 1 << (lg - 3);
+    return (bytes + step - 1) / step * step;
+}
+
+struct WtRegistered { void *base; size_t map_len; size_t len; };
+static std::mutex g_reg_mu;
+static std::map<void *, WtRegistered> g_registered;
+static std::atomic<int> g_reg_state{0};
+static std::atomic<int> g_reg_failures{0};
+
+static bool wt_is_registered(const void *q) {
+    std::lock_guard<std::mutex> lk(g_reg_mu);
+    auto it = g_registered.upper_bound((void *) q);
+    if (it == g_registered.begin()) return false;
+    --it;
+    return (const char *) q < (const char *) it->first + it->second.len;
+}
+
+static int wt_pin_threads() {
+    static const int n = [] {
+        int c = (int) std::thread::hardware_concurrency();
+        if (FILE *fp = fopen("/sys/fs/cgroup/cpu.max", "r")) {
+            char q[64]; long long period = 0;
+            if (fscanf(fp, "%63s %lld", q, &period) == 2 && period > 0 && strcmp(q, "max") != 0) {
+                const long long k = atoll(q) / period;
+                if (k >= 1 && k < c) c = (int) k;
+            }
+            fclose(fp);
+        }
+        return c < 1 ? 1 : (c > 16 ? 16 : c);
+    }();
+    return n;
+}
+
+static bool wt_pin_by_register(void **out, size_t bytes) {
+    static const bool off = getenv("WTAMD_PIN") && !strcmp(getenv("WTAMD_PIN"), "malloc");
+    if (off || g_reg_state.load() < 0 || bytes < ((size_t) 2 << 20)) return false;
+    const size_t huge = (size_t) 2 << 20;
+    const size_t len = (bytes + huge - 1) / huge * huge;
+    void *base = mmap(nullptr, len + huge, PROT_READ | PROT_WRITE, MAP_PRIVATE | MAP_ANONYMOUS, -1, 0);
+    if (base == MAP_FAILED) return false;
+    char *p = (char *) (((uintptr_t) base + huge - 1) & ~(uintptr_t) (huge - 1));
+#ifdef MADV_HUGEPAGE
+    (void) madvise(p, len, MADV_HUGEPAGE);
+#endif
+    int T = wt_pin_threads();
+    const size_t per_thread_min = (size_t) 32 << 20;
+    if ((size_t) T > len / per_thread_min) T = (int) (len / per_thread_min);
+    if (T < 1) T = 1;
+    const size_t slice = (len / (size_t) T + huge - 1) / huge * huge;
+    auto touch = [p, len, slice](int t) {
+        const size_t a = slice * (size_t) t, b = a + slice < len ? a + slice : len;
+        for (size_t q = a; q < b; q += 4096) ((volatile char *) p)[q] = 0;
+    };
+    std::vector<std::thread> th;
+    for (int t = 1; t < T; t++) th.emplace_back(touch, t);
+    touch(0);
+    for (auto &t : th) t.join();
+    void *dp = nullptr;
+    const bool registered = hipHostRegister(p, len, hipHostRegisterDefault) == hipSuccess;
+    if (!registered || hipHostGetDevicePointer(&dp, p, 0) != hipSuccess || dp != (void *) p) {
+        (void) hipGetLastError();
+        const bool never = registered;
+        if (registered) (void) hipHostUnregister(p);
+        munmap(base, len + huge);
+        if (never || g_reg_failures.fetch_add(1) + 1 >= 3) g_reg_state.store(-1);
+        return false;
+    }
+    g_reg_state.store(1);
+    g_reg_failures.store(0);
+    { std::lock_guard<std::mutex> lk(g_reg_mu); g_registered[p] = WtRegistered{base, len + huge, len}; }
+    *out = p;
+    return true;
+}
+
+static hipError_t wt_pin_raw_alloc(void **out, size_t bytes) {
+    if (wt_pin_by_register(out, bytes)) return hipSuccess;
+    return hipHostMalloc(out, bytes, hipHostMallocDefault);
+}
+
+static void wt_pin_raw_free(void *q) {
+    WtRegistered r{nullptr, 0};
+    {
+        std::lock_guard<std::mutex> lk(g_reg_mu);
+        auto it = g_registered.find(q);
+        if (it != g_registered.end()) { r = it->second; g_registered.erase(it); }
+    }
+    if (r.base) { (void) hipHostUnregister(q); munmap(r.base, r.map_len); }
+    else (void) hipHostFree(q);
+}
+
+hipError_t wt_host_alloc(void **out, size_t bytes) {
+    if (bytes < 1) bytes = 1;
+    bytes = wt_pool_round(bytes);
+    {
+        std::lock_guard<std::mutex> lk(g_pinned_pool.mu);
+        auto it = g_pinned_pool.free_list.lower_bound(bytes);
+        if (it != g_pinned_pool.free_list.end() && it->first <= bytes + bytes / 4) {
+            *out = it->second;
+            g_pinned_pool.pooled -= it->first;
+            g_pinned_pool.free_list.erase(it);
+            return hipSuccess;
+        }
+    }
+    const auto t_alloc0 = std::chrono::steady_clock::now();
+    hipError_t e = wt_pin_raw_alloc(out, bytes);
+    if (e != hipSuccess) {
+        std::vector<void *> idle;
+        {
+            std::lock_guard<std::mutex> lk(g_pinned_pool.mu);
+            for (auto &kv : g_pinned_pool.free_list) { idle.push_back(kv.second); g_pinned_pool.size_of.erase(kv.second); }
+            g_pinned_pool.free_list.clear();
+            g_pinned_pool.pooled = 0;
+        }
+        if (!idle.empty()) {
+            (void) hipGetLastError();
+            for (void *x : idle) wt_pin_raw_free(x);
+            e = wt_pin_raw_alloc(out, bytes);
+        }
+    }
+    if (e == hipSuccess && bytes < (1u << 20)) {
+        std::lock_guard<std::mutex> lk(g_pinned_pool.mu);
+        g_pinned_pool.size_of[*out] = bytes;
+    } else if (e == hipSuccess) {
+        std::lock_guard<std::mutex> lk(g_pinned_pool.mu);
+        g_pinned_pool.size_of[*out] = bytes;
+        g_pinned_pool.misses++;
+        g_pinned_pool.miss_bytes += bytes;
+        static const bool trace = getenv("WTAMD_TRACE_POOL") != nullptr;
+        bool by_register = false;
+        if (trace) { std::lock_guard<std::mutex> lk2(g_reg_mu); by_register = g_registered.count(*out) != 0; }
+        if (trace) fprintf(stderr, "[pool] page-locked %.1f MB (%s) in %.1f ms\n", bytes / 1048576.0, by_register ? "mmap + hipHostRegister" : "hipHostMalloc",
+                           std::chrono::duration<double, std::milli>(std::chrono::steady_clock::now() - t_alloc0).count());
+    }
+    return e;
+}
+
+void wt_host_free(void *q) {
+    if (!q) return;
+    {
+        std::lock_guard<std::mutex> lk(g_pinned_pool.mu);
+        auto it = g_pinned_pool.size_of.find(q);
+        if (it != g_pinned_pool.size_of.end()) {
+            if (g_pinned_pool.pooled + it->second <= g_pinned_pool.limit()) {
+                g_pinned_pool.free_list.emplace(it->second, q);
+                g_pinned_pool.pooled += it->second;
+                return;
+            }
+            g_pinned_pool.size_of.erase(it);
+        }
+    }
+    wt_pin_raw_free(q);
+}
+
+struct WtDevPool {
+    std::mutex mu;
+    std::multimap<std::pair<int, size_t>, void *> free_list;
+    std::map<void *, std::pair<int, size_t>> size_of;
+    size_t pooled = 0, misses = 0, miss_bytes = 0;
+    size_t limit() const {
+        const char *e = getenv("WTAMD_DEVICE_POOL_MB");
+        return (size_t) (e ? atoll(e) : 65536) << 20;
+    }
+};
+static WtDevPool g_dev_pool;
+
+hipError_t wt_dev_alloc_bytes(void **out, size_t bytes, const char *file, int line) {
+    if (bytes < 1) bytes = 1;
+    bytes = wt_pool_round(bytes);
+    int dev = 0;
+    (void) hipGetDevice(&dev);
+    {
+        std::lock_guard<std::mutex> lk(g_dev_pool.mu);
+        auto it = g_dev_pool.free_list.lower_bound({dev, bytes});
+        if (it != g_dev_pool.free_list.end() && it->first.first == dev && it->first.second <= bytes + bytes / 4) {
+            *out = it->second;
+            g_dev_pool.pooled -= it->first.second;
+            g_dev_pool.free_list.erase(it);
+            return hipSuccess;
+        }
+    }
+    void *q = nullptr;
+    const auto t_alloc0 = std::chrono::steady_clock::now();
+    hipError_t e = hipMalloc(&q, bytes);
+    if (e != hipSuccess) {
+        std::vector<void *> idle;
+        {
+            std::lock_guard<std::mutex> lk(g_dev_pool.mu);
+            for (auto &kv : g_dev_pool.free_list) { idle.push_back(kv.second); g_dev_pool.size_of.erase(kv.second); }
+            g_dev_pool.free_list.clear();
+            g_dev_pool.pooled = 0;
+        }
+        if (!idle.empty()) {
+            (void) hipGetLastError();
+            for (void *x : idle) (void) hipFree(x);
+            e = hipMalloc(&q, bytes);
+        }
+    }
+    *out = q;
+    if (e == hipSuccess) {
+        std::lock_guard<std::mutex> lk(g_dev_pool.mu);
+        g_dev_pool.size_of[q] = {dev, bytes};
+        g_dev_pool.misses++;
+        g_dev_pool.miss_bytes += bytes;
+        static const bool trace = getenv("WTAMD_TRACE_POOL") != nullptr;
+        if (trace && bytes >= (1u << 20)) fprintf(stderr, "[pool] hipMalloc %.1f MB in %.1f ms (device %d, %s:%d)\n", bytes / 1048576.0,
+                                                  std::chrono::duration<double, std::milli>(std::chrono::steady_clock::now() - t_alloc0).count(), dev, file, line);
+    }
+    return e;
+}
+
+hipError_t wt_dev_free(void *q) {
+    if (!q) return hipSuccess;
+    {
+        std::lock_guard<std::mutex> lk(g_dev_pool.mu);
+        auto it = g_dev_pool.size_of.find(q);
+        if (it != g_dev_pool.size_of.end()) {
+            if (g_dev_pool.pooled + it->second.second <= g_dev_pool.limit()) {
+                g_dev_pool.free_list.emplace(it->second, q);
+                g_dev_pool.pooled += it->second.second;
+                return hipSuccess;
+            }
+            g_dev_pool.size_of.erase(it);
+        }
+    }
+    return hipFree(q);
+}
+
+
+hipError_t wt_pool_quiesce() { return hipDeviceSynchronize(); }
+
+extern "C" {
+
+void wtamd_pool_trim(void) {
+    std::vector<void *> host, dev;
+    {
+        std::lock_guard<std::mutex> lk(g_pinned_pool.mu);
+        for (auto &kv : g_pinned_pool.free_list) { host.push_back(kv.second); g_pinned_pool.size_of.erase(kv.second); }
+        g_pinned_pool.free_list.clear();
+        g_pinned_pool.pooled = 0;
+    }
+    {
+        std::lock_guard<std::mutex> lk(g_dev_pool.mu);
+        for (auto &kv : g_dev_pool.free_list) { dev.push_back(kv.second); g_dev_pool.size_of.erase(kv.second); }
+        g_dev_pool.free_list.clear();
+        g_dev_pool.pooled = 0;
+    }
+    for (void *x : host) wt_pin_raw_free(x);
+    for (void *x : dev) (void) hipFree(x);
+}
+
+void wtamd_pool_stats(int64_t out[6]) {
+    if (!out) return;
+    {
+        std::lock_guard<std::mutex> lk(g_pinned_pool.mu);
+        out[0] = (int64_t) g_pinned_pool.misses; out[1] = (int64_t) g_pinned_pool.miss_bytes; out[2] = (int64_t) g_pinned_pool.pooled;
+    }
+    std::lock_guard<std::mutex> lk(g_dev_pool.mu);
+    out[3] = (int64_t) g_dev_pool.misses; out[4] = (int64_t) g_dev_pool.miss_bytes; out[5] = (int64_t) g_dev_pool.pooled;
+}
+
+}
diff --git a/wiggletools_amd/csrc/wt_trackset.h b/wiggletools_amd/csrc/wt_trackset.h
--- a/wiggletools_amd/csrc/wt_trackset.h
+++ b/wiggletools_amd/csrc/wt_trackset.h
@@ -20,7 +20,10 @@
     bool indexed = false;
     int64_t cap_chrom = 0, cap_win = 0, cap_widx = 0, cap_bad = 0, cap_cidx = 0;
     bool tab_valid = false;
-    int64_t *h_tab = nullptr;
+    char *h_tab = nullptr;
+    int64_t h_tab_bytes = 0;
+    hipEvent_t ev_tab = nullptr;
+    bool tab_in_flight = false;
     char *d_tabs = nullptr;
     int64_t cap_tabs = 0;
 };
@@ -42,6 +45,7 @@
     unsigned long long *h_counters = nullptr;
     unsigned long long *h_debug = nullptr;
     int64_t *d_chrom_run_off = nullptr;
+    int32_t *d_extents = nullptr, *h_extents = nullptr;
     char *d_gscratch = nullptr;
     size_t gscratch_bytes = 0;
     double *d_mwu_table = nullptr;
```
